# emanuelev/supereight

Measured on AMD Instinct MI355X. Metric: frames/sec (integrate+raycast), 640x480 depth -> 512^3 TSDF, higher is better.
Workload: dtype f32

## Files before the change

### include/se_hip.h

```cpp
#ifndef SE_HIP_H
#define SE_HIP_H

#include <stdint.h>

#ifdef __cplusplus
extern "C" {
#endif

#define SE_HIP_FIELD_SDF 0
#define SE_HIP_FIELD_OFUSION 1

#define SE_HIP_OK 0
#define SE_HIP_E_INVALID (-1)
#define SE_HIP_E_DEVICE (-2)
#define SE_HIP_E_CAPACITY (-3)
#define SE_HIP_E_NOGPU (-4)

typedef struct se_hip_pipeline se_hip_pipeline;

typedef struct se_hip_config {
  int32_t width;
  int32_t height;
  int32_t volume_resolution;
  float volume_dimension;
  int32_t field_type;
  int32_t device;
  int64_t max_blocks;
  int32_t row_begin;
  int32_t row_end;
} se_hip_config;

int se_hip_create(const se_hip_config* cfg, se_hip_pipeline** out);
int se_hip_create_replicas(const se_hip_config* cfg, const int32_t* device_ids, int32_t n_devices, se_hip_pipeline** out_handles);
int se_hip_destroy(se_hip_pipeline* p);
const char* se_hip_last_error(void);
int se_hip_sync(se_hip_pipeline* p);
int se_hip_clear_overflow(se_hip_pipeline* p);
int se_hip_set_stream(se_hip_pipeline* p, void* hip_stream);
int se_hip_set_scan_stream(se_hip_pipeline* p, void* hip_stream);
int se_hip_scan_overlaps(se_hip_pipeline* p);
int se_hip_set_streaming(se_hip_pipeline* p, int32_t on);
int se_hip_frame_is_fused(se_hip_pipeline* p);
int se_hip_set_image_ring(se_hip_pipeline* p, float* device_ring, int32_t slots);

int se_hip_upload_depth(se_hip_pipeline* p, const float* host_depth_m);
int se_hip_upload_depth_mm(se_hip_pipeline* p, const uint16_t* host_depth_mm, int32_t in_w, int32_t in_h);
int se_hip_set_pinned_input(se_hip_pipeline* p, int32_t on);
void* se_hip_host_alloc(size_t bytes);
void se_hip_host_free(void* host);
int se_hip_set_depth_device(se_hip_pipeline* p, const float* device_depth_m);

int se_hip_integrate(se_hip_pipeline* p, const float pose[16], const float k[4], uint32_t integration_rate, float mu,
                     uint32_t frame);
int se_hip_alloc_scan(se_hip_pipeline* p, const float pose[16], const float k[4], uint32_t integration_rate, float mu,
                      uint32_t frame);
int se_hip_new_keys_device(se_hip_pipeline* p, uint64_t** device_list, int64_t* capacity_words);
int se_hip_set_new_keys_buffer(se_hip_pipeline* p, uint64_t* device_list, int64_t capacity_words);
int se_hip_alloc_commit(se_hip_pipeline* p, const uint64_t* device_lists, int32_t nlists, int64_t stride_words);
int se_hip_set_exchange(se_hip_pipeline* p, void* nccl_comm, void* nccl_all_gather, int32_t world);
int se_hip_alloc_exchange(se_hip_pipeline* p, uint64_t* recv_device, int64_t words);
int se_hip_integrate_sweep(se_hip_pipeline* p, const float pose[16], const float k[4], uint32_t integration_rate,
                           float mu, uint32_t frame);
size_t se_hip_sweep_shard_bytes(size_t cap_bricks);
int se_hip_set_sweep_shard(se_hip_pipeline* p, int32_t rank, int32_t world, void* send_device, size_t cap_bricks);
int se_hip_apply_bricks(se_hip_pipeline* p, const void* recv_device, int32_t world);
int se_hip_brick_exchange(se_hip_pipeline* p, void* recv_device);

size_t se_hip_image_tile_bytes(se_hip_pipeline* p, int32_t max_rows);
int se_hip_pack_image_tile(se_hip_pipeline* p, void* send_device, int32_t max_rows);
int se_hip_apply_image_tiles(se_hip_pipeline* p, const void* recv_device, int32_t world, int32_t max_rows, const int32_t* row_begin, const int32_t* row_end);
int se_hip_gather_images(se_hip_pipeline* p, void* send_device, void* recv_device, int32_t max_rows, const int32_t* row_begin, const int32_t* row_end);

int se_hip_frame(se_hip_pipeline* p, const float* device_depth_m, const float pose[16], const float k[4], uint32_t integration_rate,
                 float mu, uint32_t frame);

int se_hip_raycast(se_hip_pipeline* p, const float pose[16], const float k[4], float mu, uint32_t frame);
int se_hip_raycast_deferred(se_hip_pipeline* p, const float pose[16], const float k[4], float mu, uint32_t frame);
int se_hip_download_vertex_normal(se_hip_pipeline* p, float* host_vertex_xyz, float* host_normal_xyz);
int se_hip_vertex_normal_device(se_hip_pipeline* p, float** device_vertex_xyz, float** device_normal_xyz);

int se_hip_track(se_hip_pipeline* p, const float k[4], float icp_threshold, uint32_t tracking_rate, uint32_t frame,
                 const int32_t* pyramid, int32_t n_levels, float pose_inout[16]);
int se_hip_frame_tracked(se_hip_pipeline* p, const float* device_depth_m, const float k[4], float icp_threshold, uint32_t tracking_rate,
                         const int32_t* pyramid, int32_t n_levels, float pose_inout[16], uint32_t integration_rate, float mu, uint32_t frame);
int se_hip_filter_depth(se_hip_pipeline* p, int32_t on);
int se_hip_download_scaled_depth(se_hip_pipeline* p, int32_t level, float* host_out);
int se_hip_download_track(se_hip_pipeline* p, void* host_trackdata, float host_reduce32[32], int32_t* iterations);

int se_hip_render_volume(se_hip_pipeline* p, uint8_t* host_rgbw, const float view_pose[16], const float k[4], float mu, float largestep,
                         uint32_t frame, uint32_t raycast_rendering_rate);
int se_hip_render_depth(se_hip_pipeline* p, uint8_t* host_rgbw);
int se_hip_render_track(se_hip_pipeline* p, uint8_t* host_rgbw);

int se_hip_counts(se_hip_pipeline* p, int32_t* n_blocks, int32_t* n_nodes);
int se_hip_memory_info(se_hip_pipeline* p, int64_t out[4]);
int se_hip_download_blocks(se_hip_pipeline* p, int32_t* coords, float* x, float* y, uint8_t* active);
int se_hip_download_nodes(se_hip_pipeline* p, uint64_t* code, uint32_t* side, float* x, float* y);

typedef struct se_hip_query_out {
  float* fine;
  float* coarse;
  float* interp;
  float* grad;
  uint8_t* status;
} se_hip_query_out;
int se_hip_query_points(se_hip_pipeline* p, const float* device_points_m, int64_t n, const se_hip_query_out* device_out);
int se_hip_query_points_host(se_hip_pipeline* p, const float* host_points_m, int64_t n, const se_hip_query_out* host_out);

#define SE_HIP_COLLISION_OCCUPIED 0
#define SE_HIP_COLLISION_UNSEEN 1
#define SE_HIP_COLLISION_EMPTY 2
#define SE_HIP_COLLISION_INVALID 255
#define SE_HIP_COLLIDE_STRICT 0
#define SE_HIP_COLLIDE_REFERENCE 1
typedef struct se_hip_collide_test {
  float threshold;
  int32_t occupied_above;
} se_hip_collide_test;
int se_hip_collide_boxes(se_hip_pipeline* p, const int32_t* device_boxes, int64_t n, const se_hip_collide_test* test, int32_t mode,
                         uint8_t* device_status);
int se_hip_collide_boxes_host(se_hip_pipeline* p, const int32_t* host_boxes, int64_t n, const se_hip_collide_test* test, int32_t mode,
                              uint8_t* host_status);

#define SE_HIP_RAY_VALID 1
#define SE_HIP_RAY_ENTERED 2
#define SE_HIP_RAY_HIT 4
#define SE_HIP_RAY_NORMAL 8
typedef struct se_hip_ray_out {
  float* hit;
  float* normal;
  uint8_t* status;
} se_hip_ray_out;
int se_hip_cast_rays(se_hip_pipeline* p, const float* device_rays, int64_t n, float mu, const se_hip_ray_out* device_out);
int se_hip_cast_rays_host(se_hip_pipeline* p, const float* host_rays, int64_t n, float mu, const se_hip_ray_out* host_out);

int se_hip_save_map(se_hip_pipeline* p, const char* filename);
int se_hip_load_map(se_hip_pipeline* p, const char* filename);

int se_hip_mesh_count(se_hip_pipeline* p, int64_t* n_triangles);
int se_hip_mesh_download(se_hip_pipeline* p, float* host_triangles, int64_t capacity_triangles, int64_t* n_written);
int se_hip_dump_mesh(se_hip_pipeline* p, const char* filename);

#define SE_HIP_MESH_MAX_VIEWS 64
#define SE_HIP_MESH_SKIP_EMPTY 1u
typedef struct se_hip_mesh_view {
  float pose[16];
  float k[4];
  int32_t width, height;
} se_hip_mesh_view;
typedef struct se_hip_mesh_select {
  int32_t lo[3], hi[3];
  int32_t n_views;
  uint32_t flags;
  const se_hip_mesh_view* views;
} se_hip_mesh_select;
typedef struct se_hip_mesh_out {
  float* triangles;
  int64_t capacity_triangles;
  int32_t* block_coords;
  int64_t* block_range;
  int64_t capacity_blocks;
  int64_t* header;
} se_hip_mesh_out;
int se_hip_mesh_blocks(se_hip_pipeline* p, const se_hip_mesh_select* select, const se_hip_mesh_out* device_out);
int se_hip_mesh_blocks_host(se_hip_pipeline* p, const se_hip_mesh_select* select, const se_hip_mesh_out* host_out);

#define SE_HIP_EDIT_SET_X 1u
#define SE_HIP_EDIT_SET_Y 2u
#define SE_HIP_EDIT_BLOCKS 4u
#define SE_HIP_EDIT_NODES 8u
#define SE_HIP_EDIT_STRICT 0
#define SE_HIP_EDIT_REFERENCE 1
typedef struct se_hip_edit {
  int32_t lo[3], hi[3];
  float x, y;
  uint32_t flags;
  uint32_t only;
} se_hip_edit;
int se_hip_edit_boxes(se_hip_pipeline* p, const se_hip_edit* device_edits, int64_t n, const se_hip_collide_test* test,
                      int32_t mode, int64_t* device_counts);
int se_hip_edit_boxes_host(se_hip_pipeline* p, const se_hip_edit* host_edits, int64_t n, const se_hip_collide_test* test,
                           int32_t mode, int64_t* host_counts);

typedef struct se_hip_alloc_box {
  int32_t lo[3], hi[3];
  int32_t level;
  uint32_t reserved;
} se_hip_alloc_box;
int se_hip_allocate_boxes(se_hip_pipeline* p, const se_hip_alloc_box* device_boxes, int64_t n, int64_t* device_counts,
                          uint64_t* device_new_keys, int64_t capacity_words);
int se_hip_allocate_boxes_host(se_hip_pipeline* p, const se_hip_alloc_box* host_boxes, int64_t n, int64_t* host_counts,
                               uint64_t* host_new_keys, int64_t capacity_words);

#define SE_HIP_K_ALLOC_SCAN 0
#define SE_HIP_K_ALLOC_COMMIT 1
#define SE_HIP_K_INTEGRATE 2
#define SE_HIP_K_RAYCAST 3
#define SE_HIP_K_APPLY_BRICKS 4
#define SE_HIP_K_COUNT 5
int se_hip_enable_timing(se_hip_pipeline* p, int32_t on);
int se_hip_get_timings(se_hip_pipeline* p, double ms_sum[SE_HIP_K_COUNT], int64_t launches[SE_HIP_K_COUNT], int32_t reset);
int se_hip_get_launch_counts(se_hip_pipeline* p, int64_t counts[SE_HIP_K_COUNT + 1], int32_t reset);
int se_hip_enable_stats(se_hip_pipeline* p, int32_t on);
int se_hip_get_stats(se_hip_pipeline* p, uint64_t out[16], int32_t reset);

#ifdef __cplusplus
}
#endif
#endif
```

### supereight_amd/csrc/se_hip_api.hip

```cpp
#include "../../include/se_hip.h"

#include <hip/hip_runtime.h>
#include <hipcub/device/device_radix_sort.hpp>

#include <algorithm>
#include <cmath>
#include <cstdio>
#include <cstdlib>
#include <atomic>
#include <chrono>
#include <cstring>
#include <thread>
#include <numeric>
#include <string>
#include <vector>

#include "se_kernels.h"
#include "se_track_kernels.h"
#include "se_mesh_kernels.h"
#include "se_query_kernels.h"
#include "se_collide_kernels.h"
#include "se_edit_kernels.h"
#include "se_alloc_kernels.h"
#include "se_ray_kernels.h"
// ... 17 lines not shown
  for (int c = 0; c < 4; ++c)
    for (int r = 0; r < 4; ++r) a.m[r][c] = p[c * 4 + r];
  return a;
}
M4 mul(const M4& a, const M4& b) {
  M4 c;
  for (int i = 0; i < 4; ++i)
    for (int j = 0; j < 4; ++j)
      c.m[i][j] = ((a.m[i][0] * b.m[0][j] + a.m[i][1] * b.m[1][j]) + a.m[i][2] * b.m[2][j]) + a.m[i][3] * b.m[3][j];
  return c;
}
M4 camera_matrix(const float k[4]) { return {{{k[0], 0, k[2], 0}, {0, k[1], k[3], 0}, {0, 0, 1, 0}, {0, 0, 0, 1}}}; }
M4 inverse_camera_matrix(const float k[4]) {
  return {{{1.0f / k[0], 0, -k[2] / k[0], 0}, {0, 1.0f / k[1], -k[3] / k[1], 0}, {0, 0, 1, 0}, {0, 0, 0, 1}}};
}
void mul3(const float r[9], const float v[3], float out[3]) {
  out[0] = (r[0] * v[0] + r[1] * v[1]) + r[2] * v[2];
  out[1] = (r[3] * v[0] + r[4] * v[1]) + r[5] * v[2];
  out[2] = (r[6] * v[0] + r[7] * v[1]) + r[8] * v[2];
}

struct TimedLaunch { int kernel; hipEvent_t start, stop; };

inline void cpu_relax() {
#if defined(__x86_64__) || defined(__i386__)
  __builtin_ia32_pause();
#elif defined(__aarch64__) || defined(__arm__)
  asm volatile("yield" ::: "memory");
#else
  std::this_thread::yield();
#endif
}
template <typename F> bool spin_until(F done, long long limit_us) {
  const auto t0 = std::chrono::steady_clock::now();
  for (unsigned n = 1;; ++n) {
    if (done()) { std::atomic_thread_fence(std::memory_order_acquire); return true; }
    cpu_relax();
    if ((n & 255u) == 0u && std::chrono::duration_cast<std::chrono::microseconds>(std::chrono::steady_clock::now() - t0).count() > limit_us) {
      const bool ok = done();
      std::atomic_thread_fence(std::memory_order_acquire);
      return ok;
    }
  }
}

}

struct se_hip_pipeline {
  se_hip_config cfg;
  int device = 0;
  hipStream_t stream = nullptr;
  bool own_stream = false;
  hipStream_t side = nullptr;
  bool own_side = false;
  hipEvent_t ev_sweep = nullptr, ev_scan = nullptr;
  hipEvent_t ev_edit = nullptr;
  bool overlap = false;
  bool host_gate = false;
  uint32_t* gate_host = nullptr;
  uint32_t ray_seq = 0;
  uint32_t gate_target = 0;
  bool gate_armed = false;
  bool gate_followed = false;
  bool sharded = false;
  bool fuse = false, in_frame = false, has_pending = false;
  int flush_streak = 0;
  bool pinned_input = false;
  int sort_every = 0;
  uint32_t* bpos_sorted = nullptr; void* sort_tmp = nullptr; size_t sort_tmp_bytes = 0, sort_cap = 0;
  uint32_t sorted_n = 0; int sweeps_since_sort = 0;
  bool ptrs_exposed = false;
  float pend_pose[16] = {0}, pend_k[4] = {0}, pend_mu = 0.f;
  uint32_t pend_frame = 0;
  bool images_complete = true;
  bool scan_pending = false;
  bool scan_on_side = false;
  const float* scaled0 = nullptr;
  void* xcomm = nullptr;
  int (*xgather)(const void*, void*, size_t, int, void*, hipStream_t) = nullptr;
  int xworld = 0;
  int shard_world = 0, shard_rank = 0;
  unsigned char* shard_send = nullptr;
  size_t shard_cap = 0;
  bool mc_table_ready = false;
  unsigned long long* mesh_ctr = nullptr;
  unsigned char* staging = nullptr;
  size_t staging_cap = 0;
  unsigned char* meshb_dev = nullptr;
  bool filter_input = false;
  bool occ_commit_due = false;
  OccLists occ_lists{nullptr, 0, 0};
  float raycast_pose[16] = {1, 0, 0, 0, 0, 1, 0, 0, 0, 0, 1, 0, 0, 0, 0, 1};
  std::vector<float*> pyr_depth, pyr_vertex, pyr_normal;
  TrackData* track = nullptr;
  float* reduce_partial = nullptr;
  IcpState* icp = nullptr;
  IcpHostRecord* icp_host = nullptr;
  unsigned reduce_seq = 0;
  int track_iterations = 0;
  int icp_lookahead = 2;
  bool scan_on_main_once = false;
  unsigned char* rgbw = nullptr;
  DevMap map{};
  int leaf_level = 0, max_level = 0;
  size_t tab_entries = 0;
  size_t occ_words = 0, lbits_words = 0, cbits_words = 0, fbits_words = 0;
  bool of_leap = true;
  int beam = 2;
  size_t slots = 0;
  size_t cap_blocks = 0, cap_nodes = 0;
  int ray_cache_levels = -1;
  const float* depth = nullptr;
  static constexpr int kIn = 3;
  float* depth_ring[kIn] = {nullptr, nullptr, nullptr};
  void* in_host[kIn] = {nullptr, nullptr, nullptr};
  size_t in_cap = 0;
  int in_next = 0;
  int in_state[kIn] = {0, 0, 0};
  uint32_t in_seq[kIn] = {0, 0, 0};
  hipEvent_t in_done[kIn] = {nullptr, nullptr, nullptr};
  bool in_event[kIn] = {false, false, false};
  int cur_in = -1;
  DepthSrc in_pending{nullptr, nullptr, 0, 0, 0};
  float* vertex = nullptr;
  float* normal = nullptr;
  float* vertex_own = nullptr;
  float* normal_own = nullptr;
  float* ring = nullptr;
  int ring_slots = 0;
  int64_t n_launch[SE_HIP_K_COUNT + 1] = {0};
  float* bspline = nullptr;
  float* logodds = nullptr;
  unsigned long long* chain = nullptr;
  unsigned long long* newkeys_own = nullptr;
  unsigned long long* newkeys_own2 = nullptr;
  unsigned long long cap_keys_own = 0;
  int own_next = 0;
  bool own_clean[2] = {false, false};
  uint32_t* ctr_host = nullptr;
  bool timing = false, stats = false;
  std::vector<TimedLaunch> pending;
  std::vector<hipEvent_t> event_pool;
  double ms_sum[SE_HIP_K_COUNT] = {0};
  int64_t launches[SE_HIP_K_COUNT] = {0};
  int row_begin = 0, row_end = 0;
  int integ_grid = 0;
  bool ieee_sweep = false;
  unsigned short* tile_cost = nullptr;
  int* prio_thr = nullptr;
  bool prio_hint = true;
  int prio_permille[3] = {400, 150, 50};
  uint32_t* ray_order = nullptr;
  int n_cus = 256;
};

namespace {

int ilog2(int v) { int l = 0; while ((1 << l) < v) ++l; return l; }

hipEvent_t get_event(se_hip_pipeline* p) {
  if (!p->event_pool.empty()) { hipEvent_t e = p->event_pool.back(); p->event_pool.pop_back(); return e; }
  hipEvent_t e;
  hipEventCreateWithFlags(&e, hipEventDisableSystemFence);
  return e;
}
struct ScopedTimer {
  se_hip_pipeline* p; int k; hipStream_t s; hipEvent_t a{}, b{};
  ScopedTimer(se_hip_pipeline* p_, int k_, hipStream_t s_ = nullptr) : p(p_), k(k_), s(s_ ? s_ : p_->stream) {
    p->n_launch[k]++;
    if (p->timing) { a = get_event(p); b = get_event(p); hipEventRecord(a, s); }
  }
  ~ScopedTimer() {
    if (p->timing) { hipEventRecord(b, s); p->pending.push_back({k, a, b}); }
  }
};
void drain_timings(se_hip_pipeline* p) {
  if (p->pending.empty()) return;
  if (p->side) hipStreamSynchronize(p->side);
  hipStreamSynchronize(p->stream);
  for (auto& t : p->pending) {
    float ms = 0.f;
    if (hipEventElapsedTime(&ms, t.start, t.stop) == hipSuccess) { p->ms_sum[t.kernel] += ms; p->launches[t.kernel]++; }
    p->event_pool.push_back(t.start);
    p->event_pool.push_back(t.stop);
  }
  p->pending.clear();
}

double bspline_cdf(double t) {
  if (t >= -3.0 && t <= -1.0) return std::pow(3 + t, 3) / 48.0;
  if (t > -1 && t <= 1) return 0.5 + (t * (3 + t) * (3 - t)) / 24.0;
  if (t > 1 && t <= 3) return 1 - std::pow(3 - t, 3) / 48.0;
  if (t > 3) return 1.0;
  return 0.0;
}
void make_bspline(std::vector<float>& lut) {
  lut.resize(1000);
  for (int i = 0; i < 1000; ++i) {
    char buf[64];
    std::snprintf(buf, sizeof buf, "%.12g", bspline_cdf(-3.0 + 6.0 * i / 999.0));
    lut[i] = (float)std::strtod(buf, nullptr);
  }
}
void make_logodds(const std::vector<float>& lut, std::vector<float>& tab) {
  tab.resize((size_t)SE_LO_DIM * SE_LO_DIM);
  auto q = [&](int i) { return i < 1000 ? lut[i] : (i == 1001 ? 1.f : 0.f); };
  for (int i1 = 0; i1 < SE_LO_DIM; ++i1)
    for (int i2 = 0; i2 < SE_LO_DIM; ++i2) {
      float sample = q(i1) - q(i2) * 0.5f;
      sample = std::max(0.03f, std::min(sample, 0.97f));
      tab[(size_t)i1 * SE_LO_DIM + i2] = log2f(sample / (1.f - sample));
    }
}

int run_zero_chain(se_hip_pipeline* p, const unsigned long long* lists, int nlists, long long stride_words) {
  ScopedTimer t(p, SE_HIP_K_ALLOC_COMMIT);
  hipLaunchKernelGGL(k_zero_chain, dim3(1), dim3(SE_WG), 0, p->stream, p->map, lists, nlists, stride_words);
  return SE_HIP_OK;
}


M4 rigid_inverse(const M4& a) {
  M4 r{};
  for (int i = 0; i < 3; ++i)
    for (int j = 0; j < 3; ++j) r.m[i][j] = a.m[j][i];
  for (int i = 0; i < 3; ++i) r.m[i][3] = -((r.m[i][0] * a.m[0][3] + r.m[i][1] * a.m[1][3]) + r.m[i][2] * a.m[2][3]);
  r.m[3][3] = 1.f;
  return r;
}

struct RayLaunchArgs { RayArgs a; size_t smem; dim3 grid; };

size_t ray_map_args(se_hip_pipeline* p, float mu, RayArgs& a) {
  const DevMap& m = p->map;
  a.mu = mu;
  a.step = m.dim / (float)m.size;
  a.largestep = a.step * 8;
  a.inv_voxel = (float)m.size / m.dim;
  a.grad_scale = 0.5f * m.dim / (float)m.size;
  a.epsilon = exp2f(-(float)p->max_level);
  a.min_scale = 23 - p->leaf_level;
  int cl = p->ray_cache_levels >= 0 ? p->ray_cache_levels : 5;
  cl = std::min(cl, p->leaf_level);
  a.cache_levels = cl;
  a.cache_words = (int)occ_words_upto(cl);
  a.cache_codes = 2u << (3 * cl);
  a.has_deep = cl < p->leaf_level - 1 ? 1 : 0;
  a.stack_depth = p->leaf_level;
  return ((size_t)a.cache_words + (size_t)2 * a.stack_depth * SE_WG_RAY) * sizeof(uint32_t);
}

RayLaunchArgs make_ray_args(se_hip_pipeline* p, const float pose_cm[16], const float k[4], float mu) {
  RayLaunchArgs L{};
  const DevMap& m = p->map;
  const M4 view = mul(from_colmajor(pose_cm), inverse_camera_matrix(k));
  RayArgs& a = L.a;
  for (int i = 0; i < 3; ++i) { for (int j = 0; j < 3; ++j) a.view3[i * 3 + j] = view.m[i][j]; a.org[i] = view.m[i][3]; }
  a.nearp = 0.4f; a.farp = 4.0f;
  a.near_n = a.nearp / m.dim; a.far_n = a.farp / m.dim;
  for (int i = 0; i < 3; ++i) a.scaled_origin[i] = a.org[i] / m.dim + 1.f;
  L.smem = ray_map_args(p, mu, a);
  a.W = p->cfg.width; a.H = p->cfg.height; a.row_begin = p->row_begin; a.row_end = p->row_end;
  a.tile_cost = p->prio_hint ? p->tile_cost : nullptr;
  a.prio_thr = p->prio_thr;
  a.cost_shift = std::max(0, p->leaf_level - 6);
  a.ray_order = p->ray_order; a.n_cus = p->n_cus;
  a.beam = (p->beam >= 2 && !m.fbits) ? 1 : p->beam;
  const int flevel = m.fbits ? se_flevel(m) : m.leaf_level;
  a.beam_cellf = m.dim / (float)(1 << flevel);
  a.beam_inv_cellf = (float)(1 << flevel) / m.dim;
  a.beam_dt2 = 0.4f * a.beam_cellf;
  if (a.beam >= 2) {
    const float rad = 1.05f * std::hypot(0.5f * (SE_TILE_W - 1) / std::fabs(k[0]), 0.5f * (SE_TILE_H - 1) / std::fabs(k[1])) + a.epsilon;
    if (!((0.75f * a.farp + 0.5f * a.beam_dt2) * rad + 0.5f * a.beam_dt2 <= 0.9f * a.beam_cellf)) a.beam = 1;
  }
  a.beam_cell = m.dim / (float)(1 << m.clevel);
  a.beam_inv_cell = (float)(1 << m.clevel) / m.dim;
  a.beam_dt = std::max(0.5f * a.beam_cell, (a.farp - a.nearp) / 64.f);
  a.inv_dim = 1.f / m.dim;
  a.leap_bits = !p->of_leap ? nullptr : m.fbits ? m.fbits : (m.clevel == m.leaf_level ? m.cbits : nullptr);
  a.leap_level = flevel;
  a.leap_dt = 0.9f * a.beam_cellf;
  a.wlog = nullptr;
#ifdef SE_WAVE_PROBE
  {
    static unsigned long long* wl = nullptr;
    static bool tried = false;
    if (!tried) { tried = true; if (std::getenv("SE_HIP_WLOG")) { hipHostMalloc((void**)&wl, 4 * 8 * 32768, 0); std::memset(wl, 0, 4 * 8 * 32768); } }
    a.wlog = wl;
    if (wl) { hipStreamSynchronize(p->stream); if (FILE* f = std::fopen(std::getenv("SE_HIP_WLOG"), "wb")) { std::fwrite(wl, 8, 4 * 32768, f); std::fclose(f); } std::memset(wl, 0, 4 * 8 * 32768); }
  }
#endif
  const int tiles_x = (a.W + SE_TILE_W - 1) / SE_TILE_W, tiles_y = (a.row_end - a.row_begin + SE_TILE_H - 1) / SE_TILE_H;
  const int n_pairs = (tiles_x * tiles_y + 1) / 2;
  L.grid = dim3((unsigned)(((n_pairs + p->n_cus - 1) / p->n_cus) * p->n_cus));
  return L;
}

RayLaunchArgs make_batch_ray_args(se_hip_pipeline* p, float mu) {
  RayLaunchArgs L{};
  RayArgs& a = L.a;
  L.smem = ray_map_args(p, mu, a);
  a.gate = nullptr; a.tile_cost = nullptr; a.ray_order = nullptr; a.prio_thr = nullptr; a.wlog = nullptr; a.leap_bits = nullptr;
  a.beam = 0;
  return L;
}

struct RaySel { bool ofusion, dense, shallow, o32; };
RaySel ray_kernel_sel(const se_hip_pipeline* p, const RayArgs& a) {
  const DevMap& m = p->map;
  const size_t nb = (size_t)(m.size >> 3);
  const bool shallow = !a.has_deep;
  return {p->cfg.field_type != SE_HIP_FIELD_SDF, m.dense != 0, shallow,
          m.dense && shallow && nb * nb * nb * (size_t)SE_BRICK_STRIDE * sizeof(float) <= ((size_t)4 << 30)};
}

void wait_last_sweep(se_hip_pipeline* p) {
  if (!p->gate_armed) return;
  p->gate_armed = false;
  if (p->gate_followed) {
    volatile uint32_t* w = p->gate_host;
    const uint32_t target = p->gate_target;
    if (!spin_until([&] { return (int32_t)(*w - target) >= 0; }, 20000)) hipStreamSynchronize(p->stream);
    return;
  }
  hipStreamSynchronize(p->stream);
}

void materialise_depth(se_hip_pipeline* p, hipStream_t s) {
  if (p->in_pending.kind == 0) return;
  const int W = p->cfg.width, H = p->cfg.height;
  hipLaunchKernelGGL(k_depth_from_host, dim3((W + 255) / 256, H), dim3(256), 0, s, p->in_pending, W, H);
  p->in_pending.kind = 0;
}
void input_slot_in_use(se_hip_pipeline* p) { if (p->cur_in >= 0) { p->in_state[p->cur_in] = 1; p->in_event[p->cur_in] = false; } }
void input_slots_followed(se_hip_pipeline* p, uint32_t seq) {
  for (int i = 0; i < se_hip_pipeline::kIn; ++i) if (p->in_state[i] == 1) { p->in_state[i] = 2; p->in_seq[i] = seq; }
}

int join_scan(se_hip_pipeline* p, bool fold_into_sweep = false) {
  if (p->scan_pending) {
    p->scan_pending = false;
    HIP_TRY(hipStreamWaitEvent(p->stream, p->ev_scan, 0));
    p->occ_commit_due = true;
    if (!p->occ_lists.lists) p->occ_lists = OccLists{p->map.newkeys, 1, (long long)p->map.cap_keys + 1};
    if (p->cfg.field_type == SE_HIP_FIELD_OFUSION && !p->sharded)
      if (int r = run_zero_chain(p, p->map.newkeys, 1, (long long)p->map.cap_keys + 1)) return r;
  }
  if (p->occ_commit_due && !fold_into_sweep) {
    p->occ_commit_due = false;
    ScopedTimer t(p, SE_HIP_K_ALLOC_COMMIT);
    hipLaunchKernelGGL(k_occ_commit, dim3(64), dim3(SE_WG), 0, p->stream, p->map, p->occ_lists);
    p->occ_lists = OccLists{nullptr, 0, 0};
  }
  return SE_HIP_OK;
}

int check(se_hip_pipeline* p) {
  if (!p) return fail(SE_HIP_E_INVALID, "null handle");
  int cur = -1;
  if (!(hipGetDevice(&cur) == hipSuccess && cur == p->device)) {
    hipError_t e = hipSetDevice(p->device);
    if (e != hipSuccess) return fail(SE_HIP_E_DEVICE, std::string("hipSetDevice: ") + hipGetErrorString(e));
  }
  if (p->has_pending && !p->in_frame) { ++p->flush_streak; return flush_pending_raycast(p); }
  return SE_HIP_OK;
}

int check_overflow(se_hip_pipeline* p) {
  const uint32_t o = p->ctr_host[C_OVERFLOW];
  if (o == 3) return fail(SE_HIP_E_CAPACITY, "brick exchange segment overflow: the peers missed block updates (raise cap_bricks of se_hip_set_sweep_shard)");
  if (o) return fail(SE_HIP_E_CAPACITY, o == 2 ? "new-key list overflow: blocks were allocated locally but not reported to the peers (raise the exchange capacity)"
                                              : "block / node pool exhausted (raise max_blocks)");
  return SE_HIP_OK;
}

int fetch_counters(se_hip_pipeline* p) {
  if (int r = join_scan(p)) return r;
  HIP_TRY(hipMemcpyAsync(p->ctr_host, p->map.ctr, C_COUNT * sizeof(uint32_t), hipMemcpyDeviceToHost, p->stream));
  HIP_TRY(hipStreamSynchronize(p->stream));
  return check_overflow(p);
}

int reserve_staging(se_hip_pipeline* p, size_t need) {
  if (need <= p->staging_cap) return SE_HIP_OK;
  if (p->staging) { HIP_TRY(hipStreamSynchronize(p->stream)); hipFree(p->staging); p->staging = nullptr; p->staging_cap = 0; }
  HIP_TRY(hipMalloc((void**)&p->staging, need));
  p->staging_cap = need;
  return SE_HIP_OK;
}
size_t staging_layout(const size_t* bytes, int k, size_t* off) {
  size_t at = 0;
  for (int i = 0; i < k; ++i) { off[i] = at; at += bytes[i]; }
  return at;
}
template <typename Check> int query_prologue(se_hip_pipeline* p, Check args_ok) {
  if (int r = check(p)) return r;
  if (int r = args_ok()) return r;
  return join_scan(p);
}
struct BatchOut { void* ptr; size_t item_bytes; bool per_call = false; };
struct BatchOuts { int count; BatchOut o[5]; };
template <typename Check, typename Launch>
int batch_device(se_hip_pipeline* p, const void* in, int64_t n, const BatchOuts& out, Check args_ok, Launch launch) {
  if (int r = query_prologue(p, args_ok)) return r;
  if (int r = check_overflow(p)) return r;
  if (n == 0) return SE_HIP_OK;
  void* dev[5];
  for (int k = 0; k < out.count; ++k) dev[k] = out.o[k].ptr;
  launch(in, dev);
  HIP_TRY(hipGetLastError());
  return SE_HIP_OK;
}
template <typename Check, typename Launch>
int batch_host(se_hip_pipeline* p, const void* in, size_t in_item_bytes, int64_t n, const BatchOuts& out, Check args_ok, Launch launch) {
  if (int r = query_prologue(p, args_ok)) return r;
  if (n == 0) return fetch_counters(p);
  const size_t un = (size_t)n;
  size_t bytes[6], off[6];
  bytes[0] = un * in_item_bytes;
  for (int k = 0; k < out.count; ++k) bytes[k + 1] = out.o[k].ptr ? (out.o[k].per_call ? 1 : un) * out.o[k].item_bytes : 0;
  if (int r = reserve_staging(p, staging_layout(bytes, out.count + 1, off))) return r;
  unsigned char* b = p->staging;
  HIP_TRY(hipMemcpyAsync(b, in, bytes[0], hipMemcpyHostToDevice, p->stream));
  void* dev[5];
  for (int k = 0; k < out.count; ++k) dev[k] = bytes[k + 1] ? b + off[k + 1] : nullptr;
  launch(b, dev);
  HIP_TRY(hipGetLastError());
  for (int k = 0; k < out.count; ++k)
    if (bytes[k + 1]) HIP_TRY(hipMemcpyAsync(out.o[k].ptr, dev[k], bytes[k + 1], hipMemcpyDeviceToHost, p->stream));
  return fetch_counters(p);
}

void select_image_target(se_hip_pipeline* p, uint32_t frame) {
  if (p->ring) {
    const size_t n3 = (size_t)p->cfg.width * p->cfg.height * 3;
    p->vertex = p->ring + (size_t)(frame % (uint32_t)p->ring_slots) * 2 * n3;
    p->normal = p->vertex + n3;
  } else {
    p->vertex = p->vertex_own; p->normal = p->normal_own;
  }
}
struct InFrame { se_hip_pipeline* p; bool was; explicit InFrame(se_hip_pipeline* q, bool on = true) : p(q), was(q->in_frame) { q->in_frame = on; } ~InFrame() { p->in_frame = was; } };

bool finite_pose(const float* pose_cm, const float* k) {
  bool ok = true;
  for (int i = 0; i < 16; ++i) ok = ok && std::isfinite(pose_cm[i]);
  for (int i = 0; i < 4; ++i) ok = ok && std::isfinite(k[i]);
  return ok && k[0] != 0.f && k[1] != 0.f;
}

bool stage_runs_integration(uint32_t frame, uint32_t rate) { return ((frame % rate) == 0) || (frame <= 3); }

void reset_map_state(se_hip_pipeline* p) {
  DevMap& m = p->map;
  hipMemsetAsync(m.tab, 0, p->tab_entries * sizeof(uint32_t), p->stream);
  hipMemsetAsync(m.occ, 0, p->occ_words * sizeof(uint32_t), p->stream);
  hipMemsetAsync(m.lbits, 0, p->lbits_words * sizeof(uint32_t), p->stream);
  hipMemsetAsync(m.cbits, 0, 2 * p->cbits_words * sizeof(uint32_t), p->stream);
  if (m.fbits) hipMemsetAsync(m.fbits, 0, p->fbits_words * sizeof(uint32_t), p->stream);
  hipMemsetAsync(m.bpos, 0, p->cap_blocks * sizeof(uint32_t), p->stream);
  hipMemsetAsync(m.bactive, 0, p->slots, p->stream);
  hipMemsetAsync(m.npos, 0, p->cap_nodes * sizeof(uint32_t), p->stream);
  hipMemsetAsync(m.nlevel, 0, p->cap_nodes, p->stream);
  hipMemsetAsync(m.stats, 0, S_COUNT * sizeof(unsigned long long), p->stream);
  hipMemsetAsync(m.newkeys, 0, sizeof(unsigned long long), p->stream);
  if (p->newkeys_own) hipMemsetAsync(p->newkeys_own, 0, sizeof(unsigned long long), p->stream);
  if (p->newkeys_own2) hipMemsetAsync(p->newkeys_own2, 0, sizeof(unsigned long long), p->stream);
  p->own_clean[0] = p->newkeys_own != nullptr; p->own_clean[1] = p->newkeys_own2 != nullptr;
  const uint32_t ctr0[C_COUNT] = {0u, 1u, 0u, 0u, 0u, 0u, 0u, 0u};
  hipMemcpyAsync(m.ctr, ctr0, sizeof ctr0, hipMemcpyHostToDevice, p->stream);
  std::memset(p->ctr_host, 0, C_COUNT * sizeof(uint32_t));
  p->ctr_host[C_NODES] = 1u;
  p->sorted_n = 0; p->sweeps_since_sort = 0;
  hipLaunchKernelGGL(k_fill_bricks, dim3(16384), dim3(256), 0, p->stream, m.vx, m.init_x, m.init_y, p->slots * 1024);
  hipLaunchKernelGGL(k_fill, dim3(256), dim3(256), 0, p->stream, m.nx, m.init_x, p->cap_nodes * 8);
  hipLaunchKernelGGL(k_fill, dim3(256), dim3(256), 0, p->stream, m.ny, m.init_y, p->cap_nodes * 8);
}

int grid_for(size_t n, int wg, int cap) { size_t g = (n + wg - 1) / wg; if (g < 1) g = 1; if (g > (size_t)cap) g = cap; return (int)g; }

}

extern "C" {

const char* se_hip_last_error(void) { return g_err.c_str(); }

int se_hip_create(const se_hip_config* cfg, se_hip_pipeline** out) {
  if (!cfg || !out) return fail(SE_HIP_E_INVALID, "null argument");
  *out = nullptr;
  const int N = cfg->volume_resolution;
  if (cfg->width <= 0 || cfg->height <= 0) return fail(SE_HIP_E_INVALID, "bad image size");
  if (N < 64 || N > 4096 || (N & (N - 1))) return fail(SE_HIP_E_INVALID, "volume_resolution must be a power of two in [64, 4096]");
  if (!(cfg->volume_dimension > 0)) return fail(SE_HIP_E_INVALID, "volume_dimension must be positive");
  if (cfg->field_type != SE_HIP_FIELD_SDF && cfg->field_type != SE_HIP_FIELD_OFUSION) return fail(SE_HIP_E_INVALID, "unknown field type");
  int ndev = 0;
  if (hipGetDeviceCount(&ndev) != hipSuccess || ndev <= 0) return fail(SE_HIP_E_NOGPU, "no HIP device visible (this library has no CPU path)");
  if (cfg->device < 0 || cfg->device >= ndev) return fail(SE_HIP_E_INVALID, "device ordinal out of range");
  HIP_TRY(hipSetDevice(cfg->device));
  hipDeviceProp_t prop;
  HIP_TRY(hipGetDeviceProperties(&prop, cfg->device));
  if (std::string(prop.gcnArchName).find("gfx950") == std::string::npos)
    return fail(SE_HIP_E_NOGPU, std::string("device is ") + prop.gcnArchName + ", this library is built for gfx950 only");

  se_hip_pipeline* p = new se_hip_pipeline();
  p->cfg = *cfg;
  p->device = cfg->device;
  p->row_begin = cfg->row_begin;
  p->row_end = (cfg->row_end > cfg->row_begin) ? cfg->row_end : cfg->height;
  if (p->row_begin < 0 || p->row_end > cfg->height) { delete p; return fail(SE_HIP_E_INVALID, "bad row range"); }
  if (const char* ev = std::getenv("SE_HIP_RAY_CACHE_LEVELS")) p->ray_cache_levels = std::atoi(ev);
  if (const char* ev = std::getenv("SE_HIP_ICP_LOOKAHEAD")) p->icp_lookahead = std::max(0, std::atoi(ev));
  if (const char* ev = std::getenv("SE_HIP_INTEG_GRID")) p->integ_grid = std::atoi(ev);
  if (const char* ev = std::getenv("SE_HIP_BEAM")) p->beam = std::max(0, std::min(2, std::atoi(ev)));
  if (const char* ev = std::getenv("SE_HIP_OF_LEAP")) p->of_leap = std::atoi(ev) != 0;
  if (const char* ev = std::getenv("SE_HIP_IEEE_SWEEP")) p->ieee_sweep = std::atoi(ev) != 0;
  if (const char* ev = std::getenv("SE_HIP_PRIO")) p->prio_hint = std::atoi(ev) != 0;
  if (const char* ev = std::getenv("SE_HIP_PRIO_SHARE")) {
    int a = 0, b = 0, c = 0;
    if (std::sscanf(ev, "%d,%d,%d", &a, &b, &c) == 3 && a >= b && b >= c && c >= 0 && a <= 1000) { p->prio_permille[0] = a; p->prio_permille[1] = b; p->prio_permille[2] = c; }
  }
  p->max_level = ilog2(N);
  p->leaf_level = p->max_level - 3;
  DevMap& m = p->map;
  m.size = N; m.max_level = p->max_level; m.leaf_level = p->leaf_level; m.dim = cfg->volume_dimension;
  size_t off = 0;
  for (int l = 0; l < SE_MAX_LEVELS; ++l) m.off[l] = 0;
  for (int l = 1; l <= p->leaf_level; ++l) { m.off[l] = (uint32_t)off; off += (size_t)1 << (3 * l); }
  p->tab_entries = off;
  m.leaf_off = m.off[p->leaf_level];
  p->occ_words = occ_words_upto(p->leaf_level);
  const size_t cells = (size_t)1 << (3 * p->leaf_level);
  size_t free_b = 0, total_b = 0;
  hipMemGetInfo(&free_b, &total_b);
  size_t dense_max_gib = 64;
  if (const char* ev = std::getenv("SE_HIP_DENSE_MAX_GIB")) dense_max_gib = (size_t)std::max(0, std::atoi(ev));

  bool dense = cfg->max_blocks <= 0 && cells * 4096 <= free_b / 3 && cells * 4096 <= (dense_max_gib << 30);
  if (const char* ev = std::getenv("SE_HIP_DENSE")) dense = std::atoi(ev) != 0 && cells * 4096 <= free_b / 2;
  const size_t nb_side = (size_t)cfg->volume_resolution / 8;
  const size_t cap_default = std::max((size_t)1 << 16, ((24 * nb_side * nb_side + 4095) / 4096) * 4096);
  size_t cap = cfg->max_blocks > 0 ? (size_t)cfg->max_blocks : (dense ? cells : std::max((size_t)1 << 16, std::min(cap_default, free_b / 3 / 4096)));
  cap = std::min(cap, cells);
  m.dense = dense ? 1 : 0;
  p->sort_every = (dense && nb_side >= 128) ? 4 : 0;
  if (const char* ev = std::getenv("SE_HIP_SORT_BLOCKS")) p->sort_every = dense ? std::max(0, std::atoi(ev)) : 0;
  const size_t slots = dense ? cells : cap;
  p->slots = slots;
  size_t capn = std::min(off - cells + 1, cap / 2 + 4096);
  m.cap_blocks = (uint32_t)cap; m.cap_nodes = (uint32_t)capn;
  m.cap_keys = cap + capn;
  if (cfg->field_type == SE_HIP_FIELD_SDF) { m.init_x = 1.f; m.init_y = 0.f; m.empty_x = 1.f; }
  else { m.init_x = 0.f; m.init_y = 0.f; m.empty_x = 0.f; }

  auto bail = [&](hipError_t e, const char* what) { std::string msg = std::string(what) + ": " + hipGetErrorString(e); se_hip_destroy(p); return fail(SE_HIP_E_DEVICE, msg); };
#define ALLOC(ptr, bytes) do { hipError_t e_ = hipMalloc((void**)&(ptr), (bytes)); if (e_ != hipSuccess) return bail(e_, "hipMalloc " #ptr); } while (0)
  hipError_t e = hipStreamCreateWithFlags(&p->stream, hipStreamNonBlocking);
  if (e != hipSuccess) return bail(e, "hipStreamCreate");
  p->own_stream = true;
  e = hipStreamCreateWithFlags(&p->side, hipStreamNonBlocking);
  if (e != hipSuccess) return bail(e, "hipStreamCreate");
  p->own_side = true;
  hipEventCreateWithFlags(&p->ev_sweep, hipEventDisableTiming | hipEventDisableSystemFence);
  hipEventCreateWithFlags(&p->ev_scan, hipEventDisableTiming | hipEventDisableSystemFence);
  p->sharded = (p->row_begin != 0 || p->row_end != cfg->height);
  p->overlap = (dense || !(std::getenv("SE_HIP_POOLED_OVERLAP") && std::atoi(std::getenv("SE_HIP_POOLED_OVERLAP")) == 0)) && !std::getenv("SE_HIP_NO_OVERLAP");
  p->host_gate = p->overlap && !p->sharded;
  if (const char* ev = std::getenv("SE_HIP_HOST_GATE")) p->host_gate = p->host_gate && std::atoi(ev) != 0;
  if (p->host_gate) {
    e = hipHostMalloc((void**)&p->gate_host, 64);
    if (e != hipSuccess) return bail(e, "hipHostMalloc");
    std::memset(p->gate_host, 0, 64);
  }
  ALLOC(m.tab, p->tab_entries * sizeof(uint32_t));
  ALLOC(m.occ, p->occ_words * sizeof(uint32_t));
  p->lbits_words = (cells + 31) / 32;
  ALLOC(m.lbits, p->lbits_words * sizeof(uint32_t));
  m.clevel = std::min(p->leaf_level, 5);
  p->cbits_words = std::max<size_t>(1, ((size_t)1 << (3 * m.clevel)) / 32);
  ALLOC(m.cbits, 2 * p->cbits_words * sizeof(uint32_t));
  m.fbits = nullptr;
  if (se_flevel(m) > m.clevel) { p->fbits_words = ((size_t)1 << (3 * se_flevel(m))) / 32; ALLOC(m.fbits, p->fbits_words * sizeof(uint32_t)); }
  ALLOC(m.vx, slots * 1024 * sizeof(float));
  m.ybyte = cfg->field_type == SE_HIP_FIELD_SDF ? 1 : 0;
  ALLOC(m.bpos, cap * sizeof(uint32_t));
  ALLOC(m.bactive, (slots + 3) & ~(size_t)3);
  ALLOC(m.nx, capn * 8 * sizeof(float));
  ALLOC(m.ny, capn * 8 * sizeof(float));
  ALLOC(m.npos, capn * sizeof(uint32_t));
  ALLOC(m.nlevel, capn);
  ALLOC(m.ctr, C_COUNT * sizeof(uint32_t));
  ALLOC(m.stats, S_COUNT * sizeof(unsigned long long));
  ALLOC(m.newkeys, (m.cap_keys + 1) * sizeof(unsigned long long));
  p->newkeys_own = m.newkeys; p->cap_keys_own = m.cap_keys;
  ALLOC(p->newkeys_own2, (m.cap_keys + 1) * sizeof(unsigned long long));
  for (int i = 0; i < se_hip_pipeline::kIn; ++i) ALLOC(p->depth_ring[i], (size_t)cfg->width * cfg->height * sizeof(float));
  ALLOC(p->vertex_own, (size_t)cfg->width * cfg->height * 3 * sizeof(float));
  ALLOC(p->normal_own, (size_t)cfg->width * cfg->height * 3 * sizeof(float));
  p->vertex = p->vertex_own; p->normal = p->normal_own;
  ALLOC(p->chain, 4 * sizeof(unsigned long long));
  const size_t n_tiles = ((size_t)(cfg->width + SE_TILE_W - 1) / SE_TILE_W) * ((size_t)(cfg->height + SE_TILE_H - 1) / SE_TILE_H);
  ALLOC(p->tile_cost, (n_tiles + 4096) * sizeof(unsigned short));
  ALLOC(p->prio_thr, 4 * sizeof(int));
  hipMemsetAsync(p->tile_cost, 0, (n_tiles + 4096) * sizeof(unsigned short), p->stream);
  {
    hipDeviceProp_t prop{};
    if (hipGetDeviceProperties(&prop, p->device) == hipSuccess && prop.multiProcessorCount > 0) p->n_cus = prop.multiProcessorCount;
    if (const char* ev = std::getenv("SE_HIP_RAY_DEAL")) p->n_cus = std::max(1, std::atoi(ev));
    const size_t n_pairs = (n_tiles + 1) / 2;
    ALLOC(p->ray_order, n_pairs * sizeof(uint32_t));
    std::vector<uint32_t> ident(n_pairs);
    for (size_t i = 0; i < n_pairs; ++i) ident[i] = (uint32_t)i;
    hipMemcpyAsync(p->ray_order, ident.data(), n_pairs * sizeof(uint32_t), hipMemcpyHostToDevice, p->stream);
    hipStreamSynchronize(p->stream);
  }
  { const int off[4] = {256, 256, 256, 0}; hipMemcpyAsync(p->prio_thr, off, sizeof off, hipMemcpyHostToDevice, p->stream); }
  p->depth = p->depth_ring[0]; p->cur_in = 0;
  e = hipHostMalloc((void**)&p->ctr_host, C_COUNT * sizeof(uint32_t));
  if (e != hipSuccess) return bail(e, "hipHostMalloc");
  std::memset(p->ctr_host, 0, C_COUNT * sizeof(uint32_t));

  p->cap_blocks = cap; p->cap_nodes = capn;
  reset_map_state(p);
  for (int i = 0; i < se_hip_pipeline::kIn; ++i) hipMemsetAsync(p->depth_ring[i], 0, (size_t)cfg->width * cfg->height * sizeof(float), p->stream);
  hipMemsetAsync(p->vertex, 0, (size_t)cfg->width * cfg->height * 3 * sizeof(float), p->stream);
  hipMemsetAsync(p->normal, 0, (size_t)cfg->width * cfg->height * 3 * sizeof(float), p->stream);
  if (cfg->field_type == SE_HIP_FIELD_OFUSION) {
    std::vector<float> lut, lo;
    make_bspline(lut);
    make_logodds(lut, lo);
    ALLOC(p->bspline, lut.size() * sizeof(float));
    ALLOC(p->logodds, lo.size() * sizeof(float));
    hipMemcpy(p->bspline, lut.data(), lut.size() * sizeof(float), hipMemcpyHostToDevice);
    hipMemcpy(p->logodds, lo.data(), lo.size() * sizeof(float), hipMemcpyHostToDevice);
  }
#undef ALLOC
  e = hipStreamSynchronize(p->stream);
  if (e != hipSuccess) return bail(e, "initialisation");
  *out = p;
  return SE_HIP_OK;
}

int se_hip_destroy(se_hip_pipeline* p) {
  if (!p) return SE_HIP_OK;
  p->has_pending = false;
  hipSetDevice(p->device);
  if (p->side) hipStreamSynchronize(p->side);
  if (p->stream) hipStreamSynchronize(p->stream);
  for (auto& t : p->pending) { hipEventDestroy(t.start); hipEventDestroy(t.stop); }
  for (auto& ev : p->event_pool) hipEventDestroy(ev);
  DevMap& m = p->map;
  void* ptrs[] = {m.occ, m.lbits, m.cbits, m.fbits, m.tab, m.vx, m.bpos, m.bactive, m.nx, m.ny, m.npos, m.nlevel, m.ctr, m.stats, p->newkeys_own, p->newkeys_own2,
                  p->depth_ring[0], p->depth_ring[1], p->depth_ring[2], p->vertex_own, p->normal_own, p->bspline, p->logodds, p->chain, p->tile_cost, p->prio_thr, p->ray_order};
  for (void* q : ptrs) if (q) hipFree(q);
  for (auto* q : p->pyr_depth) if (q) hipFree(q);
  for (auto* q : p->pyr_vertex) if (q) hipFree(q);
  for (auto* q : p->pyr_normal) if (q) hipFree(q);
  if (p->track) hipFree(p->track);
  if (p->rgbw) hipFree(p->rgbw);
  if (p->reduce_partial) hipFree(p->reduce_partial);
  if (p->icp) hipFree(p->icp);
  if (p->icp_host) hipHostFree(p->icp_host);
  if (p->ctr_host) hipHostFree(p->ctr_host);
  if (p->bpos_sorted) hipFree(p->bpos_sorted);
  if (p->sort_tmp) hipFree(p->sort_tmp);
  if (p->gate_host) hipHostFree(p->gate_host);
  if (p->mesh_ctr) hipFree(p->mesh_ctr);
  if (p->staging) hipFree(p->staging);
  if (p->meshb_dev) hipFree(p->meshb_dev);
  for (int i = 0; i < se_hip_pipeline::kIn; ++i) { if (p->in_host[i]) hipHostFree(p->in_host[i]); if (p->in_done[i]) hipEventDestroy(p->in_done[i]); }
  if (p->own_side && p->side) hipStreamDestroy(p->side);
  if (p->ev_sweep) hipEventDestroy(p->ev_sweep);
  if (p->ev_scan) hipEventDestroy(p->ev_scan);
  if (p->ev_edit) hipEventDestroy(p->ev_edit);
  if (p->own_stream && p->stream) hipStreamDestroy(p->stream);
  delete p;
  return SE_HIP_OK;
}

int se_hip_sync(se_hip_pipeline* p) {
  if (int r = check(p)) return r;
  if (p->side) HIP_TRY(hipStreamSynchronize(p->side));
  HIP_TRY(hipStreamSynchronize(p->stream));
  p->gate_armed = false;
  return check_overflow(p);
}

int se_hip_clear_overflow(se_hip_pipeline* p) {
  if (int r = check(p)) return r;
  if (p->side) HIP_TRY(hipStreamSynchronize(p->side));
  HIP_TRY(hipStreamSynchronize(p->stream));
  p->gate_armed = false;
  uint32_t dev = 0;
  HIP_TRY(hipMemcpy(&dev, p->map.ctr + C_OVERFLOW, sizeof dev, hipMemcpyDeviceToHost));
  const uint32_t pending = std::max(dev, p->ctr_host[C_OVERFLOW]);
  HIP_TRY(hipMemsetAsync(p->map.ctr + C_OVERFLOW, 0, sizeof(uint32_t), p->stream));
  HIP_TRY(hipStreamSynchronize(p->stream));
  p->ctr_host[C_OVERFLOW] = 0u;
  return (int)pending;
}

int se_hip_set_stream(se_hip_pipeline* p, void* hip_stream) {
  if (int r = check(p)) return r;
  HIP_TRY(hipStreamSynchronize(p->stream));
  p->gate_armed = false;
  drain_timings(p);
  if (p->own_stream && p->stream) hipStreamDestroy(p->stream);
  p->stream = (hipStream_t)hip_stream;
  p->own_stream = false;
  return SE_HIP_OK;
}

int se_hip_scan_overlaps(se_hip_pipeline* p) {
  if (int r = check(p)) return r;
  return p->overlap ? 1 : 0;
}

int se_hip_set_scan_stream(se_hip_pipeline* p, void* hip_stream) {
  if (int r = check(p)) return r;
  if (p->side) HIP_TRY(hipStreamSynchronize(p->side));
  HIP_TRY(hipStreamSynchronize(p->stream));
  drain_timings(p);
  if (p->own_side && p->side) hipStreamDestroy(p->side);
  p->side = nullptr; p->own_side = false;
  if (hip_stream) { p->side = (hipStream_t)hip_stream; return SE_HIP_OK; }
  HIP_TRY(hipStreamCreateWithFlags(&p->side, hipStreamNonBlocking));
  p->own_side = true;
  return SE_HIP_OK;
}

static int stage_input(se_hip_pipeline* p, const void* host, size_t bytes, int kind, int in_w, int ratio) {
  constexpr int R = se_hip_pipeline::kIn;
  if (p->in_cap < bytes) {
    if (p->side) HIP_TRY(hipStreamSynchronize(p->side));
    HIP_TRY(hipStreamSynchronize(p->stream));
    for (int i = 0; i < R; ++i) { if (p->in_host[i]) hipHostFree(p->in_host[i]); p->in_host[i] = nullptr; p->in_state[i] = 0; p->in_event[i] = false; }
    p->in_cap = 0; p->in_pending.kind = 0;
    for (int i = 0; i < R; ++i) HIP_TRY(hipHostMalloc(&p->in_host[i], bytes));
    p->in_cap = bytes;
  }
  const int i = p->in_next;
  p->in_next = (i + 1) % R;
  if (p->in_state[i] == 2 && p->host_gate) {
    volatile uint32_t* w = p->gate_host;
    const uint32_t target = p->in_seq[i];
    if (!spin_until([&] { return (int32_t)(*w - target) >= 0; }, 20000)) { if (p->side) hipStreamSynchronize(p->side); hipStreamSynchronize(p->stream); }
  } else if (p->in_event[i]) {
    HIP_TRY(hipEventSynchronize(p->in_done[i]));
  } else if (p->in_state[i] != 0) {
    if (p->side) HIP_TRY(hipStreamSynchronize(p->side));
    HIP_TRY(hipStreamSynchronize(p->stream));
  }
  p->in_state[i] = 0; p->in_event[i] = false;
  const void* src = p->in_host[i];
  if (p->pinned_input) {
    hipPointerAttribute_t at{};
    if (hipPointerGetAttributes(&at, host) == hipSuccess && at.type == hipMemoryTypeHost && at.devicePointer) src = at.devicePointer;
    else (void)hipGetLastError();
  }
  if (src == p->in_host[i]) std::memcpy(p->in_host[i], host, bytes);
  p->in_pending = DepthSrc{src, p->depth_ring[i], kind, in_w, ratio};
  p->depth = p->depth_ring[i];
  p->cur_in = i;
  return SE_HIP_OK;
}

int se_hip_upload_depth(se_hip_pipeline* p, const float* host_depth_m) {
  if (!p) return fail(SE_HIP_E_INVALID, "null handle");
  InFrame guard(p);
  if (int r = check(p)) return r;
  if (!host_depth_m) return fail(SE_HIP_E_INVALID, "null depth");
  return stage_input(p, host_depth_m, (size_t)p->cfg.width * p->cfg.height * sizeof(float), 2, p->cfg.width, 1);
}

int se_hip_upload_depth_mm(se_hip_pipeline* p, const uint16_t* host_mm, int32_t in_w, int32_t in_h) {
  if (!p) return fail(SE_HIP_E_INVALID, "null handle");
  InFrame guard(p);
  if (int r = check(p)) return r;
  if (!host_mm) return fail(SE_HIP_E_INVALID, "null depth");
  const int W = p->cfg.width, H = p->cfg.height;
  if (in_w < W || in_h < H || in_w % W != 0 || in_h % H != 0 || in_w / W != in_h / H) return fail(SE_HIP_E_INVALID, "Invalid ratio.");
  return stage_input(p, host_mm, (size_t)in_w * in_h * sizeof(unsigned short), 1, in_w, in_w / W);
}

int se_hip_set_pinned_input(se_hip_pipeline* p, int32_t on) {
  if (!p) return fail(SE_HIP_E_INVALID, "null handle");
  p->pinned_input = on != 0;
  return SE_HIP_OK;
}
void* se_hip_host_alloc(size_t bytes) {
  void* h = nullptr;
  if (bytes == 0 || hipHostMalloc(&h, bytes) != hipSuccess) { (void)hipGetLastError(); return nullptr; }
  return h;
}
void se_hip_host_free(void* host) { if (host) (void)hipHostFree(host); }

int se_hip_set_depth_device(se_hip_pipeline* p, const float* device_depth_m) {
  if (!p) return fail(SE_HIP_E_INVALID, "null handle");
  InFrame guard(p);
  if (int r = check(p)) return r;
  if (device_depth_m) { p->depth = device_depth_m; p->cur_in = -1; p->in_pending.kind = 0; }
  else if (p->cur_in < 0) { p->depth = p->depth_ring[0]; p->cur_in = 0; }
  return SE_HIP_OK;
}

int launch_raycast_scan(se_hip_pipeline* p, const DevMap& ms, const AllocArgs& sa, int scan_wgs, const DepthSrc& ds) {
  const DevMap& m = p->map;
  if (int r = check_overflow(p)) return r;
  p->has_pending = false;
  p->flush_streak = 0;
  std::memcpy(p->raycast_pose, p->pend_pose, sizeof p->raycast_pose);
  p->images_complete = !p->sharded;
  select_image_target(p, p->pend_frame);
  p->n_launch[SE_HIP_K_ALLOC_SCAN]++; p->n_launch[SE_HIP_K_COUNT]++;
  RayLaunchArgs L = make_ray_args(p, p->pend_pose, p->pend_k, p->pend_mu);
  if (p->host_gate) { L.a.gate = p->gate_host; L.a.gate_seq = ++p->ray_seq; if (p->gate_armed) p->gate_followed = true; input_slots_followed(p, L.a.gate_seq); }
  const RayArgs& a = L.a;
  const int ray_wgs = (int)L.grid.x;
  const size_t smem = std::max(L.smem, (size_t)SE_SCAN_SLOTS * SE_WG_SCAN * sizeof(uint32_t));
  const dim3 grid((unsigned)(ray_wgs + scan_wgs)), block(SE_WG_RAY);
  const RaySel s = ray_kernel_sel(p, a);
  const bool shallow = s.dense ? s.o32 : s.shallow;
  {
    ScopedTimer t(p, SE_HIP_K_RAYCAST);
#define SE_RS(OF, DN, SH, O3) hipLaunchKernelGGL((k_raycast_scan<OF, DN, SH, O3>), grid, block, smem, p->stream, m, a, p->vertex, p->normal, ray_wgs, ms, p->depth, sa, ds)
    if (!s.ofusion) {
      if (s.dense) { if (shallow) SE_RS(false, true, true, true); else SE_RS(false, true, false, false); }
      else { if (shallow) SE_RS(false, false, true, false); else SE_RS(false, false, false, false); }
    } else {
      if (s.dense) { if (shallow) SE_RS(true, true, true, true); else SE_RS(true, true, false, false); }
      else { if (shallow) SE_RS(true, false, true, false); else SE_RS(true, false, false, false); }
    }
#undef SE_RS
  }
  HIP_TRY(hipGetLastError());
  return SE_HIP_OK;
}

static bool frame_can_fuse(se_hip_pipeline* p);
int se_hip_alloc_scan(se_hip_pipeline* p, const float pose_cm[16], const float k[4], uint32_t rate, float mu, uint32_t frame) {
  if (!p) return fail(SE_HIP_E_INVALID, "null handle");
  const bool ride = p->has_pending && !p->in_frame && rate != 0 && stage_runs_integration(frame, rate) && frame_can_fuse(p);
  InFrame guard(p, ride || p->in_frame);
  if (int r = check(p)) return r;
  if (!pose_cm || !k || rate == 0) return fail(SE_HIP_E_INVALID, "bad argument");
  if (!finite_pose(pose_cm, k)) return fail(SE_HIP_E_INVALID, "non-finite pose or intrinsics");
  if (!stage_runs_integration(frame, rate)) return 0;
  const DevMap& m = p->map;
  const M4 pose = from_colmajor(pose_cm);
  const bool sdf = p->cfg.field_type == SE_HIP_FIELD_SDF;
  AllocArgs a{};
  const float voxelsize = m.dim / (float)m.size;
  const M4 kPose = mul(pose, inverse_camera_matrix(k));
  for (int i = 0; i < 3; ++i)
    for (int j = 0; j < 4; ++j) a.kpose[i * 4 + j] = kPose.m[i][j];
  a.cam[0] = pose.m[0][3]; a.cam[1] = pose.m[1][3]; a.cam[2] = pose.m[2][3];
  a.band = sdf ? 2 * mu : 6 * mu;
  a.voxel = voxelsize;
  a.inv_voxel = sdf ? 1 / voxelsize : 1.f / voxelsize;
  a.num_steps = (int)std::ceil(a.band * a.inv_voxel);
  a.W = p->cfg.width; a.H = p->cfg.height; a.row_begin = p->row_begin; a.row_end = p->row_end;
  a.sharded = (p->row_begin != 0 || p->row_end != p->cfg.height) ? 1 : 0;
  auto s2d = [&](float step) { return (int)(floorf(log2f(voxelsize / step)) + m.max_level); };
  a.depth_fine = s2d(voxelsize); a.depth_mid = s2d(10.f * voxelsize); a.depth_coarse = s2d(30.f * voxelsize);
  const bool caller_list = p->map.newkeys != p->newkeys_own && p->map.newkeys != p->newkeys_own2;
  const bool fuse_now = p->has_pending && p->in_frame && p->overlap && !p->stats && p->shard_world <= 1;
  const bool chain = p->scan_on_main_once && !p->sharded && !caller_list && p->xgather == nullptr;
  p->scan_on_main_once = false;
  const bool ov = !fuse_now && !chain && p->overlap && (p->sharded || caller_list || p->xgather != nullptr || hipStreamQuery(p->stream) == hipErrorNotReady);
  p->scan_on_side = ov;
  hipStream_t s = ov ? p->side : p->stream;
  DevMap ms = m;
  ms.defer_occ = (ov || fuse_now) ? 1 : 0;
  ms.defer_mark = 1;
  if (ov) { if (p->host_gate) wait_last_sweep(p); else HIP_TRY(hipStreamWaitEvent(p->side, p->ev_sweep, 0)); }
  else if (p->overlap) { if (int r = join_scan(p)) return r; }
  const bool own_list = p->map.newkeys == p->newkeys_own || p->map.newkeys == p->newkeys_own2;
  if (own_list) {
    const int w = p->own_next;
    p->map.newkeys = w ? p->newkeys_own2 : p->newkeys_own;
    ms.newkeys = p->map.newkeys;
    if (!p->own_clean[w]) HIP_TRY(hipMemsetAsync(p->map.newkeys, 0, sizeof(unsigned long long), s));
    p->own_clean[w] = false;
  } else {
    HIP_TRY(hipMemsetAsync(m.newkeys, 0, sizeof(unsigned long long), s));
  }
  const int npix = (p->row_end - p->row_begin) * p->cfg.width;
  const dim3 grid((npix + SE_WG_SCAN - 1) / SE_WG_SCAN), block(SE_WG_SCAN);
  if (a.sharded) materialise_depth(p, s);
  const DepthSrc ds = p->in_pending;
  p->in_pending.kind = 0;
  const int sdf_tiles = ds.kind ? ((p->cfg.width + 63) / 64) * (p->row_end - p->row_begin) : ((p->cfg.width + 7) / 8) * ((p->row_end - p->row_begin + 7) / 8);
  if (!sdf) {
    const int dep[3] = {a.depth_fine, a.depth_mid, a.depth_coarse};
    for (int i = 0; i < 3; ++i) { a.of_lvl[i] = std::min(dep[i], m.leaf_level); a.of_off[i] = a.of_lvl[i] >= 1 ? m.off[a.of_lvl[i]] : 0u; }
  }
  if (fuse_now) {
    const int scan_wgs = sdf ? (sdf_tiles + SE_WG_SCAN / 64 - 1) / (SE_WG_SCAN / 64) : (int)grid.x;
    if (int r = launch_raycast_scan(p, ms, a, scan_wgs, ds)) return r;
    input_slot_in_use(p);
    p->occ_commit_due = true;
    if (!p->occ_lists.lists) p->occ_lists = OccLists{p->map.newkeys, 1, (long long)p->map.cap_keys + 1};
    if (!sdf && !a.sharded) { if (int r = run_zero_chain(p, p->map.newkeys, 1, (long long)p->map.cap_keys + 1)) return r; }
    HIP_TRY(hipGetLastError());
    return 1;
  }
  {
    ScopedTimer t(p, SE_HIP_K_ALLOC_SCAN, s);
    if (sdf) {
      const dim3 sgrid((sdf_tiles + SE_WG_SCAN / 64 - 1) / (SE_WG_SCAN / 64));
      if (m.dense) {
        if (p->stats) hipLaunchKernelGGL((k_alloc_scan_sdf<true, true>), sgrid, block, 0, s, ms, p->depth, a, ds);
        else hipLaunchKernelGGL((k_alloc_scan_sdf<false, true>), sgrid, block, 0, s, ms, p->depth, a, ds);
      } else {
        if (p->stats) hipLaunchKernelGGL((k_alloc_scan_sdf<true, false>), sgrid, block, 0, s, ms, p->depth, a, ds);
        else hipLaunchKernelGGL((k_alloc_scan_sdf<false, false>), sgrid, block, 0, s, ms, p->depth, a, ds);
      }
    } else {
      if (p->stats) hipLaunchKernelGGL(k_alloc_scan_ofusion<true>, grid, block, 0, s, ms, p->depth, a, ds);
      else hipLaunchKernelGGL(k_alloc_scan_ofusion<false>, grid, block, 0, s, ms, p->depth, a, ds);
    }
  }
  input_slot_in_use(p);
  if (ov) {
    HIP_TRY(hipEventRecord(p->ev_scan, p->side));
    p->scan_pending = true;
    HIP_TRY(hipGetLastError());
    return 1;
  }
  p->occ_commit_due = true;
  if (!p->occ_lists.lists) p->occ_lists = OccLists{p->map.newkeys, 1, (long long)p->map.cap_keys + 1};
  if (!sdf && !a.sharded) {
    if (int r = run_zero_chain(p, m.newkeys, 1, (long long)m.cap_keys + 1)) return r;
  }
  HIP_TRY(hipGetLastError());
  return 1;
}

int se_hip_new_keys_device(se_hip_pipeline* p, uint64_t** device_list, int64_t* capacity_words) {
  if (int r = check(p)) return r;
  if (int r = join_scan(p)) return r;
  if (device_list) *device_list = (uint64_t*)p->map.newkeys;
  if (capacity_words) *capacity_words = (int64_t)p->map.cap_keys + 1;
  return SE_HIP_OK;
}

int se_hip_set_new_keys_buffer(se_hip_pipeline* p, uint64_t* device_list, int64_t capacity_words) {
  if (!p) return fail(SE_HIP_E_INVALID, "null handle");
  InFrame guard(p);
  if (int r = check(p)) return r;
  if (device_list && capacity_words < 2) return fail(SE_HIP_E_INVALID, "key buffer too small");
  p->map.newkeys = device_list ? (unsigned long long*)device_list : p->newkeys_own;
  p->map.cap_keys = device_list ? (unsigned long long)(capacity_words - 1) : p->cap_keys_own;
  return SE_HIP_OK;
}

int se_hip_alloc_commit(se_hip_pipeline* p, const uint64_t* device_lists, int32_t nlists, int64_t stride_words) {
  if (int r = check(p)) return r;
  if (!device_lists || nlists <= 0 || stride_words < 1) return fail(SE_HIP_E_INVALID, "bad argument");
  const unsigned long long* lists = (const unsigned long long*)device_lists;
  if (p->overlap && p->side && p->scan_on_side) {
    DevMap md = p->map;
    md.defer_occ = 1; md.defer_mark = 1;
    {
      ScopedTimer t(p, SE_HIP_K_ALLOC_COMMIT, p->side);
      hipLaunchKernelGGL(k_alloc_commit, dim3(64, nlists), dim3(SE_WG), 0, p->side, md, lists, nlists, (long long)stride_words);
    }
    HIP_TRY(hipEventRecord(p->ev_scan, p->side));
    p->scan_pending = true;
    p->occ_lists = OccLists{lists, nlists, (long long)stride_words};
  } else if (p->occ_commit_due && !p->scan_pending) {
    ScopedTimer t(p, SE_HIP_K_ALLOC_COMMIT);
    hipLaunchKernelGGL(k_alloc_commit, dim3(64, nlists), dim3(SE_WG), 0, p->stream, p->map, lists, nlists, (long long)stride_words);
  } else {
    if (int r = join_scan(p)) return r;
    ScopedTimer t(p, SE_HIP_K_ALLOC_COMMIT);
    hipLaunchKernelGGL(k_alloc_commit, dim3(64, nlists), dim3(SE_WG), 0, p->stream, p->map, lists, nlists, (long long)stride_words);
  }
  if (p->cfg.field_type == SE_HIP_FIELD_OFUSION) {
    if (int r = join_scan(p, true)) return r;
    if (int r = run_zero_chain(p, lists, nlists, (long long)stride_words)) return r;
  }
  HIP_TRY(hipGetLastError());
  return SE_HIP_OK;
}

int se_hip_set_exchange(se_hip_pipeline* p, void* nccl_comm, void* nccl_all_gather, int32_t world) {
  if (int r = check(p)) return r;
  if ((nccl_comm == nullptr) != (nccl_all_gather == nullptr) || (nccl_comm && world < 1)) return fail(SE_HIP_E_INVALID, "bad argument");
  p->xcomm = nccl_comm;
  p->xgather = (int (*)(const void*, void*, size_t, int, void*, hipStream_t))nccl_all_gather;
  p->xworld = nccl_comm ? world : 0;
  return SE_HIP_OK;
}

int se_hip_alloc_exchange(se_hip_pipeline* p, uint64_t* recv_device, int64_t words) {
  if (int r = check(p)) return r;
  if (!p->xgather) return fail(SE_HIP_E_INVALID, "no exchange set (se_hip_set_exchange)");
  if (!recv_device || words < 2 || (unsigned long long)words > p->map.cap_keys + 1) return fail(SE_HIP_E_INVALID, "bad argument");
  hipStream_t s = (p->overlap && p->side && p->scan_on_side) ? p->side : p->stream;
  const int rc = p->xgather(p->map.newkeys, recv_device, (size_t)words,  4, p->xcomm, s);
  if (rc != 0) return fail(SE_HIP_E_DEVICE, "ncclAllGather failed with code " + std::to_string(rc));
  return se_hip_alloc_commit(p, recv_device, p->xworld, words);
}

size_t se_hip_sweep_shard_bytes(size_t cap_bricks) { return SE_SHARD_SUB * 8 + cap_bricks * 4 + cap_bricks * 4096; }

int se_hip_set_sweep_shard(se_hip_pipeline* p, int32_t rank, int32_t world, void* send_device, size_t cap_bricks) {
  if (int r = check(p)) return r;
  if (world <= 1) { p->shard_world = 0; p->shard_send = nullptr; p->shard_cap = 0; return SE_HIP_OK; }
  if (rank < 0 || rank >= world || !send_device || ((uintptr_t)send_device & 15u) || cap_bricks == 0 || (cap_bricks % SE_SHARD_SUB) || cap_bricks > ((size_t)1 << 30))
    return fail(SE_HIP_E_INVALID, "bad argument (send segment 16-byte aligned, cap_bricks a positive multiple of 64)");
  p->shard_world = world; p->shard_rank = rank; p->shard_send = (unsigned char*)send_device; p->shard_cap = cap_bricks;
  return SE_HIP_OK;
}

int se_hip_apply_bricks(se_hip_pipeline* p, const void* recv_device, int32_t world) {
  if (int r = check(p)) return r;
  if (p->shard_world <= 1 || world != p->shard_world || !recv_device) return fail(SE_HIP_E_INVALID, "no sharded sweep set (se_hip_set_sweep_shard) or bad argument");
  {
    ScopedTimer t(p, SE_HIP_K_APPLY_BRICKS);
    const size_t est = (size_t)p->ctr_host[C_BLOCKS] / (size_t)world + 1024;
    const size_t wgs = std::min<size_t>((est + 3) / 4, 16384);
    const dim3 grid((unsigned)(((wgs + 15) / 16) * 16), (unsigned)world);
    hipLaunchKernelGGL(k_apply_bricks, grid, dim3(SE_WG), 0, p->stream, p->map, (const unsigned char*)recv_device,
                       se_hip_sweep_shard_bytes(p->shard_cap), (uint32_t)p->shard_cap, p->shard_rank);
  }
  if (!p->host_gate) hipEventRecord(p->ev_sweep, p->stream);
  HIP_TRY(hipGetLastError());
  return SE_HIP_OK;
}

int se_hip_brick_exchange(se_hip_pipeline* p, void* recv_device) {
  if (int r = check(p)) return r;
  if (!p->xgather) return fail(SE_HIP_E_INVALID, "no exchange set (se_hip_set_exchange)");
  if (p->shard_world <= 1 || p->xworld != p->shard_world || !recv_device) return fail(SE_HIP_E_INVALID, "no sharded sweep set (se_hip_set_sweep_shard) or bad argument");
  const int rc = p->xgather(p->shard_send, recv_device, se_hip_sweep_shard_bytes(p->shard_cap),  1, p->xcomm, p->stream);
  if (rc != 0) return fail(SE_HIP_E_DEVICE, "ncclAllGather failed with code " + std::to_string(rc));
  return se_hip_apply_bricks(p, recv_device, p->xworld);
}

static int sort_block_list(se_hip_pipeline* p) {
  if (p->sort_every <= 0 || !p->map.dense) return SE_HIP_OK;
  const uint32_t n0 = std::min<uint32_t>(p->ctr_host[C_BLOCKS], p->map.cap_blocks);
  if (++p->sweeps_since_sort < p->sort_every || n0 < 4096 || (size_t)n0 * 2 < (size_t)p->sorted_n * 3) return SE_HIP_OK;
  if (p->sort_cap < n0) {
    if (p->bpos_sorted) hipFree(p->bpos_sorted);
    if (p->sort_tmp) hipFree(p->sort_tmp);
    p->bpos_sorted = nullptr; p->sort_tmp = nullptr;
    const size_t cap = std::min<size_t>((size_t)n0 + n0 / 2 + 65536, p->map.cap_blocks);
    HIP_TRY(hipMalloc((void**)&p->bpos_sorted, cap * sizeof(uint32_t)));
    size_t bytes = 0;
    HIP_TRY(hipcub::DeviceRadixSort::SortKeys(nullptr, bytes, p->map.bpos, p->bpos_sorted, (int)cap, 0, 30, p->stream));
    HIP_TRY(hipMalloc(&p->sort_tmp, bytes));
    p->sort_tmp_bytes = bytes; p->sort_cap = cap;
  }
  size_t bytes = p->sort_tmp_bytes;
  HIP_TRY(hipcub::DeviceRadixSort::SortKeys(p->sort_tmp, bytes, p->map.bpos, p->bpos_sorted, (int)n0, 0, 30, p->stream));
  HIP_TRY(hipMemcpyAsync(p->map.bpos, p->bpos_sorted, (size_t)n0 * sizeof(uint32_t), hipMemcpyDeviceToDevice, p->stream));
  p->sorted_n = n0; p->sweeps_since_sort = 0;
  return SE_HIP_OK;
}

int se_hip_integrate_sweep(se_hip_pipeline* p, const float pose_cm[16], const float k[4], uint32_t rate, float mu, uint32_t frame) {
  if (int r = check(p)) return r;
  if (!pose_cm || !k || rate == 0) return fail(SE_HIP_E_INVALID, "bad argument");
  if (!finite_pose(pose_cm, k)) return fail(SE_HIP_E_INVALID, "non-finite pose or intrinsics");
  if (!stage_runs_integration(frame, rate)) return 0;
  if (int r = check_overflow(p)) return r;
  if (int r = join_scan(p, true)) return r;
  materialise_depth(p, p->stream);
  input_slot_in_use(p);
  if (int r = sort_block_list(p)) return r;
  const DevMap& m = p->map;
  const M4 pose = from_colmajor(pose_cm);
  const bool sdf = p->cfg.field_type == SE_HIP_FIELD_SDF;
  IntegArgs a{};
  a.commit_occ = p->occ_commit_due ? 1 : 0;
  a.occ_lists = p->occ_lists;
  p->occ_commit_due = false;
  p->occ_lists = OccLists{nullptr, 0, 0};
  for (int i = 0; i < 3; ++i)
    for (int j = 0; j < 3; ++j) a.R[i * 3 + j] = pose.m[j][i];
  const float nt[3] = {pose.m[0][3] * -1.f, pose.m[1][3] * -1.f, pose.m[2][3] * -1.f};
  mul3(a.R, nt, a.t);
  const M4 K = camera_matrix(k);
  for (int i = 0; i < 3; ++i)
    for (int j = 0; j < 3; ++j) a.K3[i * 3 + j] = K.m[i][j];
  M4 Tcw{};
  for (int i = 0; i < 3; ++i) { for (int j = 0; j < 3; ++j) Tcw.m[i][j] = a.R[i * 3 + j]; Tcw.m[i][3] = a.t[i]; }
  Tcw.m[3][0] = Tcw.m[3][1] = Tcw.m[3][2] = 0.f; Tcw.m[3][3] = 1.f;
  const M4 cam = mul(K, Tcw);
  for (int i = 0; i < 3; ++i)
    for (int j = 0; j < 4; ++j) a.cam[i * 4 + j] = cam.m[i][j];
  a.voxel = m.dim / (float)m.size;
  const float vs3[3] = {a.voxel, 0, 0};
  mul3(a.R, vs3, a.delta);
  mul3(a.K3, a.delta, a.cdelta);
  a.mu = mu;
  {
    auto fin = [](float v) { return std::isfinite(v); };
    bool ok = fin(mu) && mu >= 0x1p-30f && mu <= 0x1p30f && fin(a.voxel) && a.voxel >= 0x1p-60f && m.dim <= 0x1p30f;
    for (int i = 0; i < 3 && ok; ++i) {
      float bound = std::fabs(a.t[i]);
      for (int j = 0; j < 3; ++j) bound += std::fabs(a.R[i * 3 + j]) * m.dim;
      ok = fin(bound) && bound < 0x1p40f;
    }
    ok = ok && a.K3[1] == 0.f && a.K3[3] == 0.f && a.K3[6] == 0.f && a.K3[7] == 0.f && a.K3[8] == 1.f;
    for (int i = 0; i < 9; ++i) ok = ok && fin(a.K3[i]) && std::fabs(a.K3[i]) < 0x1p40f;
    a.fast_div = (ok && !p->ieee_sweep) ? 1 : 0;
  }
  a.maxweight = 100.f;
  a.timestamp = (1.f / 30.f) * frame;
  a.W = p->cfg.width; a.H = p->cfg.height;
  a.bspline = p->bspline; a.logodds = p->logodds;
  a.ctr_mirror = p->ctr_host;
  if (p->map.newkeys == p->newkeys_own || p->map.newkeys == p->newkeys_own2) {
    const int other = p->map.newkeys == p->newkeys_own ? 1 : 0;
    a.zero_count = other ? p->newkeys_own2 : p->newkeys_own;
    p->own_clean[other] = true;
    p->own_next = other;
  }
  if (p->shard_world > 1) {
    a.shard_world = p->shard_world; a.shard_rank = p->shard_rank; a.shard_cap = (uint32_t)p->shard_cap;
    a.shard_count = (unsigned long long*)p->shard_send;
    a.shard_recs = (uint32_t*)(p->shard_send + SE_SHARD_SUB * 8);
    a.shard_vx = (float*)(p->shard_send + SE_SHARD_SUB * 8 + p->shard_cap * 4);
    a.shard_vy = a.shard_vx + p->shard_cap * 512;
    HIP_TRY(hipMemsetAsync(p->shard_send, 0, SE_SHARD_SUB * 8, p->stream));
  }
  if (p->prio_hint) {
    a.tile_cost = p->tile_cost; a.prio_thr = p->prio_thr;
    for (int i = 0; i < 3; ++i) a.prio_permille[i] = p->prio_permille[i];
    a.n_tiles = ((p->cfg.width + SE_TILE_W - 1) / SE_TILE_W) * ((p->row_end - p->row_begin + SE_TILE_H - 1) / SE_TILE_H);
    a.ray_order = sdf ? p->ray_order : nullptr;
  }
  const dim3 block(SE_WG);
  {
    ScopedTimer t(p, SE_HIP_K_INTEGRATE);
    const size_t est = (size_t)p->ctr_host[C_BLOCKS] + (size_t)p->ctr_host[C_BLOCKS] / 8 + 2048;
    const size_t wgs = std::min<size_t>(std::max<size_t>((est + 3) / 4, 2048), 65536);
    const dim3 grid(p->integ_grid > 0 ? (unsigned)p->integ_grid : (unsigned)wgs);
#define SE_SWEEP(OF, FD, SHD) hipLaunchKernelGGL((k_integrate<OF, FD, SHD>), grid, block, 0, p->stream, m, p->depth, a)
    a.stats = p->stats ? 1 : 0;
    switch ((sdf ? 0 : 4) | (a.fast_div ? 2 : 0) | (a.shard_world > 1 ? 1 : 0)) {
      case 0: SE_SWEEP(false, false, false); break;
      case 1: SE_SWEEP(false, false, true); break;
      case 2: SE_SWEEP(false, true, false); break;
      case 3: SE_SWEEP(false, true, true); break;
      case 4: SE_SWEEP(true, false, false); break;
      case 5: SE_SWEEP(true, false, true); break;
      case 6: SE_SWEEP(true, true, false); break;
      case 7: SE_SWEEP(true, true, true); break;
    }
#undef SE_SWEEP
  }
  if (p->host_gate) { p->gate_armed = true; p->gate_followed = false; p->gate_target = p->ray_seq + 1u; }
  else {
    hipEventRecord(p->ev_sweep, p->stream);
    if (p->cur_in >= 0) {
      const int i = p->cur_in;
      if (!p->in_done[i]) HIP_TRY(hipEventCreateWithFlags(&p->in_done[i], hipEventDisableTiming));
      HIP_TRY(hipEventRecord(p->in_done[i], p->stream));
      p->in_event[i] = true;
    }
  }
  HIP_TRY(hipGetLastError());
  return 1;
}

static bool frame_can_fuse(se_hip_pipeline* p) {
  const int ray_pairs = (((p->cfg.width + SE_TILE_W - 1) / SE_TILE_W) * ((p->row_end - p->row_begin + SE_TILE_H - 1) / SE_TILE_H) + 1) / 2;
  return p->fuse && !p->ptrs_exposed && p->overlap && !p->stats && p->shard_world <= 1 && ray_pairs <= 10 * p->n_cus;
}
int se_hip_set_streaming(se_hip_pipeline* p, int32_t on) {
  if (int r = check(p)) return r;
  p->fuse = on != 0;
  p->flush_streak = 0;
  return frame_can_fuse(p) ? 1 : 0;
}
int se_hip_frame_is_fused(se_hip_pipeline* p) {
  if (!p) return fail(SE_HIP_E_INVALID, "null handle");
  return frame_can_fuse(p) ? 1 : 0;
}
int se_hip_set_image_ring(se_hip_pipeline* p, float* device_ring, int32_t slots) {
  if (int r = check(p)) return r;
  if ((device_ring != nullptr) != (slots > 0)) return fail(SE_HIP_E_INVALID, "bad argument (ring and slots go together)");
  if (p->ring && device_ring != p->ring && p->vertex != p->vertex_own) {
    const size_t bytes = (size_t)p->cfg.width * p->cfg.height * 3 * sizeof(float);
    HIP_TRY(hipMemcpyAsync(p->vertex_own, p->vertex, bytes, hipMemcpyDeviceToDevice, p->stream));
    HIP_TRY(hipMemcpyAsync(p->normal_own, p->normal, bytes, hipMemcpyDeviceToDevice, p->stream));
    HIP_TRY(hipStreamSynchronize(p->stream));
    p->vertex = p->vertex_own; p->normal = p->normal_own;
  }
  p->ring = device_ring; p->ring_slots = device_ring ? slots : 0;
  return SE_HIP_OK;
}
extern "C++" int flush_pending_raycast(se_hip_pipeline* p) {
  if (!p->has_pending) return SE_HIP_OK;
  InFrame guard(p);
  const int r = se_hip_raycast(p, p->pend_pose, p->pend_k, p->pend_mu, p->pend_frame);
  if (r >= 0) p->has_pending = false;
  return r < 0 ? r : SE_HIP_OK;
}

int se_hip_integrate(se_hip_pipeline* p, const float pose[16], const float k[4], uint32_t rate, float mu, uint32_t frame) {
  if (!p) return fail(SE_HIP_E_INVALID, "null handle");
  InFrame guard(p);
  if (int r = check(p)) return r;
  if (!pose || !k || rate == 0) return fail(SE_HIP_E_INVALID, "bad argument");
  if (!finite_pose(pose, k)) return fail(SE_HIP_E_INVALID, "non-finite pose or intrinsics");
  if (p->has_pending && !(frame_can_fuse(p) && stage_runs_integration(frame, rate))) { if (int r = flush_pending_raycast(p)) return r; }
  int r = se_hip_alloc_scan(p, pose, k, rate, mu, frame);
  if (p->has_pending) { if (int q = flush_pending_raycast(p)) return q; }
  if (r <= 0) return r;
  return se_hip_integrate_sweep(p, pose, k, rate, mu, frame);
}

int se_hip_raycast_deferred(se_hip_pipeline* p, const float pose[16], const float k[4], float mu, uint32_t frame) {
  if (!p) return fail(SE_HIP_E_INVALID, "null handle");
  InFrame guard(p);
  if (int r = check(p)) return r;
  if (!pose || !k) return fail(SE_HIP_E_INVALID, "bad argument");
  if (!finite_pose(pose, k)) return fail(SE_HIP_E_INVALID, "non-finite pose or intrinsics");
  if (p->has_pending) { if (int r = flush_pending_raycast(p)) return r; }
  if (!(frame > 2)) return 0;
  if (!frame_can_fuse(p) || p->flush_streak >= 2) return se_hip_raycast(p, pose, k, mu, frame);
  if (int r = check_overflow(p)) return r;
  std::memcpy(p->pend_pose, pose, sizeof p->pend_pose); std::memcpy(p->pend_k, k, sizeof p->pend_k);
  p->pend_mu = mu; p->pend_frame = frame; p->has_pending = true;
  return 1;
}

int se_hip_frame(se_hip_pipeline* p, const float* device_depth_m, const float pose[16], const float k[4], uint32_t rate, float mu, uint32_t frame) {
  if (!p) return fail(SE_HIP_E_INVALID, "null handle");
  InFrame guard(p);
  if (int r = check(p)) return r;
  if (!pose || !k || rate == 0) return fail(SE_HIP_E_INVALID, "bad argument");
  if (!finite_pose(pose, k)) return fail(SE_HIP_E_INVALID, "non-finite pose or intrinsics");
  if (device_depth_m) { p->depth = device_depth_m; p->cur_in = -1; p->in_pending.kind = 0; }
  int ran = 0;
  int r = se_hip_integrate(p, pose, k, rate, mu, frame);
  if (r < 0) return r;
  ran |= r > 0 ? 1 : 0;
  r = se_hip_raycast_deferred(p, pose, k, mu, frame);
  if (r < 0) return r;
  ran |= r > 0 ? 2 : 0;
  return ran;
}

int se_hip_raycast(se_hip_pipeline* p, const float pose_cm[16], const float k[4], float mu, uint32_t frame) {
  if (int r = check(p)) return r;
  if (!pose_cm || !k) return fail(SE_HIP_E_INVALID, "bad argument");
  if (!finite_pose(pose_cm, k)) return fail(SE_HIP_E_INVALID, "non-finite pose or intrinsics");
  if (!(frame > 2)) return 0;
  if (int r = check_overflow(p)) return r;
  if (int r = join_scan(p)) return r;
  std::memcpy(p->raycast_pose, pose_cm, sizeof p->raycast_pose);
  p->images_complete = !p->sharded;
  select_image_target(p, frame);
  const DevMap& m = p->map;
  RayLaunchArgs L = make_ray_args(p, pose_cm, k, mu);
  if (p->host_gate) { L.a.gate = p->gate_host; L.a.gate_seq = ++p->ray_seq; if (p->gate_armed) p->gate_followed = true; input_slots_followed(p, L.a.gate_seq); }
  const RayArgs& a = L.a;
  const size_t smem = L.smem;
  const dim3 grid = L.grid, block(SE_WG_RAY);
  {
    ScopedTimer t(p, SE_HIP_K_RAYCAST);
#define SE_RAY(OF, ST, DN, SH) hipLaunchKernelGGL((k_raycast<OF, ST, DN, SH>), grid, block, smem, p->stream, m, a, p->vertex, p->normal)
    const RaySel s = ray_kernel_sel(p, a);
    const bool shallow = s.shallow, o32 = s.o32;
    const int variant = (s.ofusion ? 4 : 0) | (p->stats ? 2 : 0) | (s.dense ? 1 : 0);
    switch (variant) {
      case 0: if (shallow) SE_RAY(false, false, false, true); else SE_RAY(false, false, false, false); break;
      case 1: if (o32) hipLaunchKernelGGL((k_raycast<false, false, true, true, true>), grid, block, smem, p->stream, m, a, p->vertex, p->normal);
              else if (shallow) SE_RAY(false, false, true, true); else SE_RAY(false, false, true, false); break;
      case 2: SE_RAY(false, true, false, false); break;
      case 3: SE_RAY(false, true, true, false); break;
      case 4: if (shallow) SE_RAY(true, false, false, true); else SE_RAY(true, false, false, false); break;
      case 5: if (o32) hipLaunchKernelGGL((k_raycast<true, false, true, true, true>), grid, block, smem, p->stream, m, a, p->vertex, p->normal);
              else if (shallow) SE_RAY(true, false, true, true); else SE_RAY(true, false, true, false); break;
      case 6: SE_RAY(true, true, false, false); break;
      case 7: SE_RAY(true, true, true, false); break;
    }
#undef SE_RAY
  }
  HIP_TRY(hipGetLastError());
  return 1;
}

size_t se_hip_image_tile_bytes(se_hip_pipeline* p, int32_t max_rows) {
  if (!p || max_rows <= 0) return 0;
  return (size_t)2 * (size_t)max_rows * (size_t)p->cfg.width * 3 * sizeof(float);
}
int se_hip_pack_image_tile(se_hip_pipeline* p, void* send_device, int32_t max_rows) {
  if (int r = check(p)) return r;
  const int rows = p->row_end - p->row_begin;
  if (!send_device || max_rows < rows) return fail(SE_HIP_E_INVALID, "bad argument (max_rows smaller than this handle's row share)");
  const size_t row_bytes = (size_t)p->cfg.width * 3 * sizeof(float);
  char* dst = (char*)send_device;
  HIP_TRY(hipMemcpyAsync(dst, (const char*)p->vertex + (size_t)p->row_begin * row_bytes, (size_t)rows * row_bytes, hipMemcpyDeviceToDevice, p->stream));
  HIP_TRY(hipMemcpyAsync(dst + (size_t)max_rows * row_bytes, (const char*)p->normal + (size_t)p->row_begin * row_bytes, (size_t)rows * row_bytes, hipMemcpyDeviceToDevice, p->stream));
  return SE_HIP_OK;
}
int se_hip_apply_image_tiles(se_hip_pipeline* p, const void* recv_device, int32_t world, int32_t max_rows, const int32_t* row_begin, const int32_t* row_end) {
  if (int r = check(p)) return r;
  if (!recv_device || world < 1 || max_rows <= 0 || !row_begin || !row_end) return fail(SE_HIP_E_INVALID, "bad argument");
  const size_t row_bytes = (size_t)p->cfg.width * 3 * sizeof(float);
  const size_t tile = (size_t)2 * max_rows * row_bytes;
  for (int r = 0; r < world; ++r) {
    const int b = row_begin[r], e = row_end[r];
    if (b < 0 || e > p->cfg.height || e < b || e - b > max_rows) return fail(SE_HIP_E_INVALID, "bad row partition");
    if (b == p->row_begin && e == p->row_end) continue;
    if (e == b) continue;
    const char* src = (const char*)recv_device + (size_t)r * tile;
    HIP_TRY(hipMemcpyAsync((char*)p->vertex + (size_t)b * row_bytes, src, (size_t)(e - b) * row_bytes, hipMemcpyDeviceToDevice, p->stream));
    HIP_TRY(hipMemcpyAsync((char*)p->normal + (size_t)b * row_bytes, src + (size_t)max_rows * row_bytes, (size_t)(e - b) * row_bytes, hipMemcpyDeviceToDevice, p->stream));
  }
  p->images_complete = true;
  return SE_HIP_OK;
}
int se_hip_gather_images(se_hip_pipeline* p, void* send_device, void* recv_device, int32_t max_rows, const int32_t* row_begin, const int32_t* row_end) {
  if (int r = check(p)) return r;
  if (!p->xgather) return fail(SE_HIP_E_INVALID, "no exchange set (se_hip_set_exchange)");
  if (int r = se_hip_pack_image_tile(p, send_device, max_rows)) return r;
  const int rc = p->xgather(send_device, recv_device, se_hip_image_tile_bytes(p, max_rows),  1, p->xcomm, p->stream);
  if (rc != 0) return fail(SE_HIP_E_DEVICE, "ncclAllGather failed with code " + std::to_string(rc));
  return se_hip_apply_image_tiles(p, recv_device, p->xworld, max_rows, row_begin, row_end);
}

int se_hip_download_vertex_normal(se_hip_pipeline* p, float* v, float* n) {
  if (int r = check(p)) return r;
  const size_t bytes = (size_t)p->cfg.width * p->cfg.height * 3 * sizeof(float);
  if (v) HIP_TRY(hipMemcpyAsync(v, p->vertex, bytes, hipMemcpyDeviceToHost, p->stream));
  if (n) HIP_TRY(hipMemcpyAsync(n, p->normal, bytes, hipMemcpyDeviceToHost, p->stream));
  HIP_TRY(hipStreamSynchronize(p->stream));
  return SE_HIP_OK;
}

int se_hip_vertex_normal_device(se_hip_pipeline* p, float** v, float** n) {
  if (int r = check(p)) return r;
  if (!p->ring) p->ptrs_exposed = true;
  if (v) *v = p->vertex;
  if (n) *n = p->normal;
  return SE_HIP_OK;
}


int se_hip_track(se_hip_pipeline* p, const float k[4], float icp_threshold, uint32_t tracking_rate, uint32_t frame,
                 const int32_t* pyramid, int32_t n_levels, float pose_cm[16]) {
  if (int r = check(p)) return r;
  if (!k || !pose_cm || !pyramid || n_levels < 1 || n_levels > 8 || tracking_rate == 0) return fail(SE_HIP_E_INVALID, "bad argument");
  if (frame % tracking_rate != 0) return 0;
  if (p->sharded && !p->images_complete) return fail(SE_HIP_E_INVALID, "row-sharded handle: se_hip_gather_images / se_hip_apply_image_tiles must follow the raycast before se_hip_track");
  if (int r = join_scan(p)) return r;
  const int W = p->cfg.width, H = p->cfg.height;
  if ((W >> (n_levels - 1)) < 1 || (H >> (n_levels - 1)) < 1) return fail(SE_HIP_E_INVALID, "too many pyramid levels");
  hipStream_t s = p->stream;
  if ((int)p->pyr_vertex.size() < n_levels) {
    p->pyr_depth.resize(n_levels, nullptr); p->pyr_vertex.resize(n_levels, nullptr); p->pyr_normal.resize(n_levels, nullptr);
    for (int i = 0; i < n_levels; ++i) {
      const size_t n = (size_t)(W >> i) * (H >> i);
      if (!p->pyr_depth[i]) HIP_TRY(hipMalloc((void**)&p->pyr_depth[i], n * sizeof(float)));
      if (!p->pyr_vertex[i]) { HIP_TRY(hipMalloc((void**)&p->pyr_vertex[i], n * 3 * sizeof(float))); HIP_TRY(hipMemsetAsync(p->pyr_vertex[i], 0, n * 3 * sizeof(float), s)); }
      if (!p->pyr_normal[i]) { HIP_TRY(hipMalloc((void**)&p->pyr_normal[i], n * 3 * sizeof(float))); HIP_TRY(hipMemsetAsync(p->pyr_normal[i], 0, n * 3 * sizeof(float), s)); }
    }
  }
  if (!p->track) {
    HIP_TRY(hipMalloc((void**)&p->track, (size_t)W * H * sizeof(TrackData)));
// ... 735 lines not shown
    else { const float xv = x; const uint32_t pad = 0; const double yv = y; std::fwrite(&xv, 4, 1, f); std::fwrite(&pad, 4, 1, f); std::fwrite(&yv, 8, 1, f); }
  };
  const int32_t size = p->map.size;
  const float dim = p->map.dim;
  std::fwrite(&size, 4, 1, f);
  std::fwrite(&dim, 4, 1, f);
  uint64_t n = (uint64_t)nn;
  std::fwrite(&n, 8, 1, f);
  for (int i = 0; i < nn; ++i) {
    const int32_t side = (int32_t)nside[i];
    std::fwrite(&ncode[i], 8, 1, f);
    std::fwrite(&side, 4, 1, f);
    for (int j = 0; j < 8; ++j) put_value(nx[(size_t)i * 8 + j], ny[(size_t)i * 8 + j]);
  }
  n = (uint64_t)nb;
  std::fwrite(&n, 8, 1, f);
  for (int i = 0; i < nb; ++i) {
    const uint64_t code = se_make_key(coords[3 * i] >> 3, coords[3 * i + 1] >> 3, coords[3 * i + 2] >> 3, p->leaf_level, p->max_level);
    std::fwrite(&code, 8, 1, f);
    std::fwrite(&coords[3 * (size_t)i], 4, 3, f);
    for (int j = 0; j < 512; ++j) put_value(bx[(size_t)i * 512 + j], by[(size_t)i * 512 + j]);
  }
  const bool okw = std::ferror(f) == 0;
  std::fclose(f);
  return okw ? SE_HIP_OK : fail(SE_HIP_E_INVALID, "write error");
}

int se_hip_load_map(se_hip_pipeline* p, const char* filename) {
  if (int r = check(p)) return r;
  if (!filename) return fail(SE_HIP_E_INVALID, "bad argument");
  FILE* f = std::fopen(filename, "rb");
  if (!f) return fail(SE_HIP_E_INVALID, std::string("cannot open ") + filename);
  const bool sdf = p->cfg.field_type == SE_HIP_FIELD_SDF;
  const size_t vbytes = sdf ? 8 : 16;
  int32_t size = 0; float dim = 0.f; uint64_t nn = 0, nb = 0;
  bool okr = std::fread(&size, 4, 1, f) == 1 && std::fread(&dim, 4, 1, f) == 1 && std::fread(&nn, 8, 1, f) == 1;
  if (!okr || size != p->map.size || dim != p->map.dim) { std::fclose(f); return fail(SE_HIP_E_INVALID, "map file does not match this volume (size / dim)"); }
  if (nn > p->cap_nodes) { std::fclose(f); return fail(SE_HIP_E_CAPACITY, "map file holds more nodes than the pool"); }
  auto get_values = [&](size_t count, float* x, float* y) -> bool {
    std::vector<unsigned char> raw(count * vbytes);
    if (std::fread(raw.data(), 1, raw.size(), f) != raw.size()) return false;
    for (size_t i = 0; i < count; ++i) {
      std::memcpy(&x[i], &raw[i * vbytes], 4);
      if (sdf) std::memcpy(&y[i], &raw[i * vbytes + 4], 4);
      else { double d; std::memcpy(&d, &raw[i * vbytes + 8], 8); y[i] = (float)d; }
    }
    return true;
  };
  std::vector<unsigned long long> keys; keys.reserve((size_t)nn + 1);
  std::vector<float> nx((size_t)nn * 8), ny((size_t)nn * 8);
  for (uint64_t i = 0; i < nn && okr; ++i) {
    unsigned long long code = 0; int32_t side = 0;
    okr = std::fread(&code, 8, 1, f) == 1 && std::fread(&side, 4, 1, f) == 1 && get_values(8, &nx[i * 8], &ny[i * 8]);
    keys.push_back(code);
  }
  okr = okr && std::fread(&nb, 8, 1, f) == 1;
  if (okr && nb > p->cap_blocks) { std::fclose(f); return fail(SE_HIP_E_CAPACITY, "map file holds more blocks than the pool (raise max_blocks)"); }
  std::vector<int32_t> coords((size_t)nb * 3);
  std::vector<float> bx((size_t)nb * 512), by((size_t)nb * 512);
  std::vector<unsigned long long> bkeys((size_t)nb);
  for (uint64_t i = 0; i < nb && okr; ++i) {
    okr = std::fread(&bkeys[i], 8, 1, f) == 1 && std::fread(&coords[i * 3], 4, 3, f) == 3 && get_values(512, &bx[i * 512], &by[i * 512]);
    if (okr) for (int c = 0; c < 3; ++c) okr = okr && coords[i * 3 + c] >= 0 && coords[i * 3 + c] < size && (coords[i * 3 + c] & 7) == 0;
  }
  std::fclose(f);
  if (!okr) return fail(SE_HIP_E_INVALID, "truncated or malformed map file");
  if (p->map.ybyte) {
    for (float w : by) if (!(w >= 0.f && w <= 255.f && w == (float)(int)w)) return fail(SE_HIP_E_INVALID, "map file: a voxel weight is not an integer in 0..255 (SDF weights are stored as bytes)");
  }
  for (unsigned long long kx : keys) {
    const int level = (int)(kx & 0x1FFull);
    if (level == 0 && kx != 0ull) return fail(SE_HIP_E_INVALID, "malformed map file (node key)");
    if (level == 0) continue;
    if (level >= p->leaf_level) return fail(SE_HIP_E_INVALID, "malformed map file (node level)");
    const unsigned long long code = kx & ~0x1FFull;
    const int sh = p->max_level - level;
    const unsigned long long lim = 1ull << level;
    if ((se_compact21(code) >> sh) >= lim || (se_compact21(code >> 1) >> sh) >= lim || (se_compact21(code >> 2) >> sh) >= lim)
      return fail(SE_HIP_E_INVALID, "malformed map file (node position)");
  }
  std::vector<unsigned long long> list;
  list.reserve(1 + keys.size() + bkeys.size());
  list.push_back(0ull);
  for (unsigned long long kx : keys) if ((kx & 0x1FFull) != 0ull) list.push_back(kx);
  for (uint64_t i = 0; i < nb; ++i)
    list.push_back(se_make_key(coords[i * 3] >> 3, coords[i * 3 + 1] >> 3, coords[i * 3 + 2] >> 3, p->leaf_level, p->max_level));
  list[0] = list.size() - 1;
  unsigned long long* d_list = nullptr; float *d_x = nullptr, *d_y = nullptr; int32_t* d_c = nullptr; unsigned long long* d_k = nullptr;
  auto cleanup = [&]() { for (void* q : {(void*)d_list, (void*)d_x, (void*)d_y, (void*)d_c, (void*)d_k}) if (q) hipFree(q); };
  const size_t nval = std::max((size_t)nb * 512, (size_t)nn * 8) + 8;
  if (hipMalloc((void**)&d_list, list.size() * 8) != hipSuccess || hipMalloc((void**)&d_x, nval * 4) != hipSuccess || hipMalloc((void**)&d_y, nval * 4) != hipSuccess ||
      hipMalloc((void**)&d_c, ((size_t)nb * 3 + 4) * 4) != hipSuccess || hipMalloc((void**)&d_k, ((size_t)nn + 1) * 8) != hipSuccess) { cleanup(); return fail(SE_HIP_E_DEVICE, "hipMalloc (load staging)"); }
  if (p->side) HIP_TRY(hipStreamSynchronize(p->side));
  HIP_TRY(hipStreamSynchronize(p->stream));
  p->scan_pending = false; p->occ_commit_due = false; p->occ_lists = OccLists{nullptr, 0, 0};
  reset_map_state(p);
  hipMemcpyAsync(d_list, list.data(), list.size() * 8, hipMemcpyHostToDevice, p->stream);
  hipLaunchKernelGGL(k_alloc_commit, dim3(256, 1), dim3(SE_WG), 0, p->stream, p->map, d_list, 1, (long long)list.size());
  if (nn) {
    hipMemcpyAsync(d_k, keys.data(), (size_t)nn * 8, hipMemcpyHostToDevice, p->stream);
    hipMemcpyAsync(d_x, nx.data(), (size_t)nn * 8 * 4, hipMemcpyHostToDevice, p->stream);
    hipMemcpyAsync(d_y, ny.data(), (size_t)nn * 8 * 4, hipMemcpyHostToDevice, p->stream);
    hipLaunchKernelGGL(k_load_nodes, dim3(grid_for((size_t)nn * 8, SE_WG, 4096)), dim3(SE_WG), 0, p->stream, p->map, d_k, d_x, d_y, (size_t)nn);
    hipStreamSynchronize(p->stream);
  }
  if (nb) {
    hipMemcpyAsync(d_c, coords.data(), (size_t)nb * 3 * 4, hipMemcpyHostToDevice, p->stream);
    hipMemcpyAsync(d_x, bx.data(), (size_t)nb * 512 * 4, hipMemcpyHostToDevice, p->stream);
    hipMemcpyAsync(d_y, by.data(), (size_t)nb * 512 * 4, hipMemcpyHostToDevice, p->stream);
    hipLaunchKernelGGL(k_load_blocks, dim3(grid_for((size_t)nb * 512, SE_WG, 16384)), dim3(SE_WG), 0, p->stream, p->map, d_c, d_x, d_y, (size_t)nb);
  }
  const hipError_t e = hipStreamSynchronize(p->stream);
  cleanup();
  if (e != hipSuccess) return fail(SE_HIP_E_DEVICE, std::string("load_map: ") + hipGetErrorString(e));
  int32_t gb = 0, gn = 0;
  if (int r = se_hip_counts(p, &gb, &gn)) return r;
  if ((uint64_t)gb != nb || (uint64_t)gn != nn) return fail(SE_HIP_E_INVALID, "map file is not ancestor-closed (octants without parents) or holds duplicates");
  return SE_HIP_OK;
}


int se_hip_create_replicas(const se_hip_config* cfg, const int32_t* device_ids, int32_t n_devices, se_hip_pipeline** out_handles) {
  if (!cfg || !device_ids || !out_handles || n_devices < 1) return fail(SE_HIP_E_INVALID, "bad argument");
  const int units = (cfg->height + 7) / 8;
  for (int i = 0; i < n_devices; ++i) out_handles[i] = nullptr;
  for (int i = 0; i < n_devices; ++i) {
    se_hip_config c = *cfg;
    c.device = device_ids[i];
    c.row_begin = std::min(cfg->height, 8 * ((units * i) / n_devices));
    c.row_end = (i + 1 == n_devices) ? cfg->height : std::min(cfg->height, 8 * ((units * (i + 1)) / n_devices));
    const int r = (c.row_end > c.row_begin) ? se_hip_create(&c, &out_handles[i]) : fail(SE_HIP_E_INVALID, "more devices than 8-row image tiles");
    if (r != SE_HIP_OK) { const std::string msg = g_err; for (int j = 0; j < i; ++j) { se_hip_destroy(out_handles[j]); out_handles[j] = nullptr; } return fail(r, msg); }
  }
  return SE_HIP_OK;
}

int se_hip_enable_timing(se_hip_pipeline* p, int32_t on) {
  if (!p) return fail(SE_HIP_E_INVALID, "null handle");
  p->timing = on != 0;
  return SE_HIP_OK;
}

int se_hip_get_timings(se_hip_pipeline* p, double ms_sum[SE_HIP_K_COUNT], int64_t launches[SE_HIP_K_COUNT], int32_t reset) {
  if (int r = check(p)) return r;
  drain_timings(p);
  for (int i = 0; i < SE_HIP_K_COUNT; ++i) {
    if (ms_sum) ms_sum[i] = p->ms_sum[i];
    if (launches) launches[i] = p->launches[i];
    if (reset) { p->ms_sum[i] = 0; p->launches[i] = 0; }
  }
  return SE_HIP_OK;
}

int se_hip_get_launch_counts(se_hip_pipeline* p, int64_t counts[SE_HIP_K_COUNT + 1], int32_t reset) {
  if (!p) return fail(SE_HIP_E_INVALID, "null handle");
  for (int i = 0; i <= SE_HIP_K_COUNT; ++i) {
    if (counts) counts[i] = p->n_launch[i];
    if (reset) p->n_launch[i] = 0;
  }
  return p->has_pending ? 1 : 0;
}

int se_hip_enable_stats(se_hip_pipeline* p, int32_t on) {
  if (int r = check(p)) return r;
  p->stats = on != 0;
  HIP_TRY(hipMemsetAsync(p->map.stats, 0, S_COUNT * sizeof(unsigned long long), p->stream));
  return SE_HIP_OK;
}

int se_hip_get_stats(se_hip_pipeline* p, uint64_t out[16], int32_t reset) {
  if (int r = check(p)) return r;
  if (int r = join_scan(p)) return r;
  unsigned long long h[S_COUNT];
  HIP_TRY(hipMemcpyAsync(h, p->map.stats, sizeof h, hipMemcpyDeviceToHost, p->stream));
  HIP_TRY(hipStreamSynchronize(p->stream));
  if (int r = fetch_counters(p)) return r;
  h[S_NODES] = p->ctr_host[C_NODES];
  for (int i = 0; i < S_COUNT; ++i) out[i] = h[i];
  if (reset) HIP_TRY(hipMemsetAsync(p->map.stats, 0, S_COUNT * sizeof(unsigned long long), p->stream));
  return SE_HIP_OK;
}


}
```

### supereight_amd/csrc/se_kernels.h

```cpp
#pragma once
#include "se_device.h"

#ifndef SE_WG
#define SE_WG 256
#endif
#ifndef SE_WG_RAY
#define SE_WG_RAY 128
#endif
#ifndef SE_WG_SCAN
#define SE_WG_SCAN 128
#endif
#ifndef SE_TILE_W
#define SE_TILE_W 8
#define SE_TILE_H 8
#endif
#define SE_SPEC_OF 8
#ifndef SE_COST_BATCH
#define SE_COST_BATCH 5
#endif

template <typename T>
__device__ __forceinline__ T se_wave_take(T* counter, bool mine) {
  const unsigned long long wm = __ballot(mine);
  if (!mine) return (T)0;
// ... 171 lines not shown
    } else if (e != SE_PENDING) {
      if (a.sharded) { if (se_set_active_once(m, e - 1u)) se_append_key(m, L, bx, by, bz, SE_KEY_ACTIVATE); }
      else m.bactive[e - 1u] = 1;
    }
  }
}
__device__ __forceinline__ int se_cvt_flr(float x) { int r; asm("v_cvt_flr_i32_f32 %0, %1" : "=v"(r) : "v"(x)); return r; }
template <bool STATS, bool DENSE>
__device__ __forceinline__ void se_scan_sdf_wg(const DevMap& m, const float* __restrict__ depthmap, const AllocArgs& a, uint32_t* s_blk_all, int bid, const DepthSrc& ds) {
  uint32_t* s_blk = s_blk_all + threadIdx.x;
  unsigned long long probes = 0, newk = 0;
  int x, y;
  bool in_image;
  {
    const int lane = threadIdx.x & 63;
    const int tile = bid * (SE_WG_SCAN / 64) + (threadIdx.x >> 6);
    if (ds.kind == 0) {
      const int tiles_x = (a.W + 7) >> 3;
      x = (tile % tiles_x) * 8 + (lane & 7);
      y = a.row_begin + (tile / tiles_x) * 8 + (lane >> 3);
    } else {
      const int tiles_x = (a.W + 63) >> 6;
      x = (tile % tiles_x) * 64 + lane;
      y = a.row_begin + tile / tiles_x;
    }
    in_image = x < a.W && y < a.row_end;
  }
  if (in_image) {
    const float depth = se_depth_at(ds, depthmap, x, y, a.W);
    if (!(depth == 0)) {
      const f3 worldVertex = m34_mul_h(a.kpose, {(x + 0.5f) * depth, (y + 0.5f) * depth, depth});
      const f3 camera = {a.cam[0], a.cam[1], a.cam[2]};
      const f3 direction = f3_normalized(f3_sub(camera, worldVertex));
      const f3 origin = f3_sub(worldVertex, f3_scale(a.band * 0.5f, direction));
      const f3 step = f3_div(f3_scale_r(direction, a.band), (float)a.num_steps);
      f3 voxelPos = origin;
      uint32_t last = 0xFFFFFFFFu;
      int nb = 0;
      const bool finite = fabsf(origin.x) < INFINITY && fabsf(origin.y) < INFINITY && fabsf(origin.z) < INFINITY &&
                          fabsf(step.x) < INFINITY && fabsf(step.y) < INFINITY && fabsf(step.z) < INFINITY;
      const uint32_t hi_mask = ~(uint32_t)(m.size - 1);
      const int L = m.leaf_level;
      for (int i = 0; finite && i < a.num_steps; ++i) {
        const f3 s = f3_scale_r(voxelPos, a.inv_voxel);
        const int ix = se_cvt_flr(s.x), iy = se_cvt_flr(s.y), iz = se_cvt_flr(s.z);
        if ((((uint32_t)ix | (uint32_t)iy | (uint32_t)iz) & hi_mask) == 0u) {
          ++probes;
          const uint32_t lin = ((((uint32_t)iz >> 3) << L | ((uint32_t)iy >> 3)) << L) | ((uint32_t)ix >> 3);
          if (lin != last) {
            last = lin;
            if (nb == SE_SCAN_SLOTS) { se_scan_flush<STATS, DENSE>(m, a, s_blk, nb, newk); nb = 0; }
            s_blk[nb * SE_WG_SCAN] = lin;
            ++nb;
          }
        }
        voxelPos = f3_add(voxelPos, step);
      }
      if (nb) se_scan_flush<STATS, DENSE>(m, a, s_blk, nb, newk);
    }
  }
  se_stat_add<STATS>(m, S_PROBES, probes);
  se_stat_add<STATS>(m, S_NEWKEYS, newk);
}
template <bool STATS, bool DENSE>
__global__ __launch_bounds__(SE_WG_SCAN) void k_alloc_scan_sdf(DevMap m, const float* __restrict__ depthmap, AllocArgs a, DepthSrc ds) {
  __shared__ uint32_t s_blk_all[SE_SCAN_SLOTS * SE_WG_SCAN];
  se_scan_sdf_wg<STATS, DENSE>(m, depthmap, a, s_blk_all, (int)blockIdx.x, ds);
}

template <bool STATS>
__device__ __forceinline__ void se_scan_ofusion_wg(const DevMap& m, const float* __restrict__ depthmap, const AllocArgs& a, int bid, const DepthSrc& ds) {
  const int npix = (a.row_end - a.row_begin) * a.W;
  const int pid = bid * SE_WG_SCAN + threadIdx.x;
  unsigned long long probes = 0, newk = 0;
  if (pid < npix) {
    const int x = pid % a.W;
    const int y = a.row_begin + pid / a.W;
    const float depth = se_depth_at(ds, depthmap, x, y, a.W);
    if (!(depth == 0)) {
      int tree_depth = m.max_level;
      float stepsize = a.voxel;
      const f3 worldVertex = m34_mul_h(a.kpose, {(x + 0.5f) * depth, (y + 0.5f) * depth, depth});
      const f3 camera = {a.cam[0], a.cam[1], a.cam[2]};
      const f3 direction = f3_normalized(f3_sub(camera, worldVertex));
      const f3 origin = f3_sub(worldVertex, f3_scale(a.band * 0.5f, direction));
      const float dist = sqrtf(f3_sqnorm(f3_sub(camera, origin)));
      f3 step = f3_scale_r(direction, stepsize);
      f3 voxelPos = origin;
      const float fsize = (float)m.size;
      const float hf_band = a.band, half = a.band * 0.5f;
      int llvl = -1, lox = -1, loy = -1, loz = -1;
      for (float travelled = 0.f; travelled < dist; travelled += stepsize) {
        const f3 s = f3_scale_r(voxelPos, a.inv_voxel);
        const float vx = floorf(s.x), vy = floorf(s.y), vz = floorf(s.z);
        if ((vx < fsize) && (vy < fsize) && (vz < fsize) && (vx >= 0) && (vy >= 0) && (vz >= 0)) {
          ++probes;
          const int lvl = tree_depth < m.leaf_level ? tree_depth : m.leaf_level;
          const int sh = m.max_level - lvl;
          const int ox = (int)vx >> sh, oy = (int)vy >> sh, oz = (int)vz >> sh;
          if (lvl != llvl || ox != lox || oy != loy || oz != loz) {
            llvl = lvl; lox = ox; loy = oy; loz = oz;
            const uint32_t e = m.tab[tab_index(m, lvl, ox, oy, oz)];
            if (e == 0u) {
              if (se_insert_octant(m, lvl, ox, oy, oz)) { se_append_key(m, lvl, ox, oy, oz); ++newk; }
            } else if (tree_depth >= m.leaf_level && e != SE_PENDING) {
              se_mark_active(m, e - 1u, a.sharded != 0, ox, oy, oz);
            }
          }
        }
        if (travelled < hf_band) { stepsize = a.voxel; tree_depth = a.depth_fine; }
        else if (travelled < hf_band + half) { stepsize = 10.f * a.voxel; tree_depth = a.depth_mid; }
        else { stepsize = 30.f * a.voxel; tree_depth = a.depth_coarse; }
        step = f3_scale_r(direction, stepsize);
        voxelPos = f3_add(voxelPos, step);
      }
    }
  }
  se_stat_add<STATS>(m, S_PROBES, probes);
  se_stat_add<STATS>(m, S_NEWKEYS, newk);
}
template <bool STATS>
__global__ __launch_bounds__(SE_WG_SCAN) void k_alloc_scan_ofusion(DevMap m, const float* __restrict__ depthmap, AllocArgs a, DepthSrc ds) {
  se_scan_ofusion_wg<STATS>(m, depthmap, a, (int)blockIdx.x, ds);
}

__global__ __launch_bounds__(SE_WG) void k_alloc_commit(DevMap m, const unsigned long long* __restrict__ lists, int nlists,
                                                         long long stride_words) {
  const int li = blockIdx.y;
  if (li >= nlists) return;
  const unsigned long long* list = lists + (long long)li * stride_words;
  unsigned long long n = list[0];
  if (n > (unsigned long long)(stride_words - 1)) n = (unsigned long long)(stride_words - 1);
  for (unsigned long long i = blockIdx.x * (unsigned long long)SE_WG + threadIdx.x; i < n; i += (unsigned long long)gridDim.x * SE_WG) {
    const unsigned long long raw = list[1 + i];
    const bool activate = (raw & SE_KEY_ACTIVATE) != 0ull;
    const unsigned long long key = raw & ~SE_KEY_ACTIVATE;
    const int level = (int)(key & 0x1FFull);
    if (level < 1 || level > m.leaf_level) continue;
    const unsigned long long code = key & ~0x1FFull;
    const int sh = m.max_level - level;
    const int x = (int)(se_compact21(code) >> sh), y = (int)(se_compact21(code >> 1) >> sh), z = (int)(se_compact21(code >> 2) >> sh);
    if ((unsigned)x >= (1u << level) || (unsigned)y >= (1u << level) || (unsigned)z >= (1u << level)) continue;
    if (activate) {
      if (level != m.leaf_level) continue;
      const uint32_t e = m.tab[leaf_index(m, x, y, z)];
      if (e != 0u && e != SE_PENDING) m.bactive[e - 1u] = 1;
    } else {
      se_insert_octant(m, level, x, y, z);
    }
  }
}

struct OccLists { const unsigned long long* lists; int nlists; long long stride_words; };
__device__ __forceinline__ void se_occ_commit(const DevMap& m, const OccLists L, unsigned nwg, unsigned first = 0u) {
  if (blockIdx.x < first || blockIdx.x >= first + nwg) return;
  const unsigned wg = blockIdx.x - first;
  for (int li = 0; li < L.nlists; ++li) {
    const unsigned long long* list = L.lists + (long long)li * L.stride_words;
    unsigned long long n = list[0];
    if (n > (unsigned long long)(L.stride_words - 1)) n = (unsigned long long)(L.stride_words - 1);
    for (unsigned long long i = wg * (unsigned long long)blockDim.x + threadIdx.x; i < n; i += (unsigned long long)nwg * blockDim.x) {
      const unsigned long long raw = list[1 + i];
      if (raw & SE_KEY_ACTIVATE) continue;
      const int level = (int)(raw & 0x1FFull);
      if (level < 1 || level > m.leaf_level) continue;
      const unsigned long long code = raw & ~0x1FFull;
      const int sh = m.max_level - level;
      int x = (int)(se_compact21(code) >> sh), y = (int)(se_compact21(code >> 1) >> sh), z = (int)(se_compact21(code >> 2) >> sh);
      if ((unsigned)x >= (1u << level) || (unsigned)y >= (1u << level) || (unsigned)z >= (1u << level)) continue;
      if (level == m.leaf_level) se_mark_coarse(m, x, y, z);
      for (int l = level; l >= 1; --l) {
        const uint32_t c = occ_code(l, x, y, z);
        atomicOr(&m.occ[c >> 5], 1u << (c & 31u));
        x >>= 1; y >>= 1; z >>= 1;
      }
    }
  }
}
__global__ __launch_bounds__(SE_WG) void k_occ_commit(DevMap m, OccLists L) { se_occ_commit(m, L, gridDim.x); }

__global__ __launch_bounds__(SE_WG) void k_zero_chain(DevMap m, const unsigned long long* __restrict__ lists, int nlists, long long stride_words) {
  __shared__ unsigned long long s_best[SE_WG / 64];
  __shared__ unsigned long long s_chain[3];
  unsigned long long lower = 0ull;
  for (int pass = 0; pass < 3; ++pass) {
    unsigned long long best = ~0ull;
    for (int li = 0; li < nlists; ++li) {
      const unsigned long long* list = lists + (long long)li * stride_words;
      unsigned long long n = list[0];
      if (n > (unsigned long long)(stride_words - 1)) n = (unsigned long long)(stride_words - 1);
      for (unsigned long long i = threadIdx.x; i < n; i += SE_WG) {
        const unsigned long long k = list[1 + i];
        if (k & SE_KEY_ACTIVATE) continue;
        if ((pass == 0 || k > lower) && k < best) best = k;
      }
    }
    for (int o = 32; o > 0; o >>= 1) { const unsigned long long v = __shfl_down(best, o); if (v < best) best = v; }
    if ((threadIdx.x & 63) == 0) s_best[threadIdx.x >> 6] = best;
    __syncthreads();
    if (threadIdx.x == 0) {
      unsigned long long b = s_best[0];
      for (int w = 1; w < SE_WG / 64; ++w) if (s_best[w] < b) b = s_best[w];
      s_chain[pass] = b;
    }
    __syncthreads();
    lower = s_chain[pass];
    if (lower == ~0ull) break;
  }
  if (threadIdx.x != 0) return;
  unsigned long long cur = s_chain[0];
  if (cur == ~0ull) return;
  for (int j = 1; j < 3; ++j) {
    const unsigned long long nx = s_chain[j];
    if (nx == ~0ull) break;
    const int lvl = (int)(cur & 0x1FFull);
    const int sh = 3 * (m.max_level - lvl);
    if (((nx & ~0x1FFull) >> sh) == ((cur & ~0x1FFull) >> sh)) cur = nx; else break;
  }
  const int level = (int)(cur & 0x1FFull);
  if (level < 1 || level >= m.leaf_level) return;
  const unsigned long long code = cur & ~0x1FFull;
  for (int l = level + 1; l <= m.leaf_level; ++l) {
    const int sh = m.max_level - l;
    const int x = (int)(se_compact21(code) >> sh), y = (int)(se_compact21(code >> 1) >> sh), z = (int)(se_compact21(code >> 2) >> sh);
    se_insert_octant(m, l, x, y, z);
  }
}

#define SE_SHARD_SUB 64
struct IntegArgs {
  float R[9], t[3];
  float K3[9];
  float cam[12];
  float delta[3];
  float cdelta[3];
  float voxel;
  float mu;
  int stats;
  float maxweight;
  float timestamp;
  int W, H;
  const float* bspline;
  const float* logodds;
  int fast_div;
  int commit_occ;
  OccLists occ_lists;
  uint32_t* ctr_mirror;
  unsigned long long* zero_count;
  const unsigned short* tile_cost;
  int n_tiles;
  int* prio_thr;
  int prio_permille[3];
  uint32_t* ray_order;
  int shard_world, shard_rank;
  unsigned long long* shard_count;
  uint32_t* shard_recs;
  float* shard_vx;
  float* shard_vy;
  uint32_t shard_cap;
};

__device__ __forceinline__ void se_ray_schedule(const unsigned short* __restrict__ cost, int n, int* __restrict__ thr, unsigned* hist, const int* permille,
                                                uint32_t* __restrict__ order) {
  static_assert(SE_WG == 256, "se_ray_schedule: one histogram bin per thread");
  __builtin_amdgcn_s_setprio(3);
  unsigned* phist = hist + 256;
  unsigned* base = hist + 512;
  unsigned* wsum = hist + 768;
  int* tmin = (int*)(hist + 776);
  const unsigned tid = threadIdx.x;
  constexpr int CH = 10;
  const int nch = min((n + 7) >> 3, CH * 256);
  const int n_pairs = (n + 1) >> 1;
  const int S = (nch % 37) ? 37 : ((nch % 41) ? 41 : 43);
  uint4 q[CH];
  int ck[CH];
#pragma unroll
  for (int j = 0; j < CH; ++j) {
    const int i = (int)tid + 256 * j;
    ck[j] = i < nch ? (int)(((long long)i * S) % nch) : -1;
    q[j] = ck[j] >= 0 ? *(const uint4*)(cost + 8 * ck[j]) : make_uint4(0u, 0u, 0u, 0u);
  }
  phist[tid] = 0u;
  if (tid < 3u) tmin[tid] = 256;
  __syncthreads();
#pragma unroll
  for (int j = 0; j < CH; ++j) {
    if (ck[j] < 0) continue;
    const unsigned w[4] = {q[j].x, q[j].y, q[j].z, q[j].w};
#pragma unroll
    for (int e = 0; e < 4; ++e) {
      const int t0 = 8 * ck[j] + 2 * e;
      if (t0 >= n) continue;
      const unsigned c0 = w[e] & 0xFFFFu, c1 = (t0 + 1 < n) ? (w[e] >> 16) : c0;
      atomicAdd(&phist[min((c0 + c1) >> 1, 255u)], 1u);
    }
  }
  __syncthreads();
  const unsigned ln = tid & 63u, wv = tid >> 6;
  const unsigned ph = phist[tid];
  unsigned b = ph;
#pragma unroll
  for (int o = 1; o < 64; o <<= 1) {
    const unsigned ub = __shfl_down(b, o);
    if (ln + o < 64u) b += ub;
  }
  if (ln == 0u) wsum[wv] = b;
  __syncthreads();
  for (unsigned w2 = wv + 1; w2 < 4u; ++w2) b += wsum[w2];
  base[tid] = b - ph;
  if (tid >= 1u) {
#pragma unroll
    for (int k = 0; k < 3; ++k) {
      const unsigned lim = (unsigned)((long long)n_pairs * permille[k] / 1000);
      if (b <= lim) atomicMin(&tmin[k], (int)tid);
    }
  }
  __syncthreads();
  if (tid < 3u) thr[tid] = tmin[tid];
  if (order) {
#pragma unroll
    for (int j = 0; j < CH; ++j) {
      if (ck[j] < 0) continue;
      const unsigned w[4] = {q[j].x, q[j].y, q[j].z, q[j].w};
#pragma unroll
      for (int e = 0; e < 4; ++e) {
        const int t0 = 8 * ck[j] + 2 * e;
        if (t0 >= n) continue;
        const unsigned c0 = w[e] & 0xFFFFu, c1 = (t0 + 1 < n) ? (w[e] >> 16) : c0;
        const unsigned cc = min((c0 + c1) >> 1, 255u);
        order[base[cc] + atomicSub(&phist[cc], 1u) - 1u] = (uint32_t)(4 * ck[j] + e);
      }
    }
  }
}

#define SE_LO_DIM 1002

__device__ __forceinline__ void se_sdf_apply(const IntegArgs& a, float depthSample, f3 pos, float& vx, float& vy, bool& dirty) {
  if (depthSample <= 0) return;
  const float diff = (depthSample - pos.z) * sqrtf(1 + sqf(pos.x / pos.z) + sqf(pos.y / pos.z));
  if (diff > -a.mu) {
    const float sdf = fminf(1.f, diff / a.mu);
    vx = clampf((vy * vx + sdf) / (vy + 1.f), -1.f, 1.f);
    vy = fminf(vy + 1, a.maxweight);
    dirty = true;
  }
}
__device__ __forceinline__ int se_bspline_index(float t) {
  const float inverseRange = 1 / 6.f;
  if (t >= -3.0f && t <= 3.0f) return (int)(unsigned)(((t + 3.f) * inverseRange) * (1000.f - 1) + 0.5f);
  if (t > 3) return 1001;
  return 1000;
}
struct SeRcp { float nd, r1; };
__device__ __forceinline__ SeRcp se_rcp_refined(float d) {
  const float r0 = __builtin_amdgcn_rcpf(d);
  const float e0 = __builtin_fmaf(-d, r0, 1.f);
  return {-d, __builtin_fmaf(e0, r0, r0)};
}
__device__ __forceinline__ float se_div_refined(float n, const SeRcp r) {
  const float q0 = n * r.r1;
  const float e1 = __builtin_fmaf(r.nd, q0, n);
  const float q1 = __builtin_fmaf(e1, r.r1, q0);
  const float e2 = __builtin_fmaf(r.nd, q1, n);
  return __builtin_fmaf(e2, r.r1, q1);
}
__device__ __forceinline__ float se_inv_refined(const SeRcp r) {
  const float e1 = __builtin_fmaf(r.nd, r.r1, 1.f);
  const float q1 = __builtin_fmaf(e1, r.r1, r.r1);
  const float e2 = __builtin_fmaf(r.nd, q1, 1.f);
  return __builtin_fmaf(e2, r.r1, q1);
}
__device__ __forceinline__ float se_sqrt_ge1(float s) {
  const float r = __builtin_amdgcn_sqrtf(s);
  const float dn = __uint_as_float(__float_as_uint(r) - 1u), up = __uint_as_float(__float_as_uint(r) + 1u);
  const float vp = __builtin_fmaf(-dn, r, s), vs = __builtin_fmaf(-up, r, s);
  float o = (vp <= 0.f) ? dn : r;
  o = (vs > 0.f) ? up : o;
  return o;
}
template <bool FAST>
__device__ __forceinline__ float se_ray_factor(f3 pos, const SeRcp rz) {
  if (FAST) return se_sqrt_ge1(1 + sqf(se_div_refined(pos.x, rz)) + sqf(se_div_refined(pos.y, rz)));
  return sqrtf(1 + sqf(pos.x / pos.z) + sqf(pos.y / pos.z));
}

template <bool FAST>
__device__ __forceinline__ bool se_sdf_apply_nb(const IntegArgs& a, const SeRcp rmu, bool valid, float depthSample, float posz, float root, float& vx, float& vy) {
  const float diff = (depthSample - posz) * root;
  const bool upd = valid && !(depthSample <= 0) && (diff > -a.mu);
  const float sdf = fminf(1.f, FAST ? se_div_refined(diff, rmu) : diff / a.mu);
  const float nx = clampf((vy * vx + sdf) / (vy + 1.f), -1.f, 1.f);
  const float ny = fminf(vy + 1, a.maxweight);
  vx = upd ? nx : vx;
  vy = upd ? ny : vy;
  return upd;
}
__device__ __forceinline__ bool se_bfusion_apply_nb(const IntegArgs& a, bool valid, float depthSample, float posz, float root, float& vx, float& vy) {
  const float diff = (posz - depthSample) * root;
  const float sigma = clampf(a.mu * sqf(posz), 2 * a.voxel, 0.05f);
  const float tt = diff / sigma;
  const int i1 = se_bspline_index(tt), i2 = se_bspline_index(tt - 3);
  const float q1 = a.bspline[i1 < 1000 ? i1 : 0], q2 = a.bspline[i2 < 1000 ? i2 : 0];
  const float s1 = i1 < 1000 ? q1 : (i1 == 1001 ? 1.f : 0.f), s2 = i2 < 1000 ? q2 : (i2 == 1001 ? 1.f : 0.f);
  const float sample = s1 - s2 * 0.5f;
  const bool upd = valid && !(depthSample <= 0) && !(sample == 0.5f);
  const float lo = a.logodds[i1 * SE_LO_DIM + i2];
  const double delta_t = (double)a.timestamp - (double)vy;
  const float dtf = (float)delta_t;
  float fraction = 1.f / (1.f + (dtf / 4.f));
  fraction = std_max(0.5f, fraction);
  const float nx = clampf(vx * fraction + lo, -1000.f, 1000.f);
  vx = upd ? nx : vx;
  vy = upd ? a.timestamp : vy;
  return upd;
}
__device__ __forceinline__ void se_sdf_update(const IntegArgs& a, const float* __restrict__ depthmap, f3 pos, float px_, float py_,
                                              float& vx, float& vy, bool& dirty) {
  const int px = cvt_i32(px_), py = cvt_i32(py_);
  se_sdf_apply(a, depthmap[px + a.W * py], pos, vx, vy, dirty);
}

__device__ __forceinline__ void se_bfusion_apply(const IntegArgs& a, float depthSample, f3 pos, float& vx, float& vy, bool& dirty) {
  if (depthSample <= 0) return;
  const float diff = (pos.z - depthSample) * sqrtf(1 + sqf(pos.x / pos.z) + sqf(pos.y / pos.z));
  const float sigma = clampf(a.mu * sqf(pos.z), 2 * a.voxel, 0.05f);
  const float tt = diff / sigma;
  const int i1 = se_bspline_index(tt), i2 = se_bspline_index(tt - 3);
  const float q1 = i1 < 1000 ? a.bspline[i1] : (i1 == 1001 ? 1.f : 0.f);
  const float q2 = i2 < 1000 ? a.bspline[i2] : (i2 == 1001 ? 1.f : 0.f);
  const float sample = q1 - q2 * 0.5f;
  if (sample == 0.5f) return;
  const float lo = a.logodds[i1 * SE_LO_DIM + i2];
  const double delta_t = (double)a.timestamp - (double)vy;
  const float dtf = (float)delta_t;
  float fraction = 1.f / (1.f + (dtf / 4.f));
  fraction = std_max(0.5f, fraction);
  vx = vx * fraction;
  vx = clampf(vx + lo, -1000.f, 1000.f);
  vy = a.timestamp;
  dirty = true;
}
__device__ __forceinline__ void se_bfusion_update(const IntegArgs& a, const float* __restrict__ depthmap, f3 pos, float px_, float py_,
                                                  float& vx, float& vy, bool& dirty) {
  const int px = cvt_i32(px_), py = cvt_i32(py_);
  se_bfusion_apply(a, depthmap[px + a.W * py], pos, vx, vy, dirty);
}

__device__ __forceinline__ bool se_in_frustum(const IntegArgs& a, int bx8, int by8, int bz8) {
  const f3 p = {(float)bx8 * a.voxel, (float)by8 * a.voxel, (float)bz8 * a.voxel};
  const f3 vc = m34_mul_h(a.cam, p);
  const int px = cvt_i32(vc.x / vc.z), py = cvt_i32(vc.y / vc.z);
  return px >= 0 && px < a.W && py >= 0 && py < a.H;
}

template <bool OFUSION>
__device__ __forceinline__ void se_update_node_corner(const DevMap& m, const float* __restrict__ depthmap, const IntegArgs& a, uint32_t tid) {
  const uint32_t n = tid >> 3;
  const int i = tid & 7;
  const int level = m.nlevel[n];
  const uint32_t np = m.npos[n];
  const int sh = m.max_level - level;
  const unsigned side = (unsigned)m.size >> level;
  const int vx0 = ((int)(np & 1023u) << sh) + (level & 1) + (((level >> 3) & 1) << 1);
  const int vy0 = ((int)((np >> 10) & 1023u) << sh) + ((level >> 1) & 1);
  const int vz0 = ((int)(np >> 20) << sh) + ((level >> 2) & 1);
  const float s = 0.5f * a.voxel * side;
  const f3 delta = m3_mul(a.R, {s, s, s});
  const f3 delta_c = m3_mul(a.K3, delta);
  const f3 base_cam = f3_add(m3_mul(a.R, f3_scale(a.voxel, {(float)vx0, (float)vy0, (float)vz0})), {a.t[0], a.t[1], a.t[2]});
  const f3 basepix_hom = m3_mul(a.K3, base_cam);
  const f3 dir = {(float)((i & 1) > 0), (float)((i & 2) > 0), (float)((i & 4) > 0)};
  const f3 vox_cam = f3_add(base_cam, f3_mul(dir, delta));
  const f3 pix_hom = f3_add(basepix_hom, f3_mul(dir, delta_c));
  if (vox_cam.z < 0.0001f) return;
  const float inverse_depth = 1.f / pix_hom.z;
  const float pixx = pix_hom.x * inverse_depth + 0.5f;
  const float pixy = pix_hom.y * inverse_depth + 0.5f;
  if (pixx < 0.5f || pixx > a.W - 1.5f || pixy < 0.5f || pixy > a.H - 1.5f) return;
  float vx = m.nx[tid], vy = m.ny[tid];
  bool dirty = false;
  if (OFUSION) se_bfusion_update(a, depthmap, vox_cam, pixx, pixy, vx, vy, dirty);
  else se_sdf_update(a, depthmap, vox_cam, pixx, pixy, vx, vy, dirty);
  if (dirty) { m.nx[tid] = vx; m.ny[tid] = vy; }
}

#ifndef SE_SWEEP_WAVES
#define SE_SWEEP_WAVES 5
#endif
#if SE_SWEEP_WAVES > 0
#define SE_SWEEP_OCC __attribute__((amdgpu_waves_per_eu(SE_SWEEP_WAVES, SE_SWEEP_WAVES)))
#else
#define SE_SWEEP_OCC
#endif
template <bool OFUSION, bool FAST, bool SHARD>
__global__ __launch_bounds__(SE_WG) SE_SWEEP_OCC void k_integrate(DevMap m, const float* __restrict__ depthmap, IntegArgs a) {
  const int lane = threadIdx.x & 63;
  const int wave = (blockIdx.x * SE_WG + threadIdx.x) >> 6;
  const int nwaves = (gridDim.x * SE_WG) >> 6;
  const uint32_t nblocks = min(m.ctr[C_BLOCKS], m.cap_blocks);
  const uint32_t nnodes = min(m.ctr[C_NODES], m.cap_nodes);
  const int lx = lane & 7, ly = lane >> 3;
  const float fx = (float)lx;
  unsigned long long swept = 0;
  if (a.ctr_mirror && blockIdx.x == gridDim.x - 1 && threadIdx.x < C_COUNT) a.ctr_mirror[threadIdx.x] = m.ctr[threadIdx.x];
  if (a.zero_count && blockIdx.x == gridDim.x - 1 && threadIdx.x == 0) *a.zero_count = 0ull;
  __shared__ unsigned s_hist[784];
  const bool scheduler = a.prio_thr != nullptr && gridDim.x > 1;
  const int wskip = scheduler ? SE_WG / 64 : 0;
  if (a.commit_occ) se_occ_commit(m, a.occ_lists, min(gridDim.x - (scheduler ? 1u : 0u), 64u), scheduler ? 1u : 0u);
  if (scheduler && blockIdx.x == 0) se_ray_schedule(a.tile_cost, a.n_tiles, a.prio_thr, s_hist, a.prio_permille, a.ray_order);
  const SeRcp rmu = se_rcp_refined(a.mu);
  const uint32_t stride = (uint32_t)(nwaves - wskip);
  uint32_t b = (scheduler && blockIdx.x == 0) ? 0xFFFFFFFFu : (uint32_t)(wave - wskip);
  uint32_t bp_next = m.bpos[min(b, m.cap_blocks - 1u)];
  for (; b < nblocks; b += stride) {
    const uint32_t bp = bp_next;
    bp_next = m.bpos[min(b + stride, m.cap_blocks - 1u)];
    const int bx = (int)(bp & 1023u) << 3, by = (int)((bp >> 10) & 1023u) << 3, bz = (int)(bp >> 20) << 3;
    if (SHARD && (unsigned)((bx >> 3) + (by >> 3) + (bz >> 3)) % (unsigned)a.shard_world != (unsigned)a.shard_rank) continue;
    const uint32_t slot = block_slot(m, b, bp);
    float* px = m.vx + (size_t)slot * 1024 + lane;
    float* py = px + 512;
    uint2* pyb = (uint2*)(m.vx + (size_t)slot * 1024 + 512) + lane;
    uint2 wy = {0u, 0u};
    float vx[8], vy[8];
    const unsigned char act = m.bactive[slot];
    if (!act && !se_in_frustum(a, bx, by, bz)) continue;
    if (a.stats && lane == 0) ++swept;
    {
#pragma unroll
      for (int zi = 0; zi < 8; ++zi) { vx[zi] = px[zi * 64]; if (OFUSION) vy[zi] = py[zi * 64]; }
      if (!OFUSION) {
        wy = *pyb;
#pragma unroll
        for (int zi = 0; zi < 8; ++zi) vy[zi] = (float)(((zi < 4 ? wy.x : wy.y) >> (8 * (zi & 3))) & 255u);
      }
    }
    bool visible = false;
    const int y = by + ly;
    int pidx[8];
    bool valid[8], upd[8];
    float ds[8], posz[8], root[8];
#pragma unroll
    for (int zi = 0; zi < 8; ++zi) {
      const int z = bz + zi;
      const f3 start = f3_add(m3_mul(a.R, {bx * a.voxel, y * a.voxel, z * a.voxel}), {a.t[0], a.t[1], a.t[2]});
      const f3 pos = f3_add(start, f3_scale(fx, {a.delta[0], a.delta[1], a.delta[2]}));
      float cvx, cvy, inverse_depth;
      SeRcp rz = {0.f, 0.f};
      if (FAST) {
        cvx = (a.K3[0] * start.x + a.K3[2] * start.z) + fx * a.cdelta[0];
        cvy = (a.K3[4] * start.y + a.K3[5] * start.z) + fx * a.cdelta[1];
        rz = se_rcp_refined(pos.z);
        inverse_depth = se_inv_refined(rz);
      } else {
        const f3 camera_voxel = f3_add(m3_mul(a.K3, start), f3_scale(fx, {a.cdelta[0], a.cdelta[1], a.cdelta[2]}));
        cvx = camera_voxel.x; cvy = camera_voxel.y;
        inverse_depth = 1.f / camera_voxel.z;
      }
      const float pixx = cvx * inverse_depth + 0.5f;
      const float pixy = cvy * inverse_depth + 0.5f;
      valid[zi] = !(pos.z < 0.0001f) && !(pixx < 0.5f || pixx > a.W - 1.5f || pixy < 0.5f || pixy > a.H - 1.5f);
      visible = visible || valid[zi];
      pidx[zi] = valid[zi] ? se_cvt_hw(pixx) + a.W * se_cvt_hw(pixy) : 0;
      ds[zi] = depthmap[pidx[zi]];
      posz[zi] = pos.z;
      root[zi] = se_ray_factor<FAST>(pos, rz);
    }
#pragma unroll
    for (int zi = 0; zi < 8; ++zi)
      upd[zi] = OFUSION ? se_bfusion_apply_nb(a, valid[zi], ds[zi], posz[zi], root[zi], vx[zi], vy[zi])
                        : se_sdf_apply_nb<FAST>(a, rmu, valid[zi], ds[zi], posz[zi], root[zi], vx[zi], vy[zi]);
#pragma unroll
    for (int zi = 0; zi < 8; ++zi) {
      if (__ballot(upd[zi]) != 0ull) {
        px[zi * 64] = vx[zi];
        if (OFUSION) py[zi * 64] = vy[zi];
      }
    }
    if (!OFUSION) {
      bool u = false;
#pragma unroll
      for (int zi = 0; zi < 8; ++zi) u = u || upd[zi];
      if (__ballot(u) != 0ull) {
        uint2 o;
        o.x = (uint32_t)(int)vy[0] | ((uint32_t)(int)vy[1] << 8) | ((uint32_t)(int)vy[2] << 16) | ((uint32_t)(int)vy[3] << 24);
        o.y = (uint32_t)(int)vy[4] | ((uint32_t)(int)vy[5] << 8) | ((uint32_t)(int)vy[6] << 16) | ((uint32_t)(int)vy[7] << 24);
        *pyb = o;
      }
    }
    const bool any = __ballot(visible) != 0ull;
    if (lane == 0) m.bactive[slot] = any ? 1 : 0;
    if (SHARD) {
      const uint32_t sub = (uint32_t)wave & (SE_SHARD_SUB - 1), subcap = a.shard_cap / SE_SHARD_SUB;
      uint32_t rec = 0u;
      if (lane == 0) rec = (uint32_t)atomicAdd(a.shard_count + sub, 1ull);
      rec = (uint32_t)__builtin_amdgcn_readfirstlane((int)rec);
      const bool fits = rec < subcap;
      rec += sub * subcap;
      if (fits) {
        if (lane == 0) a.shard_recs[rec] = bp | (any ? 0x80000000u : 0u);
        if (any) {
          float* sx = a.shard_vx + (size_t)rec * 512 + lane;
          float* sy = a.shard_vy + (size_t)rec * 512 + lane;
#pragma unroll
          for (int zi = 0; zi < 8; ++zi) { sx[zi * 64] = vx[zi]; sy[zi * 64] = vy[zi]; }
        }
      } else if (lane == 0) {
        m.ctr[C_OVERFLOW] = 3u;
      }
    }
  }
  if (a.stats && lane == 0 && swept) atomicAdd(&m.stats[S_SWEPT], swept);
  for (uint32_t tid = blockIdx.x * SE_WG + threadIdx.x; tid < nnodes * 8u; tid += gridDim.x * SE_WG)
    se_update_node_corner<OFUSION>(m, depthmap, a, tid);
}

__global__ __launch_bounds__(SE_WG) void k_apply_bricks(DevMap m, const unsigned char* __restrict__ recv, size_t seg_bytes, uint32_t cap, int self) {
  const int seg = blockIdx.y;
  if (seg == self) return;
  const unsigned char* base = recv + (size_t)seg * seg_bytes;
  const unsigned long long* counts = (const unsigned long long*)base;
  const uint32_t* recs = (const uint32_t*)(base + SE_SHARD_SUB * 8);
  const float* bvx = (const float*)(base + SE_SHARD_SUB * 8 + (size_t)cap * 4);
  const float* bvy = bvx + (size_t)cap * 512;
  const int lane = threadIdx.x & 63;
  const uint32_t wave = (blockIdx.x * SE_WG + threadIdx.x) >> 6, nwaves = (gridDim.x * SE_WG) >> 6;
  const uint32_t subcap = cap / SE_SHARD_SUB;
  const uint32_t sub = wave & (SE_SHARD_SUB - 1);
  const uint32_t n = (uint32_t)min(counts[sub], (unsigned long long)subcap);
  if (counts[sub] > (unsigned long long)subcap && lane == 0 && wave < SE_SHARD_SUB) m.ctr[C_OVERFLOW] = 3u;
  for (uint32_t j = wave / SE_SHARD_SUB; j < n; j += nwaves / SE_SHARD_SUB) {
    const uint32_t i = sub * subcap + j;
    const uint32_t r = recs[i], bp = r & 0x3FFFFFFFu;
    const int bx = (int)(bp & 1023u), by = (int)((bp >> 10) & 1023u), bz = (int)(bp >> 20);
    const uint32_t e = m.dense ? block_linear(m, bx, by, bz) + 1u : m.tab[leaf_index(m, bx, by, bz)];
    if (e == 0u || e == SE_PENDING) continue;
    const uint32_t slot = e - 1u;
    if (lane == 0) m.bactive[slot] = (unsigned char)(r >> 31);
    if (r >> 31) {
      const float* sx = bvx + (size_t)i * 512 + lane;
      const float* sy = bvy + (size_t)i * 512 + lane;
      float* dx = m.vx + (size_t)slot * SE_BRICK_STRIDE + lane;
#pragma unroll
      for (int zi = 0; zi < 8; ++zi) { dx[zi * 64] = sx[zi * 64]; se_st_y(m, (size_t)slot * SE_BRICK_STRIDE + lane + zi * 64, sy[zi * 64]); }
    }
  }
}

struct RayArgs {
  float view3[9];
  float org[3];
  float nearp, farp, mu, step, largestep;
  float near_n, far_n;
  float scaled_origin[3];
  float inv_voxel;
  float grad_scale;
  float epsilon;
  int min_scale;
  int W, H, row_begin, row_end;
  int cache_levels;
  int cache_words;
  uint32_t cache_codes;
  int has_deep;
  int stack_depth;
  int beam;
  float beam_dt, beam_cell, beam_inv_cell, inv_dim;
  float beam_dt2, beam_cellf, beam_inv_cellf;
  const uint32_t* leap_bits;
  int leap_level;
  float leap_dt;
  const uint32_t* ray_order;
  int n_cus;
  uint32_t* gate;
  uint32_t gate_seq;
  unsigned short* tile_cost;
  int cost_shift;
  const int* prio_thr;
  unsigned long long* wlog;
};

struct BlkCache { int bx, by, bz; uint32_t e; };
struct FieldConst { float init_x, init_y, empty_x; };
__device__ __forceinline__ FieldConst se_field_const(const DevMap& m) {
  FieldConst f = {m.init_x, m.init_y, m.empty_x};
  asm volatile("" : "+s"(f.init_x), "+s"(f.init_y), "+s"(f.empty_x));
  return f;
}

__device__ __forceinline__ size_t se_voxel_index(uint32_t e, int x, int y, int z) {
  return (size_t)(e - 1u) * SE_BRICK_STRIDE + (size_t)((x & 7) + ((y & 7) << 3) + ((z & 7) << 6));
}


template <bool DENSE>
__device__ __forceinline__ uint32_t se_block_entry(const DevMap& m, int bx, int by, int bz, const BlkCache& hint) {
  const int nb = m.size >> 3;
  uint32_t e = 0u;
  if (DENSE) return ((unsigned)bx < (unsigned)nb && (unsigned)by < (unsigned)nb && (unsigned)bz < (unsigned)nb) ? block_linear(m, bx, by, bz) + 1u : 0u;
  if (bx == hint.bx && by == hint.by && bz == hint.bz) e = hint.e;
  else if ((unsigned)bx < (unsigned)nb && (unsigned)by < (unsigned)nb && (unsigned)bz < (unsigned)nb) e = m.tab[leaf_index(m, bx, by, bz)];
  return e == SE_PENDING ? 0u : e;
}

template <bool DENSE>
__device__ __forceinline__ float se_interp_generic(const DevMap& m, const FieldConst fc, f3 pos, BlkCache& c) {
  const float flx = floorf(pos.x), fly = floorf(pos.y), flz = floorf(pos.z);
  const int bx = cvt_i32(flx), by = cvt_i32(fly), bz = cvt_i32(flz);
  const float fx = pos.x - flx, fy = pos.y - fly, fz = pos.z - flz;
  const int lx = max(bx, 0), ly = max(by, 0), lz = max(bz, 0);
  const bool cx = (lx & 7) == 7, cy = (ly & 7) == 7, cz = (lz & 7) == 7;
  const float missing = (cx && cy && cz) ? fc.init_x : fc.empty_x;
  uint32_t e[8];
  e[0] = se_block_entry<DENSE>(m, lx >> 3, ly >> 3, lz >> 3, c);
#pragma unroll
  for (int k = 1; k < 8; ++k) {
    const bool need = (!(k & 1) || cx) && (!(k & 2) || cy) && (!(k & 4) || cz);
    e[k] = 0u;
    if (need) e[k] = se_block_entry<DENSE>(m, (lx + (k & 1)) >> 3, (ly + ((k >> 1) & 1)) >> 3, (lz + (k >> 2)) >> 3, c);
  }
  uint32_t ex1[4], exy[2][2][2];
#pragma unroll
  for (int q = 0; q < 4; ++q) ex1[q] = cx ? e[2 * q + 1] : e[2 * q];
#pragma unroll
  for (int sz = 0; sz < 2; ++sz) {
    exy[0][0][sz] = e[4 * sz];
    exy[1][0][sz] = ex1[2 * sz];
    exy[0][1][sz] = cy ? e[4 * sz + 2] : e[4 * sz];
    exy[1][1][sz] = cy ? ex1[2 * sz + 1] : ex1[2 * sz];
  }
  const uint32_t ox[2] = {(uint32_t)lx & 7u, (uint32_t)(lx + 1) & 7u};
  const uint32_t oy[2] = {((uint32_t)ly & 7u) << 3, ((uint32_t)(ly + 1) & 7u) << 3};
  const uint32_t oz[2] = {((uint32_t)lz & 7u) << 6, ((uint32_t)(lz + 1) & 7u) << 6};
  float p[8];
#pragma unroll
  for (int k = 0; k < 8; ++k) {
    const int i = k & 1, j = (k >> 1) & 1, kz = k >> 2;
    const uint32_t ek = kz ? (cz ? exy[i][j][1] : exy[i][j][0]) : exy[i][j][0];
    const size_t vi = ek ? (size_t)(ek - 1u) * SE_BRICK_STRIDE + (size_t)(ox[i] + oy[j] + oz[kz]) : 0;
    const float v = m.vx[vi];
    p[k] = ek ? v : missing;
  }
  return (((p[0] * (1 - fx) + p[1] * fx) * (1 - fy) + (p[2] * (1 - fx) + p[3] * fx) * fy) * (1 - fz) +
          ((p[4] * (1 - fx) + p[5] * fx) * (1 - fy) + (p[6] * (1 - fx) + p[7] * fx) * fy) * fz);
}

struct AxisTerm { uint32_t blk, loc; };
__device__ __forceinline__ AxisTerm se_axis_x(int x) { return {(uint32_t)(x >> 3), (uint32_t)(x & 7)}; }
__device__ __forceinline__ AxisTerm se_axis_y(const DevMap& m, int y) { return {(uint32_t)(y >> 3) << m.leaf_level, (uint32_t)(y & 7) << 3}; }
__device__ __forceinline__ AxisTerm se_axis_z(const DevMap& m, int z) { return {(uint32_t)(z >> 3) << (2 * m.leaf_level), (uint32_t)(z & 7) << 6}; }
__device__ __forceinline__ size_t se_axis_index(AxisTerm a, AxisTerm b, AxisTerm c) {
  return (size_t)(a.blk + b.blk + c.blk) * SE_BRICK_STRIDE + (size_t)(a.loc + b.loc + c.loc);
}

template <bool DENSE>
__device__ __forceinline__ f3 se_grad_generic(const DevMap& m, const FieldConst fc, f3 pos, BlkCache& c) {
  const float flx = floorf(pos.x), fly = floorf(pos.y), flz = floorf(pos.z);
  const int bx = cvt_i32(flx), by = cvt_i32(fly), bz = cvt_i32(flz);
  const float fx = pos.x - flx, fy = pos.y - fly, fz = pos.z - flz;
  const int hi = m.size - 1;
  const int X[4] = {max(bx - 1, 0), max(bx, 0), min(bx + 1, hi), min(bx + 2, hi)};
  const int Y[4] = {max(by - 1, 0), max(by, 0), min(by + 1, hi), min(by + 2, hi)};
  const int Z[4] = {max(bz - 1, 0), max(bz, 0), min(bz + 1, hi), min(bz + 2, hi)};
  const int xb0 = X[0] >> 3, yb0 = Y[0] >> 3, zb0 = Z[0] >> 3;
  const int xb1 = X[3] >> 3, yb1 = Y[3] >> 3, zb1 = Z[3] >> 3;
  uint32_t e[8];
#pragma unroll
  for (int k = 0; k < 8; ++k) e[k] = se_block_entry<DENSE>(m, (k & 1) ? xb1 : xb0, (k & 2) ? yb1 : yb0, (k & 4) ? zb1 : zb0, c);
// ... 1196 lines not shown
```

### supereight_amd/pipeline.py

```python
from __future__ import annotations

import ctypes as C
import os

import numpy as np

from . import build as _build

SDF, OFUSION = 0, 1
KERNELS = ("alloc_scan", "alloc_commit", "integrate", "raycast", "apply_bricks")
STAT_NAMES = ("probes", "new_keys", "swept", "nodes", "gets", "interps", "grads", "hits",
              "clk_iter", "clk_march", "clk_grad", "clk_wave_max", "clk_stage", "r13", "r14", "r15")

_f32p = np.ctypeslib.ndpointer(dtype=np.float32, flags="C_CONTIGUOUS")
_LIB = None


class SeHipError(RuntimeError):
    pass


class _QueryOut(C.Structure):
    _fields_ = [("fine", C.c_void_p), ("coarse", C.c_void_p), ("interp", C.c_void_p), ("grad", C.c_void_p), ("status", C.c_void_p)]


class _RayOut(C.Structure):
    _fields_ = [("hit", C.c_void_p), ("normal", C.c_void_p), ("status", C.c_void_p)]


class _MeshView(C.Structure):
    _fields_ = [("pose", C.c_float * 16), ("k", C.c_float * 4), ("width", C.c_int32), ("height", C.c_int32)]


class _MeshSelect(C.Structure):
    _fields_ = [("lo", C.c_int32 * 3), ("hi", C.c_int32 * 3), ("n_views", C.c_int32), ("flags", C.c_uint32), ("views", C.POINTER(_MeshView))]


class _MeshOut(C.Structure):
    _fields_ = [("triangles", C.c_void_p), ("capacity_triangles", C.c_int64), ("block_coords", C.c_void_p), ("block_range", C.c_void_p),
                ("capacity_blocks", C.c_int64), ("header", C.c_void_p)]


MESH_MAX_VIEWS, MESH_SKIP_EMPTY = 64, 1

RAY_VALID, RAY_ENTERED, RAY_HIT, RAY_NORMAL = 1, 2, 4, 8


class _CollideTest(C.Structure):
    _fields_ = [("threshold", C.c_float), ("occupied_above", C.c_int32)]


COLLISION_OCCUPIED, COLLISION_UNSEEN, COLLISION_EMPTY, COLLISION_INVALID = 0, 1, 2, 255
_COLLIDE_MODES = {"strict": 0, "reference": 1}


class _Edit(C.Structure):
    _fields_ = [("lo", C.c_int32 * 3), ("hi", C.c_int32 * 3), ("x", C.c_float), ("y", C.c_float), ("flags", C.c_uint32), ("only", C.c_uint32)]


EDIT_DTYPE = np.dtype([("lo", np.int32, 3), ("hi", np.int32, 3), ("x", np.float32), ("y", np.float32), ("flags", np.uint32), ("only", np.uint32)])
EDIT_SET_X, EDIT_SET_Y, EDIT_BLOCKS, EDIT_NODES = 1, 2, 4, 8
EDIT_OCCUPIED, EDIT_UNSEEN, EDIT_EMPTY, EDIT_ANY = 1, 2, 4, 7
_EDIT_MODES = {"strict": 0, "reference": 1}
_EDIT_CLASSES = {"occupied": EDIT_OCCUPIED, "unseen": EDIT_UNSEEN, "empty": EDIT_EMPTY, "any": EDIT_ANY}


class _AllocBox(C.Structure):
    _fields_ = [("lo", C.c_int32 * 3), ("hi", C.c_int32 * 3), ("level", C.c_int32), ("reserved", C.c_uint32)]


ALLOC_DTYPE = np.dtype([("lo", np.int32, 3), ("hi", np.int32, 3), ("level", np.int32), ("reserved", np.uint32)])


class _Config(C.Structure):
    _fields_ = [("width", C.c_int32), ("height", C.c_int32), ("volume_resolution", C.c_int32),
                ("volume_dimension", C.c_float), ("field_type", C.c_int32), ("device", C.c_int32),
                ("max_blocks", C.c_int64), ("row_begin", C.c_int32), ("row_end", C.c_int32)]


EXPORTS = {
    "se_hip_create": (C.c_int, [C.POINTER(_Config), C.POINTER(C.c_void_p)]),
    "se_hip_destroy": (C.c_int, [C.c_void_p]),
    "se_hip_last_error": (C.c_char_p, []),
    "se_hip_sync": (C.c_int, [C.c_void_p]),
    "se_hip_memory_info": (C.c_int, [C.c_void_p, C.POINTER(C.c_int64)]),
    "se_hip_set_pinned_input": (C.c_int, [C.c_void_p, C.c_int32]),
    "se_hip_host_alloc": (C.c_void_p, [C.c_size_t]),
    "se_hip_host_free": (None, [C.c_void_p]),
    "se_hip_clear_overflow": (C.c_int, [C.c_void_p]),
    "se_hip_set_stream": (C.c_int, [C.c_void_p, C.c_void_p]),
    "se_hip_set_scan_stream": (C.c_int, [C.c_void_p, C.c_void_p]),
    "se_hip_scan_overlaps": (C.c_int, [C.c_void_p]),
    "se_hip_frame_is_fused": (C.c_int, [C.c_void_p]),
    "se_hip_set_streaming": (C.c_int, [C.c_void_p, C.c_int32]),
    "se_hip_set_image_ring": (C.c_int, [C.c_void_p, C.c_void_p, C.c_int32]),
    "se_hip_raycast_deferred": (C.c_int, [C.c_void_p, C.c_void_p, C.c_void_p, C.c_float, C.c_uint32]),
    "se_hip_get_launch_counts": (C.c_int, [C.c_void_p, C.POINTER(C.c_int64), C.c_int32]),
    "se_hip_upload_depth": (C.c_int, [C.c_void_p, _f32p]),
    "se_hip_upload_depth_mm": (C.c_int, [C.c_void_p, np.ctypeslib.ndpointer(dtype=np.uint16, flags="C_CONTIGUOUS"), C.c_int32, C.c_int32]),
    "se_hip_set_depth_device": (C.c_int, [C.c_void_p, C.c_void_p]),
    "se_hip_integrate": (C.c_int, [C.c_void_p, C.c_void_p, C.c_void_p, C.c_uint32, C.c_float, C.c_uint32]),
    "se_hip_alloc_scan": (C.c_int, [C.c_void_p, C.c_void_p, C.c_void_p, C.c_uint32, C.c_float, C.c_uint32]),
    "se_hip_new_keys_device": (C.c_int, [C.c_void_p, C.POINTER(C.c_void_p), C.POINTER(C.c_int64)]),
    "se_hip_set_new_keys_buffer": (C.c_int, [C.c_void_p, C.c_void_p, C.c_int64]),
    "se_hip_alloc_commit": (C.c_int, [C.c_void_p, C.c_void_p, C.c_int32, C.c_int64]),
    "se_hip_set_exchange": (C.c_int, [C.c_void_p, C.c_void_p, C.c_void_p, C.c_int32]),
    "se_hip_alloc_exchange": (C.c_int, [C.c_void_p, C.c_void_p, C.c_int64]),
    "se_hip_integrate_sweep": (C.c_int, [C.c_void_p, C.c_void_p, C.c_void_p, C.c_uint32, C.c_float, C.c_uint32]),
    "se_hip_sweep_shard_bytes": (C.c_size_t, [C.c_size_t]),
    "se_hip_set_sweep_shard": (C.c_int, [C.c_void_p, C.c_int32, C.c_int32, C.c_void_p, C.c_size_t]),
    "se_hip_apply_bricks": (C.c_int, [C.c_void_p, C.c_void_p, C.c_int32]),
    "se_hip_brick_exchange": (C.c_int, [C.c_void_p, C.c_void_p]),
    "se_hip_raycast": (C.c_int, [C.c_void_p, C.c_void_p, C.c_void_p, C.c_float, C.c_uint32]),
    "se_hip_image_tile_bytes": (C.c_size_t, [C.c_void_p, C.c_int32]),
    "se_hip_pack_image_tile": (C.c_int, [C.c_void_p, C.c_void_p, C.c_int32]),
    "se_hip_apply_image_tiles": (C.c_int, [C.c_void_p, C.c_void_p, C.c_int32, C.c_int32, C.c_void_p, C.c_void_p]),
    "se_hip_gather_images": (C.c_int, [C.c_void_p, C.c_void_p, C.c_void_p, C.c_int32, C.c_void_p, C.c_void_p]),
    "se_hip_frame": (C.c_int, [C.c_void_p, C.c_void_p, C.c_void_p, C.c_void_p, C.c_uint32, C.c_float, C.c_uint32]),
    "se_hip_download_vertex_normal": (C.c_int, [C.c_void_p, _f32p, _f32p]),
    "se_hip_vertex_normal_device": (C.c_int, [C.c_void_p, C.POINTER(C.c_void_p), C.POINTER(C.c_void_p)]),
    "se_hip_frame_tracked": (C.c_int, [C.c_void_p, C.c_void_p, C.c_void_p, C.c_float, C.c_uint32, C.c_void_p, C.c_int32, C.c_void_p, C.c_uint32, C.c_float, C.c_uint32]),
    "se_hip_track": (C.c_int, [C.c_void_p, C.c_void_p, C.c_float, C.c_uint32, C.c_uint32, C.c_void_p, C.c_int32, C.c_void_p]),
    "se_hip_filter_depth": (C.c_int, [C.c_void_p, C.c_int32]),
    "se_hip_download_scaled_depth": (C.c_int, [C.c_void_p, C.c_int32, C.c_void_p]),
    "se_hip_download_track": (C.c_int, [C.c_void_p, C.c_void_p, C.c_void_p, C.POINTER(C.c_int32)]),
    "se_hip_render_volume": (C.c_int, [C.c_void_p, C.c_void_p, _f32p, _f32p, C.c_float, C.c_float, C.c_uint32, C.c_uint32]),
    "se_hip_render_depth": (C.c_int, [C.c_void_p, C.c_void_p]),
    "se_hip_render_track": (C.c_int, [C.c_void_p, C.c_void_p]),
    "se_hip_save_map": (C.c_int, [C.c_void_p, C.c_char_p]),
    "se_hip_load_map": (C.c_int, [C.c_void_p, C.c_char_p]),
    "se_hip_create_replicas": (C.c_int, [C.POINTER(_Config), C.POINTER(C.c_int32), C.c_int32, C.POINTER(C.c_void_p)]),
    "se_hip_mesh_count": (C.c_int, [C.c_void_p, C.POINTER(C.c_int64)]),
    "se_hip_mesh_download": (C.c_int, [C.c_void_p, C.c_void_p, C.c_int64, C.POINTER(C.c_int64)]),
    "se_hip_dump_mesh": (C.c_int, [C.c_void_p, C.c_char_p]),
    "se_hip_counts": (C.c_int, [C.c_void_p, C.POINTER(C.c_int32), C.POINTER(C.c_int32)]),
    "se_hip_download_blocks": (C.c_int, [C.c_void_p, C.c_void_p, C.c_void_p, C.c_void_p, C.c_void_p]),
    "se_hip_download_nodes": (C.c_int, [C.c_void_p, C.c_void_p, C.c_void_p, C.c_void_p, C.c_void_p]),
    "se_hip_enable_timing": (C.c_int, [C.c_void_p, C.c_int32]),
    "se_hip_get_timings": (C.c_int, [C.c_void_p, C.POINTER(C.c_double), C.POINTER(C.c_int64), C.c_int32]),
    "se_hip_enable_stats": (C.c_int, [C.c_void_p, C.c_int32]),
    "se_hip_get_stats": (C.c_int, [C.c_void_p, C.POINTER(C.c_uint64), C.c_int32]),
    "se_hip_query_points": (C.c_int, [C.c_void_p, C.c_void_p, C.c_int64, C.POINTER(_QueryOut)]),
    "se_hip_query_points_host": (C.c_int, [C.c_void_p, C.c_void_p, C.c_int64, C.POINTER(_QueryOut)]),
    "se_hip_collide_boxes": (C.c_int, [C.c_void_p, C.c_void_p, C.c_int64, C.POINTER(_CollideTest), C.c_int32, C.c_void_p]),
    "se_hip_collide_boxes_host": (C.c_int, [C.c_void_p, C.c_void_p, C.c_int64, C.POINTER(_CollideTest), C.c_int32, C.c_void_p]),
    "se_hip_edit_boxes": (C.c_int, [C.c_void_p, C.c_void_p, C.c_int64, C.POINTER(_CollideTest), C.c_int32, C.c_void_p]),
    "se_hip_edit_boxes_host": (C.c_int, [C.c_void_p, C.c_void_p, C.c_int64, C.POINTER(_CollideTest), C.c_int32, C.c_void_p]),
    "se_hip_allocate_boxes": (C.c_int, [C.c_void_p, C.c_void_p, C.c_int64, C.c_void_p, C.c_void_p, C.c_int64]),
    "se_hip_allocate_boxes_host": (C.c_int, [C.c_void_p, C.c_void_p, C.c_int64, C.c_void_p, C.c_void_p, C.c_int64]),
    "se_hip_cast_rays": (C.c_int, [C.c_void_p, C.c_void_p, C.c_int64, C.c_float, C.POINTER(_RayOut)]),
    "se_hip_cast_rays_host": (C.c_int, [C.c_void_p, C.c_void_p, C.c_int64, C.c_float, C.POINTER(_RayOut)]),
    "se_hip_mesh_blocks": (C.c_int, [C.c_void_p, C.POINTER(_MeshSelect), C.POINTER(_MeshOut)]),
    "se_hip_mesh_blocks_host": (C.c_int, [C.c_void_p, C.POINTER(_MeshSelect), C.POINTER(_MeshOut)]),
}


def _share_torch_hip_runtime() -> None:
    import importlib.util
    import sys
    if "torch" in sys.modules:
        return
    try:
        spec = importlib.util.find_spec("torch")
    except (ImportError, ValueError):
        spec = None
    for base in (spec.submodule_search_locations or []) if spec else []:
        cand = os.path.join(base, "lib", "libamdhip64.so")
        if os.path.exists(cand):
            C.CDLL(cand, mode=C.RTLD_GLOBAL)
            return


def load_library(rebuild: bool = True):
    global _LIB
    if _LIB is None:
        _share_torch_hip_runtime()
        path = _build.LIB
        alt = os.environ.get("SE_HIP_LIB")
        if alt:
            import sys
            print(f"supereight_amd: SE_HIP_LIB is set -- loading {alt} instead of the in-tree libse_hip.so (A/B tooling)", file=sys.stderr)
            path, rebuild = alt, False
        if rebuild:
            try:
                path = _build.build()
            except RuntimeError:
                if not os.path.exists(path):
                    raise
        lib = C.CDLL(path)
        for name, (res, args) in EXPORTS.items():
            fn = getattr(lib, name)
            fn.restype, fn.argtypes = res, args
        _LIB = lib
    return _LIB


def _colmajor(m) -> np.ndarray:
    return np.ascontiguousarray(np.asarray(m, dtype=np.float32).reshape(4, 4).T).reshape(16)


def _torch_module(obj):
    import sys
    torch = sys.modules.get("torch")
    return torch if torch is not None and isinstance(obj, torch.Tensor) else None


class DenseSLAMPipeline:
    _k_last = _k_arr = _pyr_arr = None
    _k_addr = 0
    _device = None

    def __init__(self, input_size, volume_resolution: int, volume_dimension: float, init_pose=None,
                 field_type: int = SDF, device: int = 0, max_blocks: int = 0, rows=None, streaming: bool = False):
        self.lib = load_library()
        self.W, self.H = int(input_size[0]), int(input_size[1])
        self.size, self.dim, self.field = int(volume_resolution), float(volume_dimension), field_type
        self._device = int(device)
        rb, re_ = rows if rows is not None else (0, 0)
        cfg = _Config(self.W, self.H, self.size, self.dim, field_type, device, max_blocks, rb, re_)
        h = C.c_void_p()
        self._h = None
        self._check(self.lib.se_hip_create(C.byref(cfg), C.byref(h)))
        self._h = h
        self.pose_ = np.eye(4, dtype=np.float32) if init_pose is None else init_pose
        self._keepalive = None
        self._ring_keepalive = None
        self._pinned = []
        if streaming:
            self.set_streaming(True)

    @property
    def pose_(self):
        if self._pose is None:
            self._pose = self._pose_cm.reshape(4, 4).T.copy()
        return self._pose

    @pose_.setter
    def pose_(self, m):
        self._pose = np.array(m, dtype=np.float32).reshape(4, 4)
        self._pose_cm = np.ascontiguousarray(self._pose.T).reshape(16)
        self._pose_cm_addr = self._pose_cm.ctypes.data

    @staticmethod
    def _addr(a, dtype, size: int) -> int:
        if not (type(a) is np.ndarray and a.dtype == dtype and a.size == size and a.flags.c_contiguous):
            raise TypeError(f"expected a C-contiguous {np.dtype(dtype).name}[{size}] array")
        return a.ctypes.data

    def _k(self, k) -> int:
        if type(k) is int:
            return k
        if isinstance(k, np.integer):
            return int(k)
        if k is self._k_last:
            return self._k_addr
        if type(k) is np.ndarray and k.dtype == np.float32 and k.size == 4 and k.flags.c_contiguous:
            self._k_last, self._k_arr = k, k
        else:
            self._k_last, self._k_arr = None, np.ascontiguousarray(k, dtype=np.float32).reshape(4)
        self._k_addr = self._k_arr.ctypes.data
        return self._k_addr

    @staticmethod
    def addr(a) -> int:
        if not (type(a) is np.ndarray and a.dtype == np.float32 and a.flags.c_contiguous):
            raise TypeError("expected a C-contiguous float32 array")
        return a.ctypes.data

    def _check(self, status: int) -> int:
        if status < 0:
            raise SeHipError(f"se_hip error {status}: {self.lib.se_hip_last_error().decode()}")
        return status

    def close(self):
        if getattr(self, "_h", None):
            self.lib.se_hip_destroy(self._h)
            self._h = None
            for ptr in getattr(self, "_pinned", []):
                self.lib.se_hip_host_free(ptr)
            self._pinned = []

    def __del__(self):
        try:
            self.close()
        except Exception:
            pass

    def sync(self):
        self._check(self.lib.se_hip_sync(self._h))

    def clear_overflow(self) -> int:
        return self._check(self.lib.se_hip_clear_overflow(self._h))

    def set_stream(self, hip_stream_ptr: int):
        self._check(self.lib.se_hip_set_stream(self._h, C.c_void_p(hip_stream_ptr)))

    def scan_overlaps(self) -> bool:
        return bool(self._check(self.lib.se_hip_scan_overlaps(self._h)))

    def frame_is_fused(self) -> bool:
        return bool(self._check(self.lib.se_hip_frame_is_fused(self._h)))

    def set_streaming(self, on: bool = True) -> bool:
        return bool(self._check(self.lib.se_hip_set_streaming(self._h, int(on))))

    def set_image_ring(self, ptr: int, slots: int, keepalive=None):
        self._check(self.lib.se_hip_set_image_ring(self._h, C.c_void_p(ptr), slots))
        self._ring_keepalive = keepalive

    def launch_counts(self, reset: bool = False) -> dict:
        n = (C.c_int64 * (len(KERNELS) + 1))()
        pend = self._check(self.lib.se_hip_get_launch_counts(self._h, n, int(reset)))
        out = {k: int(n[i]) for i, k in enumerate(KERNELS)}
        out["fused"] = int(n[len(KERNELS)])
        out["pending"] = bool(pend)
        return out

    def set_scan_stream(self, hip_stream_ptr: int):
        self._check(self.lib.se_hip_set_scan_stream(self._h, C.c_void_p(hip_stream_ptr)))

    def setPose(self, pose):
        self.pose_ = pose

    def getPose(self):
        return self.pose_.copy()

    def set_depth(self, depth_m):
        d = np.ascontiguousarray(depth_m, dtype=np.float32).reshape(-1)
        assert d.size == self.W * self.H
        self._check(self.lib.se_hip_upload_depth(self._h, d))

    def set_depth_mm(self, depth_mm):
        d = np.ascontiguousarray(depth_mm, dtype=np.uint16)
        self._check(self.lib.se_hip_upload_depth_mm(self._h, d.reshape(-1), d.shape[1], d.shape[0]))

    def set_depth_device(self, ptr: int, keepalive=None):
        self._keepalive = keepalive
        self._check(self.lib.se_hip_set_depth_device(self._h, C.c_void_p(ptr)))

    def integration(self, k, integration_rate: int, mu: float, frame: int) -> bool:
        return bool(self._check(self.lib.se_hip_integrate(self._h, self._pose_cm_addr, self._k(k),
                                                          integration_rate, mu, frame)))

    def frame(self, depth_ptr: int, pose_cm, k, mu: float, frame: int, integration_rate: int = 1) -> int:
        if type(pose_cm) is not int:
            pose_cm = int(pose_cm) if isinstance(pose_cm, np.integer) else self._addr(pose_cm, np.float32, 16)
        return self._check(self.lib.se_hip_frame(self._h, depth_ptr, pose_cm, self._k(k), integration_rate, mu, frame))

    def raycasting(self, k, mu: float, frame: int) -> bool:
        return bool(self._check(self.lib.se_hip_raycast(self._h, self._pose_cm_addr, self._k(k), mu, frame)))

    def raycasting_deferred(self, k, mu: float, frame: int) -> bool:
        return bool(self._check(self.lib.se_hip_raycast_deferred(self._h, self._pose_cm_addr, self._k(k), mu, frame)))

    def mesh(self) -> np.ndarray:
        n = C.c_int64()
        self._check(self.lib.se_hip_mesh_count(self._h, C.byref(n)))
        out = np.empty((n.value, 3, 3), np.float32)
        if n.value:
            w = C.c_int64()
            self._check(self.lib.se_hip_mesh_download(self._h, out.ctypes.data, n.value, C.byref(w)))
            out = out[: w.value]
        return out

    def dump_mesh(self, filename: str):
        self._check(self.lib.se_hip_dump_mesh(self._h, filename.encode()))

    def filter_depth(self, on: bool = True):
        self._check(self.lib.se_hip_filter_depth(self._h, int(on)))

    def scaled_depth(self, level: int = 0) -> np.ndarray:
        out = np.empty((self.H >> level, self.W >> level), np.float32)
        self._check(self.lib.se_hip_download_scaled_depth(self._h, level, out.ctypes.data))
        return out

    TRACK_DTYPE = np.dtype([("result", np.int32), ("error", np.float32), ("J", np.float32, 6)])

    _PYRAMID = np.asarray((10, 5, 4), np.int32)
    _PYRAMID_ADDR = _PYRAMID.ctypes.data

    def _pyr(self, pyramid):
        if pyramid is None or pyramid is self._PYRAMID or tuple(pyramid) == (10, 5, 4):
            return self._PYRAMID_ADDR, 3
        self._pyr_arr = np.ascontiguousarray(pyramid, dtype=np.int32).reshape(-1)
        return self._pyr_arr.ctypes.data, self._pyr_arr.size

    def tracking(self, k, icp_threshold: float, tracking_rate: int, frame: int, pyramid=None) -> bool:
        pa, n = self._pyr(pyramid)
        r = self._check(self.lib.se_hip_track(self._h, self._k(k), icp_threshold, tracking_rate, frame, pa, n, self._pose_cm_addr))
        self._pose = None
        return bool(r)

    def frame_tracked(self, depth_ptr: int, k, mu: float, frame: int, icp_threshold: float = 1e-5, tracking_rate: int = 1,
                      integration_rate: int = 1, pyramid=None) -> int:
        pa, n = self._pyr(pyramid)
        r = self._check(self.lib.se_hip_frame_tracked(self._h, depth_ptr, self._k(k), icp_threshold, tracking_rate, pa, n,
                                                      self._pose_cm_addr, integration_rate, mu, frame))
        self._pose = None
        return r

    def track_data(self):
        t = np.zeros(self.W * self.H, self.TRACK_DTYPE)
        red = np.zeros(32, np.float32)
        it = C.c_int32()
        self._check(self.lib.se_hip_download_track(self._h, t.ctypes.data, red.ctypes.data, C.byref(it)))
        return t.reshape(self.H, self.W), red, it.value

    def renderVolume(self, view_pose, k, mu, largestep, frame=0, rate=1):
        out = np.zeros((self.H, self.W, 4), np.uint8)
        ran = self._check(self.lib.se_hip_render_volume(self._h, out.ctypes.data, _colmajor(view_pose), np.asarray(k, np.float32), mu, largestep, frame, rate))
        return out if ran else None

    def renderDepth(self):
        out = np.zeros((self.H, self.W, 4), np.uint8)
        self._check(self.lib.se_hip_render_depth(self._h, out.ctypes.data))
        return out

    def renderTrack(self):
        out = np.zeros((self.H, self.W, 4), np.uint8)
        self._check(self.lib.se_hip_render_track(self._h, out.ctypes.data))
        return out

    def alloc_scan(self, k, integration_rate: int, mu: float, frame: int) -> bool:
        return bool(self._check(self.lib.se_hip_alloc_scan(self._h, self._pose_cm_addr, self._k(k),
                                                           integration_rate, mu, frame)))

    def new_keys_device(self):
        ptr, cap = C.c_void_p(), C.c_int64()
        self._check(self.lib.se_hip_new_keys_device(self._h, C.byref(ptr), C.byref(cap)))
        return ptr.value, cap.value

    def set_new_keys_buffer(self, ptr: int, capacity_words: int, keepalive=None):
        self._keys_keepalive = keepalive
        self._check(self.lib.se_hip_set_new_keys_buffer(self._h, C.c_void_p(ptr), capacity_words))

    def alloc_commit(self, lists_ptr: int, nlists: int, stride_words: int):
        self._check(self.lib.se_hip_alloc_commit(self._h, C.c_void_p(lists_ptr), nlists, stride_words))

    def set_exchange(self, nccl_comm: int, nccl_all_gather: int, world: int):
        self._check(self.lib.se_hip_set_exchange(self._h, C.c_void_p(nccl_comm), C.c_void_p(nccl_all_gather), world))

    def alloc_exchange(self, recv_ptr: int, words: int):
        self._check(self.lib.se_hip_alloc_exchange(self._h, C.c_void_p(recv_ptr), words))

    def sweep_shard_bytes(self, cap_bricks: int) -> int:
        return int(self.lib.se_hip_sweep_shard_bytes(cap_bricks))

    def set_sweep_shard(self, rank: int, world: int, send_ptr: int, cap_bricks: int, keepalive=None):
        self._check(self.lib.se_hip_set_sweep_shard(self._h, rank, world, C.c_void_p(send_ptr), cap_bricks))
        self._shard_keepalive = keepalive

    def apply_bricks(self, recv_ptr: int, world: int):
        self._check(self.lib.se_hip_apply_bricks(self._h, C.c_void_p(recv_ptr), world))

    def brick_exchange(self, recv_ptr: int):
        self._check(self.lib.se_hip_brick_exchange(self._h, C.c_void_p(recv_ptr)))

    def integrate_sweep(self, k, integration_rate: int, mu: float, frame: int) -> bool:
        return bool(self._check(self.lib.se_hip_integrate_sweep(self._h, self._pose_cm_addr, self._k(k),
                                                                integration_rate, mu, frame)))

    def vertex_normal(self):
        v = np.zeros((self.H, self.W, 3), np.float32)
        n = np.zeros((self.H, self.W, 3), np.float32)
        self._check(self.lib.se_hip_download_vertex_normal(self._h, v.reshape(-1), n.reshape(-1)))
        return v, n

# ... 420 lines not shown
```

Before: 17020.

## Fuse allocation scan and integration sweep into one launch with device-side handover

The allocation scan is held back and launched with the integration sweep as a single kernel. The first workgroups run the scan and publish completion through an atomic counter. The sweep workgroups spin-wait on that counter before reading block counts and committing occupancy. For ofusion, the last scan workgroup also runs the zero-chain step. This removes a kernel launch and its inter-kernel gap per frame. The risks are spin-wait polling cost and the possibility that the sweep times out if scan workgroups are not scheduled, which is reported as a new error code.

```diff
diff --git a/include/se_hip.h b/include/se_hip.h
--- a/include/se_hip.h
+++ b/include/se_hip.h
@@ -15,6 +15,7 @@
 #define SE_HIP_E_DEVICE (-2)
 #define SE_HIP_E_CAPACITY (-3)
 #define SE_HIP_E_NOGPU (-4)
+#define SE_HIP_E_HANDOVER (-5)
 
 typedef struct se_hip_pipeline se_hip_pipeline;
 
@@ -201,6 +202,7 @@
 int se_hip_enable_timing(se_hip_pipeline* p, int32_t on);
 int se_hip_get_timings(se_hip_pipeline* p, double ms_sum[SE_HIP_K_COUNT], int64_t launches[SE_HIP_K_COUNT], int32_t reset);
 int se_hip_get_launch_counts(se_hip_pipeline* p, int64_t counts[SE_HIP_K_COUNT + 1], int32_t reset);
+int se_hip_get_fused_scan_sweep(se_hip_pipeline* p, int64_t* count, int32_t reset);
 int se_hip_enable_stats(se_hip_pipeline* p, int32_t on);
 int se_hip_get_stats(se_hip_pipeline* p, uint64_t out[16], int32_t reset);
 
diff --git a/supereight_amd/csrc/se_hip_api.hip b/supereight_amd/csrc/se_hip_api.hip
--- a/supereight_amd/csrc/se_hip_api.hip
+++ b/supereight_amd/csrc/se_hip_api.hip
@@ -193,6 +193,13 @@
   int prio_permille[3] = {400, 150, 50};
   uint32_t* ray_order = nullptr;
   int n_cus = 256;
+  bool fuse_scan_sweep = true;
+  bool hold_scan_ok = false;
+  struct HeldScan { bool valid = false; DevMap ms; AllocArgs a; int wgs = 0; } held;
+  uint32_t* scan_done = nullptr;
+  int done_next = 0;
+  bool done_clean[2] = {false, false};
+  int64_t n_fused_scan_sweep = 0;
 };
 
 namespace {
@@ -410,6 +417,7 @@
 
 int check_overflow(se_hip_pipeline* p) {
   const uint32_t o = p->ctr_host[C_OVERFLOW];
+  if (o == SE_OVERFLOW_HANDOVER) return fail(SE_HIP_E_HANDOVER, "scan + sweep launch: the sweep gave up waiting for the allocation scan (the frame was not integrated; SE_HIP_FUSE_SCAN_SWEEP=0 selects the two launches)");
   if (o == 3) return fail(SE_HIP_E_CAPACITY, "brick exchange segment overflow: the peers missed block updates (raise cap_bricks of se_hip_set_sweep_shard)");
   if (o) return fail(SE_HIP_E_CAPACITY, o == 2 ? "new-key list overflow: blocks were allocated locally but not reported to the peers (raise the exchange capacity)"
                                               : "block / node pool exhausted (raise max_blocks)");
@@ -556,6 +564,7 @@
   if (const char* ev = std::getenv("SE_HIP_BEAM")) p->beam = std::max(0, std::min(2, std::atoi(ev)));
   if (const char* ev = std::getenv("SE_HIP_OF_LEAP")) p->of_leap = std::atoi(ev) != 0;
   if (const char* ev = std::getenv("SE_HIP_IEEE_SWEEP")) p->ieee_sweep = std::atoi(ev) != 0;
+  if (const char* ev = std::getenv("SE_HIP_FUSE_SCAN_SWEEP")) p->fuse_scan_sweep = std::atoi(ev) != 0;
   if (const char* ev = std::getenv("SE_HIP_PRIO")) p->prio_hint = std::atoi(ev) != 0;
   if (const char* ev = std::getenv("SE_HIP_PRIO_SHARE")) {
     int a = 0, b = 0, c = 0;
@@ -643,6 +652,9 @@
   const size_t n_tiles = ((size_t)(cfg->width + SE_TILE_W - 1) / SE_TILE_W) * ((size_t)(cfg->height + SE_TILE_H - 1) / SE_TILE_H);
   ALLOC(p->tile_cost, (n_tiles + 4096) * sizeof(unsigned short));
   ALLOC(p->prio_thr, 4 * sizeof(int));
+  ALLOC(p->scan_done, 4 * sizeof(uint32_t));
+  hipMemsetAsync(p->scan_done, 0, 4 * sizeof(uint32_t), p->stream);
+  p->done_clean[0] = p->done_clean[1] = true;
   hipMemsetAsync(p->tile_cost, 0, (n_tiles + 4096) * sizeof(unsigned short), p->stream);
   {
     hipDeviceProp_t prop{};
@@ -692,7 +704,7 @@
   for (auto& ev : p->event_pool) hipEventDestroy(ev);
   DevMap& m = p->map;
   void* ptrs[] = {m.occ, m.lbits, m.cbits, m.fbits, m.tab, m.vx, m.bpos, m.bactive, m.nx, m.ny, m.npos, m.nlevel, m.ctr, m.stats, p->newkeys_own, p->newkeys_own2,
-                  p->depth_ring[0], p->depth_ring[1], p->depth_ring[2], p->vertex_own, p->normal_own, p->bspline, p->logodds, p->chain, p->tile_cost, p->prio_thr, p->ray_order};
+                  p->depth_ring[0], p->depth_ring[1], p->depth_ring[2], p->vertex_own, p->normal_own, p->bspline, p->logodds, p->chain, p->tile_cost, p->prio_thr, p->ray_order, p->scan_done};
   for (void* q : ptrs) if (q) hipFree(q);
   for (auto* q : p->pyr_depth) if (q) hipFree(q);
   for (auto* q : p->pyr_vertex) if (q) hipFree(q);
@@ -738,6 +750,7 @@
   HIP_TRY(hipMemsetAsync(p->map.ctr + C_OVERFLOW, 0, sizeof(uint32_t), p->stream));
   HIP_TRY(hipStreamSynchronize(p->stream));
   p->ctr_host[C_OVERFLOW] = 0u;
+  p->done_clean[0] = p->done_clean[1] = false;
   return (int)pending;
 }
 
@@ -879,6 +892,39 @@
 }
 
 static bool frame_can_fuse(se_hip_pipeline* p);
+static void launch_scan(se_hip_pipeline* p, const DevMap& ms, const AllocArgs& a, const DepthSrc& ds, hipStream_t s) {
+  const DevMap& m = p->map;
+  const bool sdf = p->cfg.field_type == SE_HIP_FIELD_SDF;
+  const int rows = a.row_end - a.row_begin;
+  const dim3 grid((rows * a.W + SE_WG_SCAN - 1) / SE_WG_SCAN), block(SE_WG_SCAN);
+  const int sdf_tiles = ds.kind ? ((a.W + 63) / 64) * rows : ((a.W + 7) / 8) * ((rows + 7) / 8);
+  ScopedTimer t(p, SE_HIP_K_ALLOC_SCAN, s);
+  if (sdf) {
+    const dim3 sgrid((sdf_tiles + SE_WG_SCAN / 64 - 1) / (SE_WG_SCAN / 64));
+    if (m.dense) {
+      if (p->stats) hipLaunchKernelGGL((k_alloc_scan_sdf<true, true>), sgrid, block, 0, s, ms, p->depth, a, ds);
+      else hipLaunchKernelGGL((k_alloc_scan_sdf<false, true>), sgrid, block, 0, s, ms, p->depth, a, ds);
+    } else {
+      if (p->stats) hipLaunchKernelGGL((k_alloc_scan_sdf<true, false>), sgrid, block, 0, s, ms, p->depth, a, ds);
+      else hipLaunchKernelGGL((k_alloc_scan_sdf<false, false>), sgrid, block, 0, s, ms, p->depth, a, ds);
+    }
+  } else {
+    if (p->stats) hipLaunchKernelGGL(k_alloc_scan_ofusion<true>, grid, block, 0, s, ms, p->depth, a, ds);
+    else hipLaunchKernelGGL(k_alloc_scan_ofusion<false>, grid, block, 0, s, ms, p->depth, a, ds);
+  }
+}
+static int launch_held_scan(se_hip_pipeline* p) {
+  if (!p->held.valid) return SE_HIP_OK;
+  p->held.valid = false;
+  launch_scan(p, p->held.ms, p->held.a, DepthSrc{nullptr, nullptr, 0, 0, 0}, p->stream);
+  if (p->cfg.field_type != SE_HIP_FIELD_SDF) { if (int r = run_zero_chain(p, p->map.newkeys, 1, (long long)p->map.cap_keys + 1)) return r; }
+  HIP_TRY(hipGetLastError());
+  return SE_HIP_OK;
+}
+static bool fuse_scan_sweep_ok(se_hip_pipeline* p, int scan_wgs) {
+  return p->fuse_scan_sweep && !p->stats && !p->timing && !p->sharded && p->shard_world <= 1 && p->xgather == nullptr && SE_SWEEP_WAVES > 0 &&
+         scan_wgs <= SE_SWEEP_WAVES * p->n_cus;
+}
 int se_hip_alloc_scan(se_hip_pipeline* p, const float pose_cm[16], const float k[4], uint32_t rate, float mu, uint32_t frame) {
   if (!p) return fail(SE_HIP_E_INVALID, "null handle");
   const bool ride = p->has_pending && !p->in_frame && rate != 0 && stage_runs_integration(frame, rate) && frame_can_fuse(p);
@@ -946,21 +992,11 @@
     HIP_TRY(hipGetLastError());
     return 1;
   }
-  {
-    ScopedTimer t(p, SE_HIP_K_ALLOC_SCAN, s);
-    if (sdf) {
-      const dim3 sgrid((sdf_tiles + SE_WG_SCAN / 64 - 1) / (SE_WG_SCAN / 64));
-      if (m.dense) {
-        if (p->stats) hipLaunchKernelGGL((k_alloc_scan_sdf<true, true>), sgrid, block, 0, s, ms, p->depth, a, ds);
-        else hipLaunchKernelGGL((k_alloc_scan_sdf<false, true>), sgrid, block, 0, s, ms, p->depth, a, ds);
-      } else {
-        if (p->stats) hipLaunchKernelGGL((k_alloc_scan_sdf<true, false>), sgrid, block, 0, s, ms, p->depth, a, ds);
-        else hipLaunchKernelGGL((k_alloc_scan_sdf<false, false>), sgrid, block, 0, s, ms, p->depth, a, ds);
-      }
-    } else {
-      if (p->stats) hipLaunchKernelGGL(k_alloc_scan_ofusion<true>, grid, block, 0, s, ms, p->depth, a, ds);
-      else hipLaunchKernelGGL(k_alloc_scan_ofusion<false>, grid, block, 0, s, ms, p->depth, a, ds);
-    }
+  const int fused_wgs = sdf ? (sdf_tiles + SE_WG / 64 - 1) / (SE_WG / 64) : (npix + SE_WG - 1) / SE_WG;
+  if (!ov && p->hold_scan_ok && own_list && ds.kind == 0 && fuse_scan_sweep_ok(p, fused_wgs)) {
+    p->held.valid = true; p->held.ms = ms; p->held.a = a; p->held.wgs = fused_wgs;
+  } else {
+    launch_scan(p, ms, a, ds, s);
   }
   input_slot_in_use(p);
   if (ov) {
@@ -971,7 +1007,7 @@
   }
   p->occ_commit_due = true;
   if (!p->occ_lists.lists) p->occ_lists = OccLists{p->map.newkeys, 1, (long long)p->map.cap_keys + 1};
-  if (!sdf && !a.sharded) {
+  if (!sdf && !a.sharded && !p->held.valid) {
     if (int r = run_zero_chain(p, m.newkeys, 1, (long long)m.cap_keys + 1)) return r;
   }
   HIP_TRY(hipGetLastError());
@@ -1081,10 +1117,16 @@
   return se_hip_apply_bricks(p, recv_device, p->xworld);
 }
 
+static bool sort_due(se_hip_pipeline* p, int sweeps_since_sort) {
+  if (p->sort_every <= 0 || !p->map.dense) return false;
+  const uint32_t n0 = std::min<uint32_t>(p->ctr_host[C_BLOCKS], p->map.cap_blocks);
+  return !(sweeps_since_sort < p->sort_every || n0 < 4096 || (size_t)n0 * 2 < (size_t)p->sorted_n * 3);
+}
 static int sort_block_list(se_hip_pipeline* p) {
   if (p->sort_every <= 0 || !p->map.dense) return SE_HIP_OK;
   const uint32_t n0 = std::min<uint32_t>(p->ctr_host[C_BLOCKS], p->map.cap_blocks);
-  if (++p->sweeps_since_sort < p->sort_every || n0 < 4096 || (size_t)n0 * 2 < (size_t)p->sorted_n * 3) return SE_HIP_OK;
+  ++p->sweeps_since_sort;
+  if (!sort_due(p, p->sweeps_since_sort)) return SE_HIP_OK;
   if (p->sort_cap < n0) {
     if (p->bpos_sorted) hipFree(p->bpos_sorted);
     if (p->sort_tmp) hipFree(p->sort_tmp);
@@ -1112,6 +1154,7 @@
   if (int r = join_scan(p, true)) return r;
   materialise_depth(p, p->stream);
   input_slot_in_use(p);
+  if (p->held.valid && sort_due(p, p->sweeps_since_sort + 1)) { if (int r = launch_held_scan(p)) return r; }
   if (int r = sort_block_list(p)) return r;
   const DevMap& m = p->map;
   const M4 pose = from_colmajor(pose_cm);
@@ -1184,6 +1227,26 @@
     const dim3 grid(p->integ_grid > 0 ? (unsigned)p->integ_grid : (unsigned)wgs);
 #define SE_SWEEP(OF, FD, SHD) hipLaunchKernelGGL((k_integrate<OF, FD, SHD>), grid, block, 0, p->stream, m, p->depth, a)
     a.stats = p->stats ? 1 : 0;
+    if (p->held.valid && a.shard_world <= 1) {
+      p->held.valid = false;
+      p->n_launch[SE_HIP_K_ALLOC_SCAN]++; p->n_fused_scan_sweep++;
+      const int w = p->done_next;
+      if (!p->done_clean[w]) HIP_TRY(hipMemsetAsync(p->scan_done, 0, 4 * sizeof(uint32_t), p->stream));
+      ScanDone h{p->scan_done + w, p->scan_done + (1 - w), (uint32_t)p->held.wgs + (sdf ? 0u : 1u)};
+      p->done_clean[w] = false; p->done_clean[1 - w] = true; p->done_next = 1 - w;
+      const dim3 fgrid(grid.x + (unsigned)p->held.wgs);
+#define SE_FUSED(OF, FD, DN) hipLaunchKernelGGL((k_scan_integrate<OF, FD, DN>), fgrid, block, 0, p->stream, m, p->depth, a, p->held.wgs, p->held.ms, p->held.a, h)
+      switch ((sdf ? 0 : 4) | (a.fast_div ? 2 : 0) | (sdf && m.dense ? 1 : 0)) {
+        case 0: SE_FUSED(false, false, false); break;
+        case 1: SE_FUSED(false, false, true); break;
+        case 2: SE_FUSED(false, true, false); break;
+        case 3: SE_FUSED(false, true, true); break;
+        case 4: SE_FUSED(true, false, false); break;
+        default: SE_FUSED(true, true, false); break;
+      }
+#undef SE_FUSED
+    } else {
+    if (p->held.valid) { if (int r = launch_held_scan(p)) return r; }
     switch ((sdf ? 0 : 4) | (a.fast_div ? 2 : 0) | (a.shard_world > 1 ? 1 : 0)) {
       case 0: SE_SWEEP(false, false, false); break;
       case 1: SE_SWEEP(false, false, true); break;
@@ -1194,6 +1257,7 @@
       case 6: SE_SWEEP(true, true, false); break;
       case 7: SE_SWEEP(true, true, true); break;
     }
+    }
 #undef SE_SWEEP
   }
   if (p->host_gate) { p->gate_armed = true; p->gate_followed = false; p->gate_target = p->ray_seq + 1u; }
@@ -1252,10 +1316,13 @@
   if (!pose || !k || rate == 0) return fail(SE_HIP_E_INVALID, "bad argument");
   if (!finite_pose(pose, k)) return fail(SE_HIP_E_INVALID, "non-finite pose or intrinsics");
   if (p->has_pending && !(frame_can_fuse(p) && stage_runs_integration(frame, rate))) { if (int r = flush_pending_raycast(p)) return r; }
+  p->hold_scan_ok = !p->has_pending;
   int r = se_hip_alloc_scan(p, pose, k, rate, mu, frame);
+  p->hold_scan_ok = false;
   if (p->has_pending) { if (int q = flush_pending_raycast(p)) return q; }
-  if (r <= 0) return r;
-  return se_hip_integrate_sweep(p, pose, k, rate, mu, frame);
+  if (r > 0) r = se_hip_integrate_sweep(p, pose, k, rate, mu, frame);
+  if (p->held.valid) { if (int q = launch_held_scan(p)) return q; }
+  return r;
 }
 
 int se_hip_raycast_deferred(se_hip_pipeline* p, const float pose[16], const float k[4], float mu, uint32_t frame) {
@@ -2297,6 +2364,13 @@
   return SE_HIP_OK;
 }
 
+int se_hip_get_fused_scan_sweep(se_hip_pipeline* p, int64_t* count, int32_t reset) {
+  if (!p) return fail(SE_HIP_E_INVALID, "null handle");
+  if (count) *count = p->n_fused_scan_sweep;
+  if (reset) p->n_fused_scan_sweep = 0;
+  return SE_HIP_OK;
+}
+
 int se_hip_get_launch_counts(se_hip_pipeline* p, int64_t counts[SE_HIP_K_COUNT + 1], int32_t reset) {
   if (!p) return fail(SE_HIP_E_INVALID, "null handle");
   for (int i = 0; i <= SE_HIP_K_COUNT; ++i) {
diff --git a/supereight_amd/csrc/se_kernels.h b/supereight_amd/csrc/se_kernels.h
--- a/supereight_amd/csrc/se_kernels.h
+++ b/supereight_amd/csrc/se_kernels.h
@@ -347,12 +347,13 @@
 }
 
 struct OccLists { const unsigned long long* lists; int nlists; long long stride_words; };
+template <bool HANDED = false>
 __device__ __forceinline__ void se_occ_commit(const DevMap& m, const OccLists L, unsigned nwg, unsigned first = 0u) {
   if (blockIdx.x < first || blockIdx.x >= first + nwg) return;
   const unsigned wg = blockIdx.x - first;
   for (int li = 0; li < L.nlists; ++li) {
     const unsigned long long* list = L.lists + (long long)li * L.stride_words;
-    unsigned long long n = list[0];
+    unsigned long long n = HANDED ? __hip_atomic_load(list, __ATOMIC_RELAXED, __HIP_MEMORY_SCOPE_AGENT) : list[0];
     if (n > (unsigned long long)(L.stride_words - 1)) n = (unsigned long long)(L.stride_words - 1);
     for (unsigned long long i = wg * (unsigned long long)blockDim.x + threadIdx.x; i < n; i += (unsigned long long)nwg * blockDim.x) {
       const unsigned long long raw = list[1 + i];
@@ -374,7 +375,7 @@
 }
 __global__ __launch_bounds__(SE_WG) void k_occ_commit(DevMap m, OccLists L) { se_occ_commit(m, L, gridDim.x); }
 
-__global__ __launch_bounds__(SE_WG) void k_zero_chain(DevMap m, const unsigned long long* __restrict__ lists, int nlists, long long stride_words) {
+__device__ __forceinline__ void se_zero_chain_wg(const DevMap& m, const unsigned long long* lists, int nlists, long long stride_words) {
   __shared__ unsigned long long s_best[SE_WG / 64];
   __shared__ unsigned long long s_chain[3];
   unsigned long long lower = 0ull;
@@ -382,7 +383,7 @@
     unsigned long long best = ~0ull;
     for (int li = 0; li < nlists; ++li) {
       const unsigned long long* list = lists + (long long)li * stride_words;
-      unsigned long long n = list[0];
+      unsigned long long n = __hip_atomic_load(list, __ATOMIC_RELAXED, __HIP_MEMORY_SCOPE_AGENT);
       if (n > (unsigned long long)(stride_words - 1)) n = (unsigned long long)(stride_words - 1);
       for (unsigned long long i = threadIdx.x; i < n; i += SE_WG) {
         const unsigned long long k = list[1 + i];
@@ -420,6 +421,9 @@
     const int x = (int)(se_compact21(code) >> sh), y = (int)(se_compact21(code >> 1) >> sh), z = (int)(se_compact21(code >> 2) >> sh);
     se_insert_octant(m, l, x, y, z);
   }
+}
+__global__ __launch_bounds__(SE_WG) void k_zero_chain(DevMap m, const unsigned long long* __restrict__ lists, int nlists, long long stride_words) {
+  se_zero_chain_wg(m, lists, nlists, stride_words);
 }
 
 #define SE_SHARD_SUB 64
@@ -689,26 +693,72 @@
 #else
 #define SE_SWEEP_OCC
 #endif
-template <bool OFUSION, bool FAST, bool SHARD>
-__global__ __launch_bounds__(SE_WG) SE_SWEEP_OCC void k_integrate(DevMap m, const float* __restrict__ depthmap, IntegArgs a) {
+struct ScanDone { uint32_t* done; uint32_t* zero_next; uint32_t target; };
+#ifndef SE_HANDOVER_POLLS
+#define SE_HANDOVER_POLLS 12288
+#endif
+#define SE_OVERFLOW_HANDOVER 4u
+__device__ __forceinline__ uint32_t se_handover_publish(uint32_t* done) {
+  asm volatile("s_waitcnt vmcnt(0)" ::: "memory");
+  __syncthreads();
+  uint32_t old = 0u;
+  if (threadIdx.x == 0) {
+    __threadfence();
+    asm volatile("s_waitcnt vmcnt(0)" ::: "memory");
+    old = __hip_atomic_fetch_add(done, 1u, __ATOMIC_RELAXED, __HIP_MEMORY_SCOPE_AGENT);
+  }
+  return old;
+}
+__device__ __forceinline__ bool se_handover_wait(const ScanDone& h, unsigned* s_flag) {
+  if (threadIdx.x == 0) {
+    unsigned ok = 0u;
+    for (int i = 0; i < SE_HANDOVER_POLLS; ++i) {
+      if (__hip_atomic_load(h.done, __ATOMIC_RELAXED, __HIP_MEMORY_SCOPE_AGENT) >= h.target) { ok = 1u; break; }
+      __builtin_amdgcn_s_sleep(8);
+    }
+    __builtin_amdgcn_fence(__ATOMIC_ACQUIRE, "agent");
+    asm volatile("s_waitcnt vmcnt(0)" ::: "memory");
+    *s_flag = ok;
+  }
+  __syncthreads();
+  return *s_flag != 0u;
+}
+
+template <bool OFUSION, bool FAST, bool SHARD, bool HANDOVER>
+__device__ __forceinline__ void se_integrate_wg(const DevMap& m, const float* __restrict__ depthmap, const IntegArgs& a, unsigned bid, unsigned nwg, unsigned first_wg,
+                                                unsigned* s_hist, const ScanDone& h) {
   const int lane = threadIdx.x & 63;
-  const int wave = (blockIdx.x * SE_WG + threadIdx.x) >> 6;
-  const int nwaves = (gridDim.x * SE_WG) >> 6;
-  const uint32_t nblocks = min(m.ctr[C_BLOCKS], m.cap_blocks);
-  const uint32_t nnodes = min(m.ctr[C_NODES], m.cap_nodes);
+  const int wave = (bid * SE_WG + threadIdx.x) >> 6;
+  const int nwaves = (nwg * SE_WG) >> 6;
+  uint32_t nblocks = 0u, nnodes = 0u;
+  if (!HANDOVER) {
+    nblocks = min(m.ctr[C_BLOCKS], m.cap_blocks);
+    nnodes = min(m.ctr[C_NODES], m.cap_nodes);
+  }
   const int lx = lane & 7, ly = lane >> 3;
   const float fx = (float)lx;
   unsigned long long swept = 0;
-  if (a.ctr_mirror && blockIdx.x == gridDim.x - 1 && threadIdx.x < C_COUNT) a.ctr_mirror[threadIdx.x] = m.ctr[threadIdx.x];
-  if (a.zero_count && blockIdx.x == gridDim.x - 1 && threadIdx.x == 0) *a.zero_count = 0ull;
-  __shared__ unsigned s_hist[784];
-  const bool scheduler = a.prio_thr != nullptr && gridDim.x > 1;
+  if (!HANDOVER && a.ctr_mirror && bid == nwg - 1 && threadIdx.x < C_COUNT) a.ctr_mirror[threadIdx.x] = m.ctr[threadIdx.x];
+  if (a.zero_count && bid == nwg - 1 && threadIdx.x == 0) *a.zero_count = 0ull;
+  if (HANDOVER && bid == nwg - 1 && threadIdx.x == 0) *h.zero_next = 0u;
+  const bool scheduler = a.prio_thr != nullptr && nwg > 1;
   const int wskip = scheduler ? SE_WG / 64 : 0;
-  if (a.commit_occ) se_occ_commit(m, a.occ_lists, min(gridDim.x - (scheduler ? 1u : 0u), 64u), scheduler ? 1u : 0u);
-  if (scheduler && blockIdx.x == 0) se_ray_schedule(a.tile_cost, a.n_tiles, a.prio_thr, s_hist, a.prio_permille, a.ray_order);
+  if (!HANDOVER && a.commit_occ) se_occ_commit(m, a.occ_lists, min(nwg - (scheduler ? 1u : 0u), 64u), first_wg + (scheduler ? 1u : 0u));
+  if (scheduler && bid == 0) se_ray_schedule(a.tile_cost, a.n_tiles, a.prio_thr, s_hist, a.prio_permille, a.ray_order);
   const SeRcp rmu = se_rcp_refined(a.mu);
+  if (HANDOVER) {
+    if (scheduler && bid == 0) __builtin_amdgcn_s_setprio(0);
+    if (!se_handover_wait(h, s_hist + 784)) {
+      if (threadIdx.x == 0) __hip_atomic_store(&m.ctr[C_OVERFLOW], SE_OVERFLOW_HANDOVER, __ATOMIC_RELAXED, __HIP_MEMORY_SCOPE_AGENT);
+      return;
+    }
+    nblocks = min((uint32_t)__builtin_amdgcn_readfirstlane((int)__hip_atomic_load(&m.ctr[C_BLOCKS], __ATOMIC_RELAXED, __HIP_MEMORY_SCOPE_AGENT)), m.cap_blocks);
+    nnodes = min((uint32_t)__builtin_amdgcn_readfirstlane((int)__hip_atomic_load(&m.ctr[C_NODES], __ATOMIC_RELAXED, __HIP_MEMORY_SCOPE_AGENT)), m.cap_nodes);
+    if (a.ctr_mirror && bid == nwg - 1 && threadIdx.x < C_COUNT) a.ctr_mirror[threadIdx.x] = __hip_atomic_load(&m.ctr[threadIdx.x], __ATOMIC_RELAXED, __HIP_MEMORY_SCOPE_AGENT);
+    if (a.commit_occ) se_occ_commit<true>(m, a.occ_lists, min(nwg - (scheduler ? 1u : 0u), 64u), first_wg + (scheduler ? 1u : 0u));
+  }
   const uint32_t stride = (uint32_t)(nwaves - wskip);
-  uint32_t b = (scheduler && blockIdx.x == 0) ? 0xFFFFFFFFu : (uint32_t)(wave - wskip);
+  uint32_t b = (scheduler && bid == 0) ? 0xFFFFFFFFu : (uint32_t)(wave - wskip);
   uint32_t bp_next = m.bpos[min(b, m.cap_blocks - 1u)];
   for (; b < nblocks; b += stride) {
     const uint32_t bp = bp_next;
@@ -809,8 +859,39 @@
     }
   }
   if (a.stats && lane == 0 && swept) atomicAdd(&m.stats[S_SWEPT], swept);
-  for (uint32_t tid = blockIdx.x * SE_WG + threadIdx.x; tid < nnodes * 8u; tid += gridDim.x * SE_WG)
+  for (uint32_t tid = bid * SE_WG + threadIdx.x; tid < nnodes * 8u; tid += nwg * SE_WG)
     se_update_node_corner<OFUSION>(m, depthmap, a, tid);
+}
+template <bool OFUSION, bool FAST, bool SHARD>
+__global__ __launch_bounds__(SE_WG) SE_SWEEP_OCC void k_integrate(DevMap m, const float* __restrict__ depthmap, IntegArgs a) {
+  __shared__ unsigned s_hist[784];
+  se_integrate_wg<OFUSION, FAST, SHARD, false>(m, depthmap, a, blockIdx.x, gridDim.x, 0u, s_hist, ScanDone{nullptr, nullptr, 0u});
+}
+
+static_assert(SE_WG == 2 * SE_WG_SCAN, "k_scan_integrate: a workgroup = two of the scan's");
+template <bool OFUSION, bool FAST, bool DENSE>
+__global__ __launch_bounds__(SE_WG) SE_SWEEP_OCC void k_scan_integrate(DevMap m, const float* __restrict__ depthmap, IntegArgs a, int scan_wgs, DevMap ms, AllocArgs sa,
+                                                                      ScanDone h) {
+  __shared__ uint32_t smem[2 * SE_SCAN_SLOTS * SE_WG_SCAN];
+  static_assert(2 * SE_SCAN_SLOTS * SE_WG_SCAN >= 785, "k_scan_integrate: the sweep's LDS");
+  if ((int)blockIdx.x < scan_wgs) {
+    const DepthSrc ds{nullptr, nullptr, 0, 0, 0};
+    if (OFUSION) se_scan_ofusion_wg<false>(ms, depthmap, sa, 2 * (int)blockIdx.x, ds);
+    else se_scan_sdf_wg<false, DENSE>(ms, depthmap, sa, smem + (threadIdx.x >= SE_WG_SCAN ? (SE_SCAN_SLOTS - 1) * SE_WG_SCAN : 0), 2 * (int)blockIdx.x, ds);
+    const uint32_t before = se_handover_publish(h.done);
+    if (OFUSION) {
+      if (threadIdx.x == 0) smem[0] = before == (uint32_t)scan_wgs - 1u ? 1u : 0u;
+      __syncthreads();
+      if (smem[0]) {
+        if (threadIdx.x == 0) { __builtin_amdgcn_fence(__ATOMIC_ACQUIRE, "agent"); asm volatile("s_waitcnt vmcnt(0)" ::: "memory"); }
+        __syncthreads();
+        se_zero_chain_wg(m, m.newkeys, 1, (long long)m.cap_keys + 1);
+        se_handover_publish(h.done);
+      }
+    }
+    return;
+  }
+  se_integrate_wg<OFUSION, FAST, false, true>(m, depthmap, a, blockIdx.x - (unsigned)scan_wgs, gridDim.x - (unsigned)scan_wgs, (unsigned)scan_wgs, smem, h);
 }
 
 __global__ __launch_bounds__(SE_WG) void k_apply_bricks(DevMap m, const unsigned char* __restrict__ recv, size_t seg_bytes, uint32_t cap, int self) {
diff --git a/supereight_amd/pipeline.py b/supereight_amd/pipeline.py
--- a/supereight_amd/pipeline.py
+++ b/supereight_amd/pipeline.py
@@ -96,6 +96,7 @@
     "se_hip_set_image_ring": (C.c_int, [C.c_void_p, C.c_void_p, C.c_int32]),
     "se_hip_raycast_deferred": (C.c_int, [C.c_void_p, C.c_void_p, C.c_void_p, C.c_float, C.c_uint32]),
     "se_hip_get_launch_counts": (C.c_int, [C.c_void_p, C.POINTER(C.c_int64), C.c_int32]),
+    "se_hip_get_fused_scan_sweep": (C.c_int, [C.c_void_p, C.POINTER(C.c_int64), C.c_int32]),
     "se_hip_upload_depth": (C.c_int, [C.c_void_p, _f32p]),
     "se_hip_upload_depth_mm": (C.c_int, [C.c_void_p, np.ctypeslib.ndpointer(dtype=np.uint16, flags="C_CONTIGUOUS"), C.c_int32, C.c_int32]),
     "se_hip_set_depth_device": (C.c_int, [C.c_void_p, C.c_void_p]),
@@ -313,6 +314,9 @@
         pend = self._check(self.lib.se_hip_get_launch_counts(self._h, n, int(reset)))
         out = {k: int(n[i]) for i, k in enumerate(KERNELS)}
         out["fused"] = int(n[len(KERNELS)])
+        fss = C.c_int64(0)
+        self._check(self.lib.se_hip_get_fused_scan_sweep(self._h, C.byref(fss), int(reset)))
+        out["fused_scan_sweep"] = int(fss.value)
         out["pending"] = bool(pend)
         return out
 
```

New measurement: 17010. No clear change (-0.0%).
